# jopohl/urh

Measured on NVIDIA H100. Metric: MSamples/s IQ demod+digitize (complex64), higher is better.
Workload: dtype f32

## Files before the change

urh_b200/csrc/center.cu:

```cuda
#include "dense.cuh"
#include "scan.cuh"

#include <math.h>
#include <stdlib.h>

int urh_window_var_bitwise(urh_ctx* ctx, const float* d_x, int64_t n, const int64_t* d_prefix, int64_t t0, int64_t t1, int64_t r0,
                           int64_t r1, float* h_out2);

struct CenStats {
    double sum, sumsq;
    float mn, mx;
    long long cnt;
};

__global__ void __launch_bounds__(URH_WARPS_PER_BLOCK * 32)
k_tile_stats_f32(const float* __restrict__ x, int64_t n, int64_t ntiles, UrhTileStats* __restrict__ ts) {
    const int lane = threadIdx.x & 31;
    const int64_t tile = (int64_t)blockIdx.x * URH_WARPS_PER_BLOCK + (threadIdx.x >> 5);
    if (tile >= ntiles) return;
    const int64_t base = tile * URH_TILE;
    UrhStatAcc acc;
    acc.init();
    acc.all_noise = false;
    if (base + URH_TILE <= n && (((uintptr_t)x) & 15) == 0) {
// ... 344 lines not shown
    const int lane = threadIdx.x & 31;
    if (SMEM)
        for (int b = threadIdx.x; b < nbins; b += 256) s_hist[b] = 0u;
    if (edges_in_smem)
        for (int b = threadIdx.x; b < nbins + 3; b += 256) s_fe[b] = g_fe[b];
    __syncthreads();
    HistBins hb;
    if (FAST) hb.load(s_fe, scale, nbins);
    else hb.load(edges_in_smem ? s_fe : g_fe, scale, nbins);
    HistCache hc;
    hc.init();
    const int64_t gw = (int64_t)blk * 8 + (threadIdx.x >> 5), nw = (int64_t)nblk * 8;
    const bool vec = (((uintptr_t)x) & 15) == 0;
    const unsigned one = blockDim.x >> 8;
    {
        for (int64_t t = t_first + gw; t < t_end; t += nw) {
            if (prefix[t + 1] == prefix[t]) continue;
            const int64_t base = t * URH_TILE;
            if (vec) {
                const float4* p = (const float4*)(x + base) + lane;
                constexpr int ITERS = URH_TILE / 128, DEPTH = 4;
                float4 buf[DEPTH];
#pragma unroll
                for (int j = 0; j < DEPTH; j++) buf[j] = __ldg(p + j * 32);
#pragma unroll 1
                for (int it = 0; it < ITERS; it += DEPTH) {
                    const bool more = it + DEPTH < ITERS;
#pragma unroll
                    for (int j = 0; j < DEPTH; j++) {
                        const float4 v = buf[j];
                        if (more) buf[j] = __ldg(p + (it + DEPTH + j) * 32);
                        hist_put<SMEM, FAST>(hc, hb, s_hist, hist, v.x, one);
                        hist_put<SMEM, FAST>(hc, hb, s_hist, hist, v.y, one);
                        hist_put<SMEM, FAST>(hc, hb, s_hist, hist, v.z, one);
                        hist_put<SMEM, FAST>(hc, hb, s_hist, hist, v.w, one);
                    }
                }
            } else {
                for (int j = lane; j < URH_TILE; j += 32) hist_put<SMEM, FAST>(hc, hb, s_hist, hist, x[base + j], one);
            }
        }
    }
    hist_flush<SMEM>(hc, s_hist, hist);
    if (SMEM) {
        __syncthreads();
        for (int b = threadIdx.x; b < nbins; b += 256)
            if (s_hist[b]) atomicAdd(&hist[b], (unsigned long long)s_hist[b]);
    }
}

template <bool SMEM, bool FAST>
__global__ void __launch_bounds__(256, 4) k_hist_interior(const float* __restrict__ x, int64_t n, const int64_t* __restrict__ win,
                                                      const float* __restrict__ g_fe, float scale, int nbins,
                                                      unsigned long long* __restrict__ hist, int edges_in_smem,
                                                      const int64_t* __restrict__ prefix) {
    const int64_t w0 = win[0];
    hist_interior_body<SMEM, FAST>(x, n, w0 + 1, w0 >= 0 ? win[1] : 0, blockIdx.x, gridDim.x, g_fe, scale, nbins, hist, edges_in_smem, prefix);
}

__device__ __forceinline__ void hist_window_ends_body(const float* __restrict__ x, int64_t n, const int64_t* __restrict__ prefix,
                                                      const int64_t* __restrict__ win, int64_t r0, int64_t r1,
                                                      const float* __restrict__ g_fe, float scale, int nbins,
                                                      unsigned long long* __restrict__ hist, unsigned long long* __restrict__ hist2 = nullptr) {
    __shared__ int s_pre[256];
    const int64_t t = win[blockIdx.x];
    if (t < 0 || (blockIdx.x == 1 && t == win[0])) return;
    HistBins hb;
    hb.load(g_fe, scale, nbins);
    float v[CEN_PER];
    int64_t rank = cen_tile_ranks(x, n, t, prefix[t], v, s_pre);
#pragma unroll
    for (int j = 0; j < CEN_PER; j++) {
        const bool kept = v[j] > -4.0f;
        const int k = hb.bin_of<false>(v[j]);
        if (k >= 0 && rank >= r0 && rank < r1) {
            atomicAdd(&hist[k], 1ull);
            if (hist2) atomicAdd(&hist2[k], 1ull);
        }
        rank += kept ? 1 : 0;
    }
}

__global__ void __launch_bounds__(256) k_hist_window_ends(const float* __restrict__ x, int64_t n, const int64_t* __restrict__ prefix,
                                                         const int64_t* __restrict__ win, int64_t r0, int64_t r1,
                                                         const float* __restrict__ g_fe, float scale, int nbins,
                                                         unsigned long long* __restrict__ hist) {
    hist_window_ends_body(x, n, prefix, win, r0, r1, g_fe, scale, nbins, hist);
}

extern "C" int urh_center_histogram_tiles(urh_ctx* ctx, const float* d_qad, int64_t n, int64_t r0, int64_t r1, double hmin,
                                          double hstep, int64_t nbins, int64_t* h_hist) {
    if (nbins <= 0) return URH_OK;
    if (!tiles_match(ctx, d_qad, n)) URH_FAIL(ctx, URH_ERR_INVALID, "urh_afp_demod_tiles (same qad, same n) must precede urh_center_histogram_tiles");
    if (nbins > (int64_t)1 << 30) URH_FAIL(ctx, URH_ERR_INVALID, "too many histogram bins");
    const int64_t ntiles = urh_div_up(n, URH_TILE);
    const int64_t* prefix = (const int64_t*)ctx->center_prefix;
    unsigned long long* hist;
    float* fe;
    int64_t* d_win;
    URH_CHECK(urh_arena(ctx, (size_t)nbins, &hist));
    URH_CHECK(urh_arena(ctx, (size_t)nbins + 3, &fe));
    URH_CHECK(urh_arena(ctx, 4, &d_win));
    URH_CUDA(ctx, cudaMemsetAsync(hist, 0, (size_t)nbins * sizeof(unsigned long long), ctx->stream));
    URH_CUDA(ctx, cudaMemsetAsync(d_win, 0xff, 4 * sizeof(int64_t), ctx->stream));
    if (r1 > r0) {
        URH_LAUNCH(ctx, k_hist_edges, (unsigned)urh_div_up(nbins + 1, 256), 256, 0, hmin, hstep, nbins, fe);
        URH_LAUNCH(ctx, k_find_window_tiles, (unsigned)urh_div_up(ntiles, 256), 256, 0, prefix, ntiles, r0, r1, d_win);
        const bool in_smem = nbins <= 12000;
        const int edges_smem = (in_smem && nbins <= 6000) ? 1 : 0;
        const size_t dyn = (in_smem ? (size_t)nbins * 4 : 0) + (edges_smem ? (size_t)(nbins + 3) * 4 : 0);
        const float scale = (float)(1.0 / hstep);
        const double edge_abs = fmax(fabs(hmin), fabs(hmin + (double)nbins * hstep));
        const bool fast = edges_smem && hstep > 0.0 && edge_abs / hstep < 1048576.0;
        const unsigned gs = (unsigned)min(urh_div_up(ntiles, 8), (int64_t)ctx->sm_count * 8);
        const int64_t* cw = d_win;
        const float* cfe = fe;
        if (in_smem && fast) URH_LAUNCH(ctx, (k_hist_interior<true, true>), gs, 256, dyn, d_qad, n, cw, cfe, scale, (int)nbins, hist, edges_smem, prefix);
        else if (in_smem) URH_LAUNCH(ctx, (k_hist_interior<true, false>), gs, 256, dyn, d_qad, n, cw, cfe, scale, (int)nbins, hist, edges_smem, prefix);
        else URH_LAUNCH(ctx, (k_hist_interior<false, false>), gs, 256, dyn, d_qad, n, cw, cfe, scale, (int)nbins, hist, edges_smem, prefix);
        URH_LAUNCH(ctx, k_hist_window_ends, 2, 256, 0, d_qad, n, prefix, (const int64_t*)d_win, r0, r1, (const float*)fe, scale, (int)nbins, hist);
    }
    URH_CUDA(ctx, cudaMemcpyAsync(h_hist, hist, (size_t)nbins * sizeof(int64_t), cudaMemcpyDeviceToHost, ctx->stream));
    URH_CUDA(ctx, cudaStreamSynchronize(ctx->stream));
    return URH_OK;
}

extern "C" int urh_center_histogram(urh_ctx* ctx, const float* d_x, int64_t n, int64_t r0, int64_t r1, double hmin,
                                    double hstep, int64_t nbins, int64_t* h_hist) {
    if (nbins <= 0 || n <= 0) return URH_OK;
    if (!tiles_match(ctx, d_x, n)) {
        int64_t total = 0;
        URH_CHECK(tiles_from_array(ctx, d_x, n, &total));
    }
    return urh_center_histogram_tiles(ctx, d_x, n, r0, r1, hmin, hstep, nbins, h_hist);
}

#include "tilescan.cuh"

#define CEN_MAX_BINS 6000

struct __align__(16) CenterPlan {
    long long total, offset;
    long long r0, r1;
    long long lr0, lr1;
    long long win[4];
    CenStats local;
    double hmin, edge1, delta;
    long long nbins;
    double center;
    float centerf;
    float scale;
    int fast;
    int state;
    unsigned int ticket;
    int certified;
    long long straddle;
    long long pad;
};

struct ScanKept {
    const UrhTileStats* ts;
    int64_t* prefix;
    __device__ __forceinline__ int64_t load(int64_t t) const { return ts[t].cnt; }
    __device__ __forceinline__ void post(int64_t t, const int64_t& excl, const int64_t&) const { prefix[t] = excl; }
};
struct CenAddI64 {
    __device__ __forceinline__ int64_t operator()(int64_t a, int64_t b) const { return a + b; }
};

__global__ void k_center_ranks(const int64_t* __restrict__ counts, int rank, int world, int64_t max_size, CenterPlan* __restrict__ plan) {
    long long total = 0, offset = 0;
    for (int q = 0; q < world; q++) {
        if (q < rank) offset += counts[q];
        total += counts[q];
    }
    const long long kept = counts[rank];
    long long r0 = (long long)(0.05 * (double)total), r1 = (long long)(0.95 * (double)total);
    if (max_size >= 0 && r1 - r0 > max_size) r1 = r0 + max_size;
    plan->total = total; plan->offset = offset; plan->r0 = r0; plan->r1 = r1;
    long long a = r0 - offset, b = r1 - offset;
    a = a < 0 ? 0 : (a > kept ? kept : a);
    b = b < 0 ? 0 : (b > kept ? kept : b);
    plan->lr0 = a; plan->lr1 = b;
    plan->ticket = 0u;
    plan->state = 1;
    plan->certified = 0;
    plan->straddle = 0;
}

__device__ __forceinline__ int64_t cen_tile_of_rank(const int64_t* __restrict__ prefix, int64_t ntiles, int64_t r) {
    int64_t lo = 0, hi = ntiles;
    while (hi - lo > 1) {
        const int64_t mid = (lo + hi) >> 1;
        if (prefix[mid] <= r) lo = mid; else hi = mid;
    }
    return lo;
}

__global__ void __launch_bounds__(256) k_center_window(const float* __restrict__ x, int64_t n, const UrhTileStats* __restrict__ ts,
                                                      const int64_t* __restrict__ prefix, int64_t ntiles, CenterPlan* __restrict__ plan,
                                                      CenStats* __restrict__ partial) {
    __shared__ long long s_win[4];
    __shared__ int s_pre[256];
    __shared__ bool s_last;
    const long long r0 = plan->lr0, r1 = plan->lr1;
    if (threadIdx.x == 0) {
        long long w0 = -1, w1 = -1, w2 = -1, w3 = -1;
        if (r1 > r0) {
            w0 = cen_tile_of_rank(prefix, ntiles, r0);
            w1 = cen_tile_of_rank(prefix, ntiles, r1 - 1);
            const bool cov0 = prefix[w0] >= r0 && prefix[w0 + 1] <= r1;
            const bool cov1 = prefix[w1] >= r0 && prefix[w1 + 1] <= r1;
            w2 = cov0 ? -1 : w0;
            w3 = (cov1 || w1 == w0) ? -1 : w1;
        }
        s_win[0] = w0; s_win[1] = w1; s_win[2] = w2; s_win[3] = w3;
        if (blockIdx.x == 0) { plan->win[0] = w0; plan->win[1] = w1; plan->win[2] = w2; plan->win[3] = w3; }
    }
    __syncthreads();
    double sum = 0.0, sq = 0.0;
    float mn = INFINITY, mx = -INFINITY;
    long long cnt = 0;
    if (s_win[0] >= 0) {
        for (int64_t t = s_win[0] + (int64_t)blockIdx.x * 256 + threadIdx.x; t <= s_win[1]; t += (int64_t)gridDim.x * 256) {
            const int64_t a = prefix[t], b = prefix[t + 1];
            if (b > a && a >= r0 && b <= r1) {
                const UrhTileStats v = ts[t];
                sum += v.sum; sq += v.sumsq; mn = fminf(mn, v.mn); mx = fmaxf(mx, v.mx); cnt += v.cnt;
            }
        }
    }
    cen_block_fold(sum, sq, mn, mx, cnt, partial + blockIdx.x);
    if (blockIdx.x < 2) {
        const int64_t t = s_win[2 + blockIdx.x];
        sum = 0.0; sq = 0.0; mn = INFINITY; mx = -INFINITY; cnt = 0;
        if (t >= 0) {
            float v[CEN_PER];
            int64_t rank = cen_tile_ranks(x, n, t, prefix[t], v, s_pre);
#pragma unroll
            for (int j = 0; j < CEN_PER; j++) {
                if (v[j] > -4.0f) {
                    if (rank >= r0 && rank < r1) {
                        sum += (double)v[j];
                        sq += (double)v[j] * (double)v[j];
                        mn = fminf(mn, v[j]);
                        mx = fmaxf(mx, v[j]);
                        cnt++;
                    }
                    rank++;
                }
            }
        }
        cen_block_fold(sum, sq, mn, mx, cnt, partial + gridDim.x + blockIdx.x);
    }
    __threadfence();
    __syncthreads();
    if (threadIdx.x == 0) s_last = atomicAdd(&plan->ticket, 1u) == gridDim.x - 1;
    __syncthreads();
    if (!s_last) return;
    __threadfence();
    sum = 0.0; sq = 0.0; mn = INFINITY; mx = -INFINITY; cnt = 0;
    for (int64_t t = threadIdx.x; t < (int64_t)gridDim.x + 2; t += 256) {
        CenStats p;
        {
            const int4* src = (const int4*)(partial + t);
            int4 w0 = __ldcg(src), w1 = __ldcg(src + 1);
            memcpy(&p, &w0, 16);
            memcpy((char*)&p + 16, &w1, 16);
        }
        sum += p.sum; sq += p.sumsq; mn = fminf(mn, p.mn); mx = fmaxf(mx, p.mx); cnt += p.cnt;
    }
    cen_block_fold(sum, sq, mn, mx, cnt, &plan->local);
}

__global__ void __launch_bounds__(256) k_center_plan(const CenStats* __restrict__ parts, int world, CenterPlan* __restrict__ plan,
                                                    float* __restrict__ fe, unsigned long long* __restrict__ hist,
                                                    unsigned long long* __restrict__ xhist) {
    __shared__ int s_state;
    __shared__ long long s_nbins;
    __shared__ double s_hmin, s_edge1, s_delta;
    if (threadIdx.x == 0) {
        double cnt = 0.0, sum = 0.0, sq = 0.0;
        float mn = INFINITY, mx = -INFINITY;
        for (int q = 0; q < world; q++) {
            cnt += (double)parts[q].cnt;
            mn = fminf(mn, parts[q].mn);
            mx = fmaxf(mx, parts[q].mx);
            sum = __dadd_rn(sum, parts[q].sum);
            sq = __dadd_rn(sq, parts[q].sumsq);
        }
        int state = 0;
        long long nbins = 0;
        double hmin = 0.0, edge1 = 0.0, delta = 0.0;
        if (plan->r1 > plan->r0 && cnt > 0.0) {
            const double mean = __ddiv_rn(sum, cnt);
            double ss = __dsub_rn(sq, __dmul_rn(__dmul_rn(cnt, mean), mean));
            if (ss < 0.0) ss = 0.0;
            const double var = __ddiv_rn(ss, cnt);
            const double hstep = (double)__double2float_rn(var);
            hmin = (double)mn;
            const double stop = __dadd_rn((double)mx, hstep);
            if (hstep != 0.0) {
                const double val = __ddiv_rn(__dsub_rn(stop, hmin), hstep);
                if (val == val && fabs(val) < 9.0e18) {
                    const long long len = (long long)ceil(val);
                    if (len >= 2) {
                        nbins = len - 1;
                        edge1 = __dadd_rn(hmin, hstep);
                        delta = __dsub_rn(edge1, hmin);
                        state = (nbins <= CEN_MAX_BINS && delta > 0.0) ? 1 : 2;
                    }
                }
            }
        }
        plan->hmin = hmin; plan->edge1 = edge1; plan->delta = delta; plan->nbins = nbins;
        plan->state = state;
        plan->center = 0.0; plan->centerf = 0.0f;
        if (state == 1) {
            plan->scale = (float)(1.0 / delta);
            const double edge_abs = fmax(fabs(hmin), fabs(hmin + (double)nbins * delta));
            plan->fast = (edge_abs / delta < 1048576.0) ? 1 : 0;
        }
        s_state = state; s_nbins = nbins; s_hmin = hmin; s_edge1 = edge1; s_delta = delta;
    }
    __syncthreads();
    if (s_state != 1) return;
    const long long nbins = s_nbins;
    for (long long k = threadIdx.x; k <= nbins; k += 256) {
        const double e = (k == 0) ? s_hmin : (k == 1 ? s_edge1 : __dadd_rn(s_hmin, __dmul_rn((double)k, s_delta)));
        fe[k] = __double2float_ru(e);
        if (k == nbins) {
            fe[nbins + 1] = __double2float_rd(e);
            fe[nbins + 2] = fmaxf(__double2float_ru(s_hmin), nextafterf(-4.0f, 0.0f));
        }
        if (k < nbins) {
            hist[k] = 0ull;
            if (xhist) xhist[k] = 0ull;
        }
    }
}

template <bool FAST>
__global__ void __launch_bounds__(256, 3) k_hist_interior_dev(const float* __restrict__ x, int64_t n, const CenterPlan* __restrict__ plan,
                                                          const float* __restrict__ g_fe, unsigned long long* __restrict__ hist,
                                                          const int64_t* __restrict__ prefix) {
    if (plan->state != 1 || plan->certified || (plan->fast != 0) != FAST) return;
    hist_interior_body<true, FAST>(x, n, plan->win[0] + 1, plan->win[1], blockIdx.x, gridDim.x, g_fe, plan->scale, (int)plan->nbins, hist, 1,
                                   prefix);
}

__device__ __forceinline__ void cen_full_slabs(int64_t win0, int64_t win1, int64_t slab_tiles, int64_t* sf, int64_t* se) {
    *sf = (win0 + slab_tiles) / slab_tiles;
    *se = win1 / slab_tiles;
}

__global__ void __launch_bounds__(256) k_hist_window_ends_dev(const float* __restrict__ x, int64_t n, const int64_t* __restrict__ prefix,
                                                             const CenterPlan* __restrict__ plan, const float* __restrict__ g_fe,
                                                             unsigned long long* __restrict__ hist, unsigned long long* __restrict__ xhist,
                                                             int64_t slab_tiles) {
    if (plan->state != 1) return;
    if (blockIdx.x < 2) {
        hist_window_ends_body(x, n, prefix, (const int64_t*)plan->win, plan->lr0, plan->lr1, g_fe, plan->scale, (int)plan->nbins, hist, xhist);
        return;
    }
    const int64_t w0 = plan->win[0], w1 = plan->win[1];
    int64_t sf, se;
    cen_full_slabs(w0, w1, slab_tiles, &sf, &se);
    int64_t a_end = w1, b_begin = w1;
    if (sf < se) { a_end = sf * slab_tiles; b_begin = se * slab_tiles; }
    const int blk = blockIdx.x - 2, nblk = gridDim.x - 2, nbins = (int)plan->nbins;
    const float scale = plan->scale;
    if (plan->fast) {
        hist_interior_body<true, true>(x, n, w0 + 1, a_end, blk, nblk, g_fe, scale, nbins, xhist, 1, prefix);
        hist_interior_body<true, true>(x, n, b_begin, w1, blk, nblk, g_fe, scale, nbins, xhist, 1, prefix);
    } else {
        hist_interior_body<true, false>(x, n, w0 + 1, a_end, blk, nblk, g_fe, scale, nbins, xhist, 1, prefix);
        hist_interior_body<true, false>(x, n, b_begin, w1, blk, nblk, g_fe, scale, nbins, xhist, 1, prefix);
    }
}

__device__ __forceinline__ double cen_left_edge(const CenterPlan* plan, int k) {
    return (k == 0) ? plan->hmin : (k == 1 ? plan->edge1 : __dadd_rn(plan->hmin, __dmul_rn((double)k, plan->delta)));
}

#define CERT_THREADS 512
__global__ void __launch_bounds__(CERT_THREADS) k_center_certify(const UrhFine fine, CenterPlan* __restrict__ plan, const float* __restrict__ fe,
                                                                 const unsigned long long* __restrict__ xhist, unsigned long long* __restrict__ lo,
                                                                 unsigned long long* __restrict__ hi) {
    __shared__ unsigned long long s_ge[URH_FINE_NB + 1];
    __shared__ unsigned long long s_part[CERT_THREADS];
    __shared__ unsigned char s_flag[CEN_MAX_BINS];
    __shared__ unsigned long long s_key[3];
    __shared__ unsigned int s_certain;
    if (plan->state != 1) return;
    const int tid = threadIdx.x;
    constexpr int PER = URH_FINE_NB / CERT_THREADS;
    int64_t sf, se;
    cen_full_slabs(plan->win[0], plan->win[1], fine.slab_tiles, &sf, &se);
    unsigned long long b[PER], tot = 0;
#pragma unroll
    for (int j = 0; j < PER; j++) {
        unsigned long long v = 0;
        for (int64_t sl = sf; sl < se; sl++) v += fine.gh[sl * URH_FINE_NB + tid * PER + j];
        b[j] = v;
        tot += v;
    }
    s_part[tid] = tot;
    if (tid < 3) s_key[tid] = 0ull;
    if (tid == 0) s_certain = 0u;
    __syncthreads();
    for (int off = 1; off < CERT_THREADS; off <<= 1) {
        const unsigned long long add = (tid + off < CERT_THREADS) ? s_part[tid + off] : 0ull;
        __syncthreads();
        s_part[tid] += add;
        __syncthreads();
    }
    unsigned long long run = (tid + 1 < CERT_THREADS) ? s_part[tid + 1] : 0ull;
#pragma unroll
    for (int j = PER - 1; j >= 0; j--) {
        run += b[j];
        s_ge[tid * PER + j] = run;
    }
    if (tid == 0) s_ge[URH_FINE_NB] = 0ull;
    __syncthreads();
    const int nbins = (int)plan->nbins;
    const float f_hi = fe[nbins + 1], f_min = fe[nbins + 2], top = nextafterf(f_hi, INFINITY);
    auto ge = [&](float t, unsigned long long& glo, unsigned long long& ghi) {
        const int bt = urh_fine_bucket(t, fine.scale, fine.off);
        const bool straddles = urh_fine_bucket(nextafterf(t, -INFINITY), fine.scale, fine.off) == bt;
        ghi = s_ge[bt];
        glo = straddles ? s_ge[bt + 1] : s_ge[bt];
    };
    for (int k = tid; k < nbins; k += CERT_THREADS) {
        const float a = fmaxf(fe[k], f_min), e = (k == nbins - 1) ? top : fminf(fe[k + 1], top);
        unsigned long long l = 0, u = 0;
        if (a < e) {
            unsigned long long alo, ahi, elo, ehi;
            ge(a, alo, ahi);
            ge(e, elo, ehi);
            l = alo > ehi ? alo - ehi : 0ull;
            u = ahi - elo;
        }
        lo[k] = xhist[k] + l;
        hi[k] = xhist[k] + u;
    }
    __syncthreads();
    int window = (int)(0.05 * (double)nbins) + 1;
    if (window < 2) window = 2;
    for (int k = tid; k < nbins; k += CERT_THREADS) {
        const unsigned long long l = lo[k], u = hi[k];
        bool certain = l > 0ull, possible = u > 0ull;
        for (int d = -(window - 1); d < window && (certain || possible); d++) {
            const int j = k + d;
            if (d == 0 || j < 0 || j >= nbins) continue;
            certain = certain && l > hi[j];
            possible = possible && u > lo[j];
        }
        s_flag[k] = certain ? 1 : (possible ? 2 : 0);
        if (certain) atomicAdd(&s_certain, 1u);
    }
    __syncthreads();
    for (int pass = 0; pass < 3; pass++) {
        const long long p0 = pass > 0 ? (long long)(8191 - (s_key[0] & 8191)) : -1, p1 = pass > 1 ? (long long)(8191 - (s_key[1] & 8191)) : -1;
        for (int k = tid; k < nbins; k += CERT_THREADS) {
            if (k == p0 || k == p1) continue;
            if (pass < 2 && s_flag[k] == 1) atomicMax(&s_key[pass], (lo[k] << 13) | (unsigned long long)(8191 - k));
            if (pass == 2 && s_flag[k] != 0) atomicMax(&s_key[2], hi[k]);
        }
        __syncthreads();
    }
    if (tid != 0 || s_certain < 2u) return;
    const int k1 = 8191 - (int)(s_key[0] & 8191), k2 = 8191 - (int)(s_key[1] & 8191);
    plan->straddle = (long long)((hi[k1] - lo[k1]) + (hi[k2] - lo[k2]));
    if (!(lo[k2] > s_key[2])) return;
    const double c = __ddiv_rn(__dadd_rn(cen_left_edge(plan, k1), cen_left_edge(plan, k2)), 2.0);
    plan->center = c;
    plan->centerf = __double2float_rn(c);
    plan->certified = 1;
}

__global__ void __launch_bounds__(256) k_center_pick(const unsigned long long* __restrict__ y, CenterPlan* __restrict__ plan) {
    __shared__ unsigned long long s_best[256];
    __shared__ int s_idx[256];
    __shared__ int s_cnt[256];
    if (plan->state != 1 || plan->certified) return;
    const int nbins = (int)plan->nbins;
    int window = (int)(0.05 * (double)nbins) + 1;
    if (window < 2) window = 2;
    unsigned long long top_val[2] = {0ull, 0ull};
    int top_idx[2] = {-1, -1};
    int found = 0;
    bool undecided = false;
    for (int pass = 0; pass < 2 && !undecided; pass++) {
        unsigned long long best = 0ull;
        int bi = -1, ties = 0;
        for (int i = threadIdx.x; i < nbins; i += 256) {
            if (pass == 1 && i == top_idx[0]) continue;
            const unsigned long long v = y[i];
            if (v == 0ull || v < best) continue;
            bool peak = true;
            for (int d = 1; d < window && peak; d++) {
                const unsigned long long a = (i + d < nbins) ? y[i + d] : 0ull;
                const unsigned long long b = (i - d >= 0) ? y[i - d] : 0ull;
                peak = v > a && v > b;
            }
            if (!peak) continue;
            if (v > best) { best = v; bi = i; ties = 1; }
            else ties++;
        }
        s_best[threadIdx.x] = best; s_idx[threadIdx.x] = bi; s_cnt[threadIdx.x] = ties;
        __syncthreads();
        if (threadIdx.x == 0) {
            unsigned long long b = 0ull;
            int idx = -1, t = 0;
            for (int j = 0; j < 256; j++) {
                if (s_idx[j] < 0) continue;
                if (s_best[j] > b) { b = s_best[j]; idx = s_idx[j]; t = s_cnt[j]; }
                else if (s_best[j] == b) t += s_cnt[j];
            }
            s_best[0] = b; s_idx[0] = idx; s_cnt[0] = t;
        }
        __syncthreads();
        const unsigned long long b = s_best[0];
        const int idx = s_idx[0], t = s_cnt[0];
        __syncthreads();
        if (idx < 0) break;
        if (pass == 0) {
            top_val[0] = b; top_idx[0] = idx; found = 1;
            if (t == 2) {
                int other = -1;
                for (int i = threadIdx.x; i < nbins; i += 256) {
                    if (i == idx || y[i] != b) continue;
                    bool peak = true;
                    for (int d = 1; d < window && peak; d++) {
                        const unsigned long long a = (i + d < nbins) ? y[i + d] : 0ull;
                        const unsigned long long c = (i - d >= 0) ? y[i - d] : 0ull;
                        peak = b > a && b > c;
                    }
                    if (peak) other = i;
                }
                s_idx[threadIdx.x] = other;
                __syncthreads();
                if (threadIdx.x == 0) {
                    int o = -1;
                    for (int j = 0; j < 256; j++) if (s_idx[j] >= 0) o = s_idx[j];
                    s_idx[0] = o;
                }
                __syncthreads();
                top_idx[1] = s_idx[0]; top_val[1] = b; found = 2;
                __syncthreads();
                break;
            }
            if (t > 2) undecided = true;
        } else {
            if (t > 1) undecided = true;
            else { top_val[1] = b; top_idx[1] = idx; found = 2; }
        }
    }
    if (threadIdx.x != 0) return;
    if (undecided) { plan->state = 2; return; }
    if (found == 0) { plan->state = 0; return; }
    double c;
    if (found == 1) c = cen_left_edge(plan, top_idx[0]);
    else c = __ddiv_rn(__dadd_rn(cen_left_edge(plan, top_idx[0]), cen_left_edge(plan, top_idx[1])), 2.0);
    plan->center = c;
    plan->centerf = __double2float_rn(c);
    plan->state = 1;
    (void)top_val;
}

int urh_coll_allgather(urh_ctx* ctx, const void* d_send, void* d_recv, size_t bytes_per_rank);
bool urh_p2p_usable(urh_ctx* ctx, size_t bytes_per_rank);
extern "C" int urh_p2p_allreduce_u64_dev(urh_ctx* ctx, const void* d_in, void* d_out, const int64_t* d_count, int max_words);
extern "C" int urh_nccl_allreduce_i64(urh_ctx* ctx, int64_t* d_buf, int64_t count, int op);

int urh_center_chain(urh_ctx* ctx, const float* d_qad, int64_t n, const UrhTileStats* ts, int64_t max_size, int rank, int world,
                     const UrhFine* fine, CenterPlan** d_plan_out) {
    const int64_t ntiles = urh_div_up(n, URH_TILE);
    int64_t* prefix;
    CenterPlan* plan;
    CenStats* partial;
    float* fe;
    unsigned long long* hist;
    int64_t* d_counts;
    CenStats* d_parts;
    unsigned long long *xhist = nullptr, *cert_lo = nullptr, *cert_hi = nullptr;
    const int nb = ctx->sm_count * 2;
    URH_CHECK(urh_arena(ctx, (size_t)ntiles + 1, &prefix));
    URH_CHECK(urh_arena(ctx, 1, &plan));
    URH_CHECK(urh_arena(ctx, (size_t)nb + 2, &partial));
    URH_CHECK(urh_arena(ctx, (size_t)CEN_MAX_BINS + 3, &fe));
    URH_CHECK(urh_arena(ctx, (size_t)CEN_MAX_BINS, &hist));
    URH_CHECK(urh_arena(ctx, (size_t)world, &d_counts));
    URH_CHECK(urh_arena(ctx, (size_t)world, &d_parts));
    if (fine) {
        URH_CHECK(urh_arena(ctx, (size_t)CEN_MAX_BINS, &xhist));
        URH_CHECK(urh_arena(ctx, (size_t)CEN_MAX_BINS, &cert_lo));
        URH_CHECK(urh_arena(ctx, (size_t)CEN_MAX_BINS, &cert_hi));
    }
    ScanKept fk;
    fk.ts = ts; fk.prefix = prefix;
    URH_CHECK((urhts::scan<int64_t, CenAddI64, ScanKept>(ctx, ntiles, (int64_t)0, CenAddI64(), fk, prefix + ntiles)));
    const int64_t* counts = prefix + ntiles;
    if (world > 1) {
        URH_TL_MARK(ctx, "x1 kept counts: enter");
        URH_CHECK(urh_coll_allgather(ctx, prefix + ntiles, d_counts, sizeof(int64_t)));
        URH_TL_MARK(ctx, "x1 kept counts: done");
        counts = d_counts;
    }
    URH_LAUNCH(ctx, k_center_ranks, 1, 1, 0, counts, rank, world, max_size, plan);
    URH_LAUNCH(ctx, k_center_window, nb, 256, 0, d_qad, n, ts, (const int64_t*)prefix, ntiles, plan, partial);
    const CenStats* parts = &plan->local;
    if (world > 1) {
        URH_TL_MARK(ctx, "x2 window partials: enter");
        URH_CHECK(urh_coll_allgather(ctx, &plan->local, d_parts, sizeof(CenStats)));
        URH_TL_MARK(ctx, "x2 window partials: done");
        parts = d_parts;
    }
    URH_LAUNCH(ctx, k_center_plan, 1, 256, 0, parts, world, plan, fe, hist, xhist);
    const size_t dyn = (size_t)CEN_MAX_BINS * 4 + (size_t)(CEN_MAX_BINS + 3) * 4;
    const unsigned gs = (unsigned)min(urh_div_up(ntiles, 8), (int64_t)ctx->sm_count * 8);
    URH_LAUNCH(ctx, k_hist_window_ends_dev, fine ? 2 + ctx->sm_count * 4 : 2, 256, fine ? dyn : 0, d_qad, n, (const int64_t*)prefix,
               (const CenterPlan*)plan, (const float*)fe, hist, xhist, fine ? fine->slab_tiles : (int64_t)1);
    if (fine) URH_LAUNCH(ctx, k_center_certify, 1, CERT_THREADS, 0, *fine, plan, (const float*)fe, (const unsigned long long*)xhist, cert_lo, cert_hi);
    URH_LAUNCH(ctx, (k_hist_interior_dev<true>), gs, 256, dyn, d_qad, n, (const CenterPlan*)plan, (const float*)fe, hist, (const int64_t*)prefix);
    URH_LAUNCH(ctx, (k_hist_interior_dev<false>), gs, 256, dyn, d_qad, n, (const CenterPlan*)plan, (const float*)fe, hist, (const int64_t*)prefix);
    const unsigned long long* hist_all = hist;
    if (world > 1) URH_TL_MARK(ctx, "x3 histogram sum: enter");
    if (world > 1) {
        if (urh_p2p_usable(ctx, 8)) {
            unsigned long long* hist_sum;
            URH_CHECK(urh_arena(ctx, (size_t)CEN_MAX_BINS, &hist_sum));
            URH_CHECK(urh_p2p_allreduce_u64_dev(ctx, hist, hist_sum, (const int64_t*)&plan->nbins, CEN_MAX_BINS));
            hist_all = hist_sum;
        } else {
            URH_CHECK(urh_nccl_allreduce_i64(ctx, (int64_t*)hist, CEN_MAX_BINS, 0));
        }
    }
    if (world > 1) URH_TL_MARK(ctx, "x3 histogram sum: done");
    URH_LAUNCH(ctx, k_center_pick, 1, 256, 0, hist_all, plan);
    ctx->center_prefix = prefix;
    ctx->center_ts = ts;
    ctx->center_n = n;
    ctx->center_x = d_qad;
    *d_plan_out = plan;
    return URH_OK;
}

int urh_center_plan_certify_stats(urh_ctx* ctx, const CenterPlan* plan, int64_t* h_dst3) {
    h_dst3[0] = h_dst3[1] = h_dst3[2] = 0;
    URH_CUDA(ctx, cudaMemcpyAsync(h_dst3, &plan->certified, sizeof(int), cudaMemcpyDeviceToHost, ctx->stream));
    URH_CUDA(ctx, cudaMemcpyAsync(h_dst3 + 2, &plan->straddle, sizeof(long long), cudaMemcpyDeviceToHost, ctx->stream));
    return URH_OK;
}

extern "C" int urh_center_certify_stats(urh_ctx* ctx, int64_t* h_out3) {
    for (int i = 0; i < 3; i++) h_out3[i] = ctx->center_cert[i];
    return URH_OK;
}

int urh_center_plan_result(urh_ctx* ctx, const CenterPlan* plan, const float** d_centerf, const double** d_center, const int** d_state) {
    if (d_centerf) *d_centerf = &plan->centerf;
    if (d_center) *d_center = &plan->center;
    if (d_state) *d_state = &plan->state;
    return URH_OK;
}
```

urh_b200/csrc/common.cuh:

```cuda
#pragma once
#include <cuda_runtime.h>
#include <stdint.h>
#include <stdio.h>
#include <stdlib.h>
#include <string.h>
#include <vector>

#include "../../include/urh_b200.h"

#define URH_FULL_MASK 0xffffffffu

struct urh_block {
    void* ptr;
    size_t bytes;
};

struct urh_ctx {
    int device;
    int sm_count;
    cudaStream_t stream;
    cudaStream_t copy_stream[2];
    cudaEvent_t ev_start, ev_stop;
    cudaEvent_t ev_copy[2], ev_comp[2];
    cudaEvent_t ev_k0, ev_k1;
    int profiling;
    int dense_timed;
    cudaEvent_t tl_ev[32];
    const char* tl_name[32];
    int tl_count, tl_ready;
    char err[512];
    int64_t launches;
    std::vector<urh_block> arena;
    size_t arena_block;
    size_t arena_used;
    size_t arena_need;
    int64_t* pulses;
    size_t pulses_cap_rows;
    int64_t pulses_k;
    int64_t* h_mail;
    void* h_stage[2];
    size_t h_stage_bytes;
    int fft_plan;
    int fft_nfft;
    int64_t fft_batch;
    bool fft_valid;
    void* img_tw;
    int img_tw_n;
    void* shard_tiles;
    void* shard_staging;
    int shard_cap, shard_tol;
    int64_t shard_n;
    void* shard_state;
    int64_t costas_stats[3];
    int64_t costas_redone;
    int64_t costas_stitch[4];
    int mod_plan[2];
    int mod_plan_valid[2];
    int64_t mod_plan_n[2];
    int bits_valid;
    int64_t bits_nmsg, bits_total, bits_npos;
    void *bits_ptr, *bits_msg_off, *bits_pauses, *bits_pos;
    const void* center_ts;
    const void* center_x;
    int64_t center_n;
    void* center_prefix;
    int64_t center_cert[3];
    int64_t spec_stats[3];
    void* nccl_comm;
    void* nccl_stage;
    void* nccl_hstage;
    int nccl_rank, nccl_world;
    void* p2p_local;
    void* p2p_peer[8];
    void* p2p_hout;
    int p2p_rank, p2p_world;
    unsigned long long p2p_seq;
    void* ts_mem;
    int64_t ts_cap_blocks;
    unsigned long long ts_issued;
    uint32_t ts_epoch;
    void* step_dev;
    void* shard_fin;
    int64_t stream_free_low, stream_chunks;
    size_t arena_live;
    size_t arena_peak;
};

#define URH_CUDA(ctx, call)                                                                         \
    do {                                                                                            \
        cudaError_t e__ = (call);                                                                   \
        if (e__ != cudaSuccess) {                                                                   \
            snprintf((ctx)->err, sizeof((ctx)->err), "%s:%d: %s -> %s", __FILE__, __LINE__, #call,  \
                     cudaGetErrorString(e__));                                                      \
            return (e__ == cudaErrorMemoryAllocation) ? URH_ERR_NOMEM : URH_ERR_CUDA;               \
        }                                                                                           \
    } while (0)

#define URH_CHECK(call)                 \
    do {                                \
        int rc__ = (call);              \
        if (rc__ != URH_OK) return rc__; \
    } while (0)

#define URH_FAIL(ctx, code, ...)                                  \
    do {                                                          \
        snprintf((ctx)->err, sizeof((ctx)->err), __VA_ARGS__);    \
        return (code);                                            \
    } while (0)

#define URH_LAUNCH(ctx, kernel, grid, block, smem, ...)                                   \
    do {                                                                                  \
        kernel<<<(grid), (block), (smem), (ctx)->stream>>>(__VA_ARGS__);                  \
        (ctx)->launches++;                                                                \
        URH_CUDA(ctx, cudaGetLastError());                                                \
    } while (0)

#define URH_TL_MARK(ctx, label) do { if ((ctx)->profiling >= 2 && (ctx)->tl_ready && (ctx)->tl_count < 32) { \
        (ctx)->tl_name[(ctx)->tl_count] = (label); cudaEventRecord((ctx)->tl_ev[(ctx)->tl_count++], (ctx)->stream); } } while (0)
#define URH_TL_RESET(ctx) do { (ctx)->tl_count = 0; } while (0)
#define URH_PROF_BEGIN(ctx) do { if ((ctx)->profiling) cudaEventRecord((ctx)->ev_k0, (ctx)->stream); } while (0)
#define URH_PROF_END(ctx) do { if ((ctx)->profiling) { cudaEventRecord((ctx)->ev_k1, (ctx)->stream); (ctx)->dense_timed = 1; } } while (0)

void urh_arena_reset(urh_ctx* ctx);
int urh_arena_alloc(urh_ctx* ctx, size_t bytes, void** out);
template <typename T>
static inline int urh_arena(urh_ctx* ctx, size_t count, T** out) {
    void* p = nullptr;
    int rc = urh_arena_alloc(ctx, count * sizeof(T), &p);
    *out = (T*)p;
    return rc;
}
struct UrhArenaMark {
    size_t block, used, live;
};
static inline UrhArenaMark urh_arena_mark(const urh_ctx* ctx) { return UrhArenaMark{ctx->arena_block, ctx->arena_used, ctx->arena_live}; }
static inline void urh_arena_release(urh_ctx* ctx, const UrhArenaMark& m) {
    ctx->arena_block = m.block;
    ctx->arena_used = m.used;
    ctx->arena_live = m.live;
}
int urh_ensure_pulses(urh_ctx* ctx, size_t rows);
int urh_ensure_pulses_keep(urh_ctx* ctx, size_t rows, size_t keep);
void urh_stream_sample_free(urh_ctx* ctx);
void urh_release_mod_plans(urh_ctx* ctx);
int urh_ensure_stage(urh_ctx* ctx, size_t bytes);

struct UrhCostasStream {
    float* state;
    int64_t* acc;
    int segs;
};
int urh_costas_stream_begin(urh_ctx* ctx, UrhCostasStream* S);
int urh_costas_stream_chunk(urh_ctx* ctx, UrhCostasStream* S, int64_t c, const void* d_iq, int dtype, int64_t n, float noise_sqrd,
                            int loop_order, float bandwidth, float* d_out);
int urh_costas_stream_end(urh_ctx* ctx, const UrhCostasStream* S);
int64_t urh_costas_arena_bytes(int64_t n, int loop_order);

int urh_read_i64(urh_ctx* ctx, const int64_t* d_src, int count, int64_t* h_out);

__host__ __device__ static inline int64_t urh_div_up(int64_t a, int64_t b) { return (a + b - 1) / b; }

static inline int urh_iq_bytes(int dtype) {
    switch (dtype) {
        case URH_DT_I8:
        case URH_DT_U8: return 2;
        case URH_DT_I16:
        case URH_DT_U16: return 4;
        case URH_DT_F32: return 8;
        default: return 0;
    }
}

static inline float urh_noise_value(int mod_type) {
    switch (mod_type) {
        case URH_MOD_ASK: return 0.0f;
        case URH_MOD_FSK:
        case URH_MOD_PSK:
        case URH_MOD_OQPSK: return -4.0f;
        case URH_MOD_QAM: return 0.0f * -4.0f;
        default: return 0.0f;
    }
}
```

urh_b200/csrc/context.cu:

```cuda
#include "common.cuh"
#include "tilescan.cuh"

extern "C" int urh_device_count(void) {
    int n = 0;
    if (cudaGetDeviceCount(&n) != cudaSuccess) return 0;
    return n;
}

extern "C" int urh_ctx_create(int device, urh_ctx** out) {
    if (!out) return URH_ERR_INVALID;
    *out = nullptr;
    int n = 0;
    if (cudaGetDeviceCount(&n) != cudaSuccess || n <= 0) return URH_ERR_NO_DEVICE;
    if (device < 0 || device >= n) return URH_ERR_INVALID;
    urh_ctx* ctx = new urh_ctx();
    ctx->device = device;
    ctx->err[0] = 0;
    ctx->launches = 0;
    ctx->arena_block = 0;
    ctx->arena_used = 0;
    ctx->arena_need = 0;
    ctx->pulses = nullptr;
    ctx->pulses_cap_rows = 0;
    ctx->pulses_k = 0;
    ctx->h_mail = nullptr;
    ctx->h_stage[0] = ctx->h_stage[1] = nullptr;
    ctx->h_stage_bytes = 0;
    ctx->fft_valid = false;
    ctx->shard_tiles = nullptr;
    ctx->shard_staging = nullptr;
    ctx->shard_state = nullptr;
    ctx->bits_valid = 0;
    ctx->mod_plan_valid[0] = ctx->mod_plan_valid[1] = 0;
    ctx->center_prefix = nullptr;
    ctx->center_ts = nullptr;
    ctx->center_x = nullptr;
    ctx->center_n = 0;
    ctx->nccl_comm = nullptr;
    ctx->nccl_stage = nullptr;
    ctx->nccl_hstage = nullptr;
    ctx->p2p_local = nullptr;
    ctx->p2p_hout = nullptr;
    ctx->p2p_world = 0;
    ctx->p2p_rank = 0;
    ctx->p2p_seq = 0;
    for (int i = 0; i < 8; i++) ctx->p2p_peer[i] = nullptr;
    ctx->nccl_rank = 0;
    ctx->nccl_world = 1;
    ctx->stream_free_low = -1;
    ctx->stream_chunks = 0;
    if (cudaSetDevice(device) != cudaSuccess) {
        delete ctx;
        return URH_ERR_CUDA;
    }
    cudaDeviceProp prop;
    if (cudaGetDeviceProperties(&prop, device) != cudaSuccess) {
        delete ctx;
        return URH_ERR_CUDA;
    }
    ctx->sm_count = prop.multiProcessorCount;
    {
        cudaMemPool_t pool;
        if (cudaDeviceGetDefaultMemPool(&pool, device) == cudaSuccess) {
            unsigned long long keep = ~0ull;
            cudaMemPoolSetAttribute(pool, cudaMemPoolAttrReleaseThreshold, &keep);
        }
    }
    bool ok = cudaStreamCreateWithFlags(&ctx->stream, cudaStreamNonBlocking) == cudaSuccess;
    ok = ok && cudaStreamCreateWithFlags(&ctx->copy_stream[0], cudaStreamNonBlocking) == cudaSuccess;
    ok = ok && cudaStreamCreateWithFlags(&ctx->copy_stream[1], cudaStreamNonBlocking) == cudaSuccess;
    ok = ok && cudaEventCreate(&ctx->ev_start) == cudaSuccess && cudaEventCreate(&ctx->ev_stop) == cudaSuccess;
    for (int i = 0; i < 2 && ok; i++) {
        ok = ok && cudaEventCreateWithFlags(&ctx->ev_copy[i], cudaEventDisableTiming) == cudaSuccess;
        ok = ok && cudaEventCreateWithFlags(&ctx->ev_comp[i], cudaEventDisableTiming) == cudaSuccess;
    }
    ok = ok && cudaEventCreate(&ctx->ev_k0) == cudaSuccess && cudaEventCreate(&ctx->ev_k1) == cudaSuccess;
    ctx->profiling = 0;
    ctx->dense_timed = 0;
    ctx->tl_count = 0;
    ctx->tl_ready = 0;
    ok = ok && cudaHostAlloc((void**)&ctx->h_mail, 64 * sizeof(int64_t), cudaHostAllocDefault) == cudaSuccess;
    if (!ok) {
        delete ctx;
        return URH_ERR_CUDA;
    }
    *out = ctx;
    return URH_OK;
}

extern "C" void urh_ctx_destroy(urh_ctx* ctx) {
    if (!ctx) return;
    cudaSetDevice(ctx->device);
    cudaStreamSynchronize(ctx->stream);
    urh_release_mod_plans(ctx);
    for (auto& b : ctx->arena) cudaFree(b.ptr);
    if (ctx->pulses) cudaFree(ctx->pulses);
    if (ctx->shard_state) free(ctx->shard_state);
    if (ctx->h_mail) cudaFreeHost(ctx->h_mail);
    if (ctx->ts_mem) cudaFree(ctx->ts_mem);
    if (ctx->step_dev) cudaFree(ctx->step_dev);
    if (ctx->img_tw) cudaFree(ctx->img_tw);
    if (ctx->shard_fin) free(ctx->shard_fin);
    for (int i = 0; i < 2; i++)
        if (ctx->h_stage[i]) cudaFreeHost(ctx->h_stage[i]);
    cudaEventDestroy(ctx->ev_start);
    cudaEventDestroy(ctx->ev_stop);
    for (int i = 0; i < 2; i++) {
        cudaEventDestroy(ctx->ev_copy[i]);
        cudaEventDestroy(ctx->ev_comp[i]);
        cudaStreamDestroy(ctx->copy_stream[i]);
    }
    cudaStreamDestroy(ctx->stream);
    delete ctx;
}

extern "C" const char* urh_last_error(urh_ctx* ctx) { return ctx ? ctx->err : "null context"; }

extern "C" int urh_sync(urh_ctx* ctx) {
    URH_CUDA(ctx, cudaStreamSynchronize(ctx->stream));
    return URH_OK;
}

extern "C" int urh_device_info(urh_ctx* ctx, int* sm_count, int* cc_major, int* cc_minor, size_t* total_mem,
                               char* name, int name_cap) {
    cudaDeviceProp prop;
    URH_CUDA(ctx, cudaGetDeviceProperties(&prop, ctx->device));
    if (sm_count) *sm_count = prop.multiProcessorCount;
    if (cc_major) *cc_major = prop.major;
    if (cc_minor) *cc_minor = prop.minor;
    if (total_mem) *total_mem = prop.totalGlobalMem;
    if (name && name_cap > 0) {
        strncpy(name, prop.name, name_cap - 1);
        name[name_cap - 1] = 0;
    }
    return URH_OK;
}

extern "C" int urh_malloc(urh_ctx* ctx, size_t bytes, void** d_ptr) {
    URH_CUDA(ctx, cudaSetDevice(ctx->device));
    if (bytes == 0) bytes = 16;
    URH_CUDA(ctx, cudaMallocAsync(d_ptr, bytes, ctx->stream));
    return URH_OK;
}

extern "C" int urh_free(urh_ctx* ctx, void* d_ptr) {
    if (!d_ptr) return URH_OK;
    URH_CUDA(ctx, cudaFreeAsync(d_ptr, ctx->stream));
    return URH_OK;
}

extern "C" int urh_memset(urh_ctx* ctx, void* d_ptr, int value, size_t bytes) {
    URH_CUDA(ctx, cudaMemsetAsync(d_ptr, value, bytes, ctx->stream));
    return URH_OK;
}

extern "C" int urh_memcpy_h2d(urh_ctx* ctx, void* d_dst, const void* h_src, size_t bytes) {
    if (bytes == 0) return URH_OK;
    URH_CUDA(ctx, cudaMemcpyAsync(d_dst, h_src, bytes, cudaMemcpyHostToDevice, ctx->stream));
    return URH_OK;
}

extern "C" int urh_memcpy_d2h(urh_ctx* ctx, void* h_dst, const void* d_src, size_t bytes) {
    if (bytes) URH_CUDA(ctx, cudaMemcpyAsync(h_dst, d_src, bytes, cudaMemcpyDeviceToHost, ctx->stream));
    URH_CUDA(ctx, cudaStreamSynchronize(ctx->stream));
    return URH_OK;
}

extern "C" int urh_memcpy_d2d(urh_ctx* ctx, void* d_dst, const void* d_src, size_t bytes) {
    if (bytes == 0) return URH_OK;
    URH_CUDA(ctx, cudaMemcpyAsync(d_dst, d_src, bytes, cudaMemcpyDeviceToDevice, ctx->stream));
    return URH_OK;
}

extern "C" int urh_host_alloc(urh_ctx* ctx, size_t bytes, void** h_ptr) {
    if (bytes == 0) bytes = 16;
    URH_CUDA(ctx, cudaHostAlloc(h_ptr, bytes, cudaHostAllocDefault));
    return URH_OK;
}

extern "C" int urh_host_free(urh_ctx* ctx, void* h_ptr) {
    if (h_ptr) URH_CUDA(ctx, cudaFreeHost(h_ptr));
    return URH_OK;
}

extern "C" int urh_timer_start(urh_ctx* ctx) {
    URH_CUDA(ctx, cudaEventRecord(ctx->ev_start, ctx->stream));
    return URH_OK;
}

extern "C" int urh_timer_stop(urh_ctx* ctx, float* ms) {
    URH_CUDA(ctx, cudaEventRecord(ctx->ev_stop, ctx->stream));
    URH_CUDA(ctx, cudaEventSynchronize(ctx->ev_stop));
    float t = 0.f;
    URH_CUDA(ctx, cudaEventElapsedTime(&t, ctx->ev_start, ctx->ev_stop));
    if (ms) *ms = t;
    return URH_OK;
}

extern "C" int urh_set_profiling(urh_ctx* ctx, int enabled) {
    ctx->profiling = enabled < 0 ? 0 : (enabled > 2 ? 2 : enabled);
    ctx->dense_timed = 0;
    if (ctx->profiling >= 2 && !ctx->tl_ready) {
        for (int i = 0; i < 32; i++) URH_CUDA(ctx, cudaEventCreate(&ctx->tl_ev[i]));
        ctx->tl_ready = 1;
    }
    ctx->tl_count = 0;
    return URH_OK;
}

extern "C" int urh_timeline_fetch(urh_ctx* ctx, float* h_ms, char* h_names, int names_cap, int* count) {
    if (!count) return URH_ERR_INVALID;
    *count = 0;
    if (ctx->profiling < 2 || ctx->tl_count == 0) return URH_OK;
    URH_CUDA(ctx, cudaEventSynchronize(ctx->tl_ev[ctx->tl_count - 1]));
    int pos = 0;
    for (int i = 0; i < ctx->tl_count; i++) {
        float t = 0.f;
        URH_CUDA(ctx, cudaEventElapsedTime(&t, ctx->tl_ev[0], ctx->tl_ev[i]));
        if (h_ms) h_ms[i] = t;
        if (h_names) pos += snprintf(h_names + pos, pos < names_cap ? (size_t)(names_cap - pos) : 0, "%s\n", ctx->tl_name[i]);
    }
    *count = ctx->tl_count;
    return URH_OK;
}

extern "C" int urh_last_dense_ms(urh_ctx* ctx, float* ms) {
    if (!ctx->dense_timed) URH_FAIL(ctx, URH_ERR_INVALID, "no dense kernel timed (enable urh_set_profiling first)");
    URH_CUDA(ctx, cudaEventSynchronize(ctx->ev_k1));
    URH_CUDA(ctx, cudaEventElapsedTime(ms, ctx->ev_k0, ctx->ev_k1));
    return URH_OK;
}

extern "C" int64_t urh_launch_count(urh_ctx* ctx) { return ctx ? ctx->launches : 0; }

void urh_arena_reset(urh_ctx* ctx) {
    if (ctx->arena.size() > 1) {
        cudaStreamSynchronize(ctx->stream);
        size_t total = 0;
        for (auto& b : ctx->arena) {
            total += b.bytes;
            cudaFree(b.ptr);
        }
        ctx->arena.clear();
        void* p = nullptr;
        if (cudaMalloc(&p, total) == cudaSuccess) ctx->arena.push_back({p, total});
        else cudaGetLastError();
    }
    ctx->arena_block = 0;
    ctx->arena_used = 0;
    ctx->arena_need = 0;
    ctx->arena_live = 0;
    ctx->arena_peak = 0;
    ctx->center_prefix = nullptr;
    ctx->bits_valid = 0;
}

static void arena_note_peak(urh_ctx* ctx) {
    if (ctx->arena_live > ctx->arena_peak) ctx->arena_peak = ctx->arena_live;
}

int urh_arena_alloc(urh_ctx* ctx, size_t bytes, void** out) {
    bytes = (bytes + 255) & ~(size_t)255;
    if (bytes == 0) bytes = 256;
    ctx->arena_need += bytes;
// ... 126 lines not shown
```

urh_b200/csrc/digitize.cu:

```cuda
#include "dense.cuh"
#include "scan.cuh"
#include "sparse.cuh"
#ifndef URH_FAST_MIN_BLOCKS
#define URH_FAST_MIN_BLOCKS 4
#endif
#include "fsk_fast.cuh"
#include "dense_f32.cuh"
#include "stream_ring.cuh"

#include <math.h>
#include <stdlib.h>


template <int DT, int MOD, bool DIGITIZE>
__device__ __forceinline__ void dense_iq_tile(const void* __restrict__ iq, int64_t n, const UrhDemodParams& dp, float* __restrict__ qad_out,
                                              int vec_in, int vec_out, const UrhClassify& cls, int tol, UrhTileSummary* __restrict__ tiles,
                                              uint32_t* __restrict__ staging, int stage_cap, int16_t* __restrict__ init_cls, int cls_of_zero,
                                              int64_t tile, int has_halo, UrhTileStats* __restrict__ tile_stats, const UrhFine& fine,
                                              unsigned int* s_fine, unsigned int* g_fine) {
    const int lane = threadIdx.x & 31;
    const int64_t tile_start = tile * URH_TILE;
    const int tile_len = (int)((n - tile_start) < URH_TILE ? (n - tile_start) : URH_TILE);
    const int iters = (tile_len + 63) >> 6;

    UrhRunTracker rt;
    if (DIGITIZE) rt.init(tol, staging + tile * (int64_t)stage_cap);
    UrhStatAcc acc;
    acc.init();

    float cA = 0.0f, cB = 0.0f;
    if (MOD == URH_MOD_FSK && (tile_start > 0 || has_halo) && lane == 0) {
        typedef typename UrhElem<DT>::type E;
        const E* pp = (const E*)iq + 2 * (tile_start - 1);
        const UrhFskTerms t = urh_fsk_terms((float)pp[0], (float)pp[1]);
        cA = t.A; cB = t.B;
    }

    UrhPair cur = urh_load_pair<DT>(iq, tile_start + 2 * lane, n, vec_in != 0);
    for (int it = 0; it < iters; it++) {
        const int64_t pos0 = tile_start + (int64_t)it * 64 + 2 * lane;
        UrhPair nxt;
        if (it + 1 < iters) nxt = urh_load_pair<DT>(iq, pos0 + 64, n, vec_in != 0);

        const float m0 = __fadd_rn(__fmul_rn(cur.r0, cur.r0), __fmul_rn(cur.i0, cur.i0));
        const float m1 = __fadd_rn(__fmul_rn(cur.r1, cur.r1), __fmul_rn(cur.i1, cur.i1));
        float s0 = dp.noise_value, s1 = dp.noise_value;
        if (MOD == URH_MOD_FSK) {
            const UrhFskTerms t0 = urh_fsk_terms(cur.r0, cur.i0);
            const UrhFskTerms t1 = urh_fsk_terms(cur.r1, cur.i1);
            float pA = __shfl_up_sync(URH_FULL_MASK, t1.A, 1);
            float pB = __shfl_up_sync(URH_FULL_MASK, t1.B, 1);
            if (lane == 0) { pA = cA; pB = cB; }
            cA = __shfl_sync(URH_FULL_MASK, t1.A, 31);
            cB = __shfl_sync(URH_FULL_MASK, t1.B, 31);
            if (!(m0 <= dp.noise_sqrd)) s0 = urh_fsk_angle(pA, pB, t0.C, t0.D);
            if (!(m1 <= dp.noise_sqrd)) s1 = urh_fsk_angle(t0.A, t0.B, t1.C, t1.D);
        } else if (MOD == URH_MOD_ASK) {
            if (!(m0 <= dp.noise_sqrd)) s0 = __fdiv_rn(__fsqrt_rn(m0), dp.max_mag);
            if (!(m1 <= dp.noise_sqrd)) s1 = __fdiv_rn(__fsqrt_rn(m1), dp.max_mag);
        }
        if (pos0 == 0 && !has_halo) s0 = dp.noise_value;

        const bool v0 = pos0 < n, v1 = pos0 + 1 < n;
        if (tile_stats) {
            if (v0) { acc.add(s0); acc.all_noise = acc.all_noise && (s0 == dp.noise_value); }
            if (v1) { acc.add(s1); acc.all_noise = acc.all_noise && (s1 == dp.noise_value); }
            if (s_fine) {
                if (v0) urh_fine_add(s0, fine, s_fine, g_fine);
                if (v1) urh_fine_add(s1, fine, s_fine, g_fine);
            }
        }
        if (qad_out) {
            if (v1 && vec_out) urh_stg_f2(qad_out + pos0, s0, s1);
            else {
                if (v0) qad_out[pos0] = s0;
                if (v1) qad_out[pos0 + 1] = s1;
            }
        }
        if (DIGITIZE) {
            const int c0 = urh_classify(s0, cls), c1 = urh_classify(s1, cls);
            if (pos0 == 0) *init_cls = (int16_t)((s0 == cls.noise_value) ? -1 : cls_of_zero);
            rt.feed(it, c0, c1, v0, v1, lane);
        }
        cur = nxt;
    }
    if (tile_stats) acc.store(tile_stats + tile, lane);
    if (DIGITIZE) rt.finish(tile_len, tiles + tile, lane);
}

template <int DT, int MOD, bool DIGITIZE>
__global__ void __launch_bounds__(URH_WARPS_PER_BLOCK * 32)
k_dense_iq(const void* __restrict__ iq, int64_t n, UrhDemodParams dp, float* __restrict__ qad_out, int vec_in,
           int vec_out, const __grid_constant__ UrhClassify cls, int tol, UrhTileSummary* __restrict__ tiles,
           uint32_t* __restrict__ staging, int stage_cap, int16_t* __restrict__ init_cls, int cls_of_zero,
           int64_t tile_begin, int64_t tile_count, int has_halo, UrhTileStats* __restrict__ tile_stats, const UrhFine fine) {
    extern __shared__ unsigned int s_fine[];
    const int64_t tile_rel = (int64_t)blockIdx.x * URH_WARPS_PER_BLOCK + (threadIdx.x >> 5);
    const int64_t block_tile0 = tile_begin + (int64_t)blockIdx.x * URH_WARPS_PER_BLOCK;
    if (fine.gh) urh_fine_zero(s_fine);
    if (tile_rel < tile_count && (tile_begin + tile_rel) * URH_TILE < n)
        dense_iq_tile<DT, MOD, DIGITIZE>(iq, n, dp, qad_out, vec_in, vec_out, cls, tol, tiles, staging, stage_cap, init_cls, cls_of_zero,
                                    tile_begin + tile_rel, has_halo, tile_stats, fine,
                                    fine.gh ? s_fine : nullptr, fine.gh ? urh_fine_row(fine, tile_begin + tile_rel, block_tile0) : nullptr);
    if (fine.gh) urh_fine_flush(fine, s_fine, block_tile0);
}

template <int DT, bool DIGITIZE, bool WRITE, bool STATS>
__global__ void __launch_bounds__(URH_WARPS_PER_BLOCK * 32, URH_FAST_MIN_BLOCKS)
k_fsk_fast(const void* __restrict__ iq, int64_t n, UrhDemodParams dp, float* __restrict__ qad_out, float thr0,
           float cls_noise, int tol, UrhTileSummary* __restrict__ tiles, uint32_t* __restrict__ staging, int stage_cap,
           int64_t tile_begin, int64_t tile_count, UrhTileStats* __restrict__ tile_stats, const UrhFine fine) {
    extern __shared__ unsigned int s_fine[];
    const bool fine_on = STATS && fine.gh;
    const int lane = threadIdx.x & 31;
    const int64_t tile_rel = (int64_t)blockIdx.x * URH_WARPS_PER_BLOCK + (threadIdx.x >> 5);
    const int64_t block_tile0 = tile_begin + (int64_t)blockIdx.x * URH_WARPS_PER_BLOCK;
    if (fine_on) urh_fine_zero(s_fine);
    if (tile_rel < tile_count) {
        const int64_t tile = tile_begin + tile_rel;
        UrhRunTracker rt;
        if (DIGITIZE) rt.init(tol, staging + tile * (int64_t)stage_cap);
        UrhOne one;
        one.p = dp.one;
        one.m = dp.mone;
        urh_fsk_full_tile<DT, DIGITIZE, WRITE, STATS>(iq, n, tile * URH_TILE, dp, qad_out, thr0, cls_noise, rt, lane, one,
                                                      STATS ? tile_stats + tile : nullptr, 0u, DIGITIZE ? tiles + tile : nullptr, fine,
                                                      fine_on ? s_fine : nullptr, fine_on ? urh_fine_row(fine, tile, block_tile0) : nullptr);
    }
    if (fine_on) urh_fine_flush(fine, s_fine, block_tile0);
}

#define URH_FSK_FIFO 3
template <int DT, bool DIGITIZE, bool WRITE, bool STATS>
__global__ void __launch_bounds__(URH_WARPS_PER_BLOCK * 32, (DT == URH_DT_F32) ? 5 : 4)
k_fsk_fifo(const void* __restrict__ iq, int64_t n, UrhDemodParams dp, float* __restrict__ qad_out, float thr0,
           float cls_noise, int tol, UrhTileSummary* __restrict__ tiles, uint32_t* __restrict__ staging, int stage_cap,
           int64_t tile_begin, int64_t tile_count, UrhTileStats* __restrict__ tile_stats, const UrhFine fine,
           const float* __restrict__ d_thr0 = nullptr, float* __restrict__ margin = nullptr) {
    __shared__ __align__(16) unsigned char s_fifo[URH_WARPS_PER_BLOCK][URH_FSK_FIFO + 1][64 * 2 * sizeof(typename UrhElem<DT>::type)];
    extern __shared__ unsigned int s_fine[];
    const bool fine_on = STATS && fine.gh;
    if (DIGITIZE && STATS) thr0 = *d_thr0;
    const int lane = threadIdx.x & 31;
    const int64_t tile_rel = (int64_t)blockIdx.x * URH_WARPS_PER_BLOCK + (threadIdx.x >> 5);
    const int64_t block_tile0 = tile_begin + (int64_t)blockIdx.x * URH_WARPS_PER_BLOCK;
    if (fine_on) urh_fine_zero(s_fine);
    if (tile_rel < tile_count) {
        const int64_t tile = tile_begin + tile_rel;
        UrhRunTracker rt;
        if (DIGITIZE) rt.init(tol, staging + tile * (int64_t)stage_cap);
        UrhOne one;
        one.p = dp.one;
        one.m = dp.mone;
        const uint32_t fifo = (uint32_t)__cvta_generic_to_shared(&s_fifo[threadIdx.x >> 5][0][0]);
        urh_fsk_full_tile<DT, DIGITIZE, WRITE, STATS, URH_FSK_FIFO>(iq, n, tile * URH_TILE, dp, qad_out, thr0, cls_noise, rt, lane, one,
                                                                    STATS ? tile_stats + tile : nullptr, fifo,
                                                                    DIGITIZE ? tiles + tile : nullptr, fine, fine_on ? s_fine : nullptr,
                                                                    fine_on ? urh_fine_row(fine, tile, block_tile0) : nullptr,
                                                                    (DIGITIZE && STATS) ? margin + tile : nullptr);
    }
    if (fine_on) urh_fine_flush(fine, s_fine, block_tile0);
}

#define URH_GUESS_SAMPLES 16384
#define URH_GUESS_BINS 128
#define URH_GUESS_THREADS 1024
__global__ void __launch_bounds__(URH_GUESS_THREADS) k_speculate_guess(const float2* __restrict__ iq, int64_t n, float noise_sqrd, int forced,
                                                                      float forced_tg, float* __restrict__ d_tg, unsigned int* __restrict__ redone) {
    constexpr int PER = URH_GUESS_SAMPLES / URH_GUESS_THREADS;
    __shared__ unsigned int s_hist[URH_GUESS_BINS];
    __shared__ float s_mn[32], s_mx[32];
    if (forced) {
        if (threadIdx.x == 0) { *d_tg = forced_tg; *redone = 0u; }
        return;
    }
    for (int b = threadIdx.x; b < URH_GUESS_BINS; b += blockDim.x) s_hist[b] = 0u;
    float v[PER];
    float mn = INFINITY, mx = -INFINITY;
#pragma unroll
    for (int k = 0; k < PER; k++) {
        const int64_t i = 1 + (int64_t)(k * URH_GUESS_THREADS + threadIdx.x) * (n - 1) / URH_GUESS_SAMPLES;
        const float2 p = iq[i - 1], c = iq[i];
        v[k] = NAN;
        if (!(c.x * c.x + c.y * c.y <= noise_sqrd)) {
            v[k] = atan2f(p.x * c.y - p.y * c.x, p.x * c.x + p.y * c.y);
            mn = fminf(mn, v[k]);
            mx = fmaxf(mx, v[k]);
        }
    }
    for (int off = 16; off > 0; off >>= 1) {
        mn = fminf(mn, __shfl_xor_sync(URH_FULL_MASK, mn, off));
        mx = fmaxf(mx, __shfl_xor_sync(URH_FULL_MASK, mx, off));
    }
    if ((threadIdx.x & 31) == 0) { s_mn[threadIdx.x >> 5] = mn; s_mx[threadIdx.x >> 5] = mx; }
    __syncthreads();
    mn = INFINITY; mx = -INFINITY;
    for (int w = 0; w < URH_GUESS_THREADS / 32; w++) { mn = fminf(mn, s_mn[w]); mx = fmaxf(mx, s_mx[w]); }
    const float width = (mx - mn) / URH_GUESS_BINS;
    if (width > 0.0f) {
#pragma unroll
        for (int k = 0; k < PER; k++)
            if (!isnan(v[k])) atomicAdd(&s_hist[min((int)((v[k] - mn) / width), URH_GUESS_BINS - 1)], 1u);
    }
    __syncthreads();
    if (threadIdx.x != 0) return;
    *redone = 0u;
    if (!(mn <= mx)) { *d_tg = 0.0f; return; }
    if (!(width > 0.0f)) { *d_tg = mn; return; }
    constexpr int WINDOW = (int)(0.05 * URH_GUESS_BINS) + 1;
    int top[2] = {-1, -1};
    for (int b = 0; b < URH_GUESS_BINS; b++) {
        const unsigned int y = s_hist[b];
        bool peak = y > 0u;
        for (int d = 1; d < WINDOW && peak; d++)
            peak = y > (b + d < URH_GUESS_BINS ? s_hist[b + d] : 0u) && y > (b - d >= 0 ? s_hist[b - d] : 0u);
        if (!peak) continue;
        if (top[0] < 0 || y > s_hist[top[0]]) { top[1] = top[0]; top[0] = b; }
        else if (top[1] < 0 || y > s_hist[top[1]]) top[1] = b;
    }
    if (top[0] < 0) *d_tg = 0.5f * (mn + mx);
    else if (top[1] < 0) *d_tg = mn + ((float)top[0] + 0.5f) * width;
    else *d_tg = mn + (0.5f * (float)(top[0] + top[1]) + 0.5f) * width;
}


extern "C" int urh_get_center_thresholds(float center, float spacing, int modulation_order, float* h_out) {
    const int n = modulation_order / 2;
    for (int i = 0; i < n; i++) {
        volatile float t = (float)(n - (i + 1)) * spacing;
        h_out[i] = center - t;
    }
    for (int i = n; i < modulation_order - 1; i++) {
        volatile float t = (float)(i + 1 - n) * spacing;
        h_out[i] = center + t;
    }
    return URH_OK;
}

static int fill_classify(urh_ctx* ctx, UrhClassify* C, int mod_type, float center, uint8_t bits_per_symbol,
                         float spacing) {
    if (bits_per_symbol > 8) URH_FAIL(ctx, URH_ERR_INVALID, "bits_per_symbol %d > 8 not supported", (int)bits_per_symbol);
    memset(C, 0, sizeof(*C));
    C->noise_value = urh_noise_value(mod_type);
    C->order = 1 << bits_per_symbol;
    if (C->order > 1) urh_get_center_thresholds(center, spacing, C->order, C->thr);
    return URH_OK;
}

static int host_classify(float s, const UrhClassify& C) {
    int c = C.order - 1;
    for (int k = 0; k < C.order - 1; k++)
        if (s <= C.thr[k]) { c = k; break; }
    return c;
}

static float max_magnitude_for(int dtype) {
    switch (dtype) {
        case URH_DT_I8: return (float)sqrt(127.0 * 127.0 + 128.0 * 128.0);
        case URH_DT_U8: return (float)sqrt(255.0 * 255.0);
        case URH_DT_I16: return (float)sqrt(32768.0 * 32768.0 + 32767.0 * 32767.0);
        case URH_DT_U16: return (float)sqrt(65535.0 * 65535.0);
        default: return (float)sqrt(2.0);
    }
}

static bool iq_vec_aligned(const void* p, int dtype) { return ((uintptr_t)p % (2 * (size_t)urh_iq_bytes(dtype))) == 0; }

template <int DT, int MOD, bool DIG>
static int launch_dense_iq_t(urh_ctx* ctx, const void* d_iq, int64_t n, const UrhDemodParams& dp, float* d_qad,
                             const UrhClassify& cls, int tol, UrhTileSummary* tiles, uint32_t* staging,
                             int stage_cap, int16_t* init_cls, int cls_of_zero, int has_halo = 0,
                             UrhTileStats* tile_stats = nullptr, int64_t tile_lo = 0, int64_t tile_hi = -1,
                             const UrhFine& fine = UrhFine{}, UrhSpec* spec = nullptr) {
    const int64_t ntiles = urh_div_up(n, URH_TILE);
    const size_t fine_smem = fine.gh ? (size_t)URH_FINE_NB * sizeof(unsigned int) : 0;
    if (tile_hi < 0 || tile_hi > ntiles) tile_hi = ntiles;
    const int vec_in = iq_vec_aligned(d_iq, DT) ? 1 : 0;
    const int vec_out = (d_qad && ((uintptr_t)d_qad % 8) == 0) ? 1 : 0;
    const int threads = URH_WARPS_PER_BLOCK * 32;
    auto generic = [&](int64_t begin, int64_t end) -> int {
        begin = begin < tile_lo ? tile_lo : begin;
        end = end > tile_hi ? tile_hi : end;
        const int64_t count = end - begin;
        if (count <= 0) return URH_OK;
        URH_LAUNCH(ctx, (k_dense_iq<DT, MOD, DIG>), (unsigned)urh_div_up(count, URH_WARPS_PER_BLOCK), threads, fine_smem, d_iq, n, dp,
                   d_qad, vec_in, vec_out, cls, tol, tiles, staging, stage_cap, init_cls, cls_of_zero, begin, count, has_halo,
                   tile_stats, fine);
        return URH_OK;
    };
    const int64_t nfull = n / URH_TILE;
    const bool fast = MOD == URH_MOD_FSK && vec_in && (!d_qad || vec_out) && (!DIG || cls.order == 2) && nfull > 1;
    URH_PROF_BEGIN(ctx);
    if (fast) {
        const int64_t fb = tile_lo > 1 ? tile_lo : 1, fe = tile_hi < nfull ? tile_hi : nfull;
        if (fe > fb) {
            const unsigned grid = (unsigned)urh_div_up(fe - fb, URH_WARPS_PER_BLOCK);
            static const bool fifo = getenv("URH_B200_FSK_NO_FIFO") == nullptr;
            const bool ff = fifo;
            bool speculated = false;
            if constexpr (DT == URH_DT_F32 && MOD == URH_MOD_FSK && !DIG) {
                if (spec && ff && tile_stats && d_qad) {
                    URH_LAUNCH(ctx, (k_fsk_fifo<DT, true, true, true>), grid, threads, fine_smem, d_iq, n, dp, d_qad, 0.0f, dp.noise_value,
                               tol, tiles, staging, stage_cap, fb, fe - fb, tile_stats, fine, (const float*)spec->tg, spec->margin);
                    spec->lo = fb;
                    spec->hi = fe;
                    speculated = true;
                }
            }
            if (speculated) {
            } else if (tile_stats && d_qad && !DIG) {
                if (ff) URH_LAUNCH(ctx, (k_fsk_fifo<DT, false, true, true>), grid, threads, fine_smem, d_iq, n, dp, d_qad, cls.thr[0], cls.noise_value,
                                   tol, tiles, staging, stage_cap, fb, fe - fb, tile_stats, fine);
                else URH_LAUNCH(ctx, (k_fsk_fast<DT, false, true, true>), grid, threads, fine_smem, d_iq, n, dp, d_qad, cls.thr[0], cls.noise_value,
                                tol, tiles, staging, stage_cap, fb, fe - fb, tile_stats, fine);
            } else if (d_qad) {
                if (ff) URH_LAUNCH(ctx, (k_fsk_fifo<DT, DIG, true, false>), grid, threads, 0, d_iq, n, dp, d_qad, cls.thr[0], cls.noise_value, tol,
                                   tiles, staging, stage_cap, fb, fe - fb, nullptr, UrhFine{});
                else URH_LAUNCH(ctx, (k_fsk_fast<DT, DIG, true, false>), grid, threads, 0, d_iq, n, dp, d_qad, cls.thr[0], cls.noise_value, tol,
                                tiles, staging, stage_cap, fb, fe - fb, nullptr, UrhFine{});
            } else {
                if (ff) URH_LAUNCH(ctx, (k_fsk_fifo<DT, DIG, false, false>), grid, threads, 0, d_iq, n, dp, d_qad, cls.thr[0], cls.noise_value, tol,
                                   tiles, staging, stage_cap, fb, fe - fb, nullptr, UrhFine{});
                else URH_LAUNCH(ctx, (k_fsk_fast<DT, DIG, false, false>), grid, threads, 0, d_iq, n, dp, d_qad, cls.thr[0], cls.noise_value, tol,
                                tiles, staging, stage_cap, fb, fe - fb, nullptr, UrhFine{});
            }
        }
        URH_CHECK(generic(0, 1));
        URH_CHECK(generic(nfull, ntiles));
    } else {
        URH_CHECK(generic(0, ntiles));
    }
    URH_PROF_END(ctx);
    return URH_OK;
}

template <int MOD, bool DIG>
static int launch_dense_iq_m(urh_ctx* ctx, int dtype, const void* d_iq, int64_t n, const UrhDemodParams& dp,
                             float* d_qad, const UrhClassify& cls, int tol, UrhTileSummary* tiles,
                             uint32_t* staging, int stage_cap, int16_t* init_cls, int cls_of_zero, int has_halo = 0,
                             UrhTileStats* tile_stats = nullptr, int64_t tile_lo = 0, int64_t tile_hi = -1,
                             const UrhFine& fine = UrhFine{}, UrhSpec* spec = nullptr) {
    switch (dtype) {
        case URH_DT_I8: return launch_dense_iq_t<URH_DT_I8, MOD, DIG>(ctx, d_iq, n, dp, d_qad, cls, tol, tiles, staging, stage_cap, init_cls, cls_of_zero, has_halo, tile_stats, tile_lo, tile_hi, fine);
        case URH_DT_U8: return launch_dense_iq_t<URH_DT_U8, MOD, DIG>(ctx, d_iq, n, dp, d_qad, cls, tol, tiles, staging, stage_cap, init_cls, cls_of_zero, has_halo, tile_stats, tile_lo, tile_hi, fine);
        case URH_DT_I16: return launch_dense_iq_t<URH_DT_I16, MOD, DIG>(ctx, d_iq, n, dp, d_qad, cls, tol, tiles, staging, stage_cap, init_cls, cls_of_zero, has_halo, tile_stats, tile_lo, tile_hi, fine);
        case URH_DT_U16: return launch_dense_iq_t<URH_DT_U16, MOD, DIG>(ctx, d_iq, n, dp, d_qad, cls, tol, tiles, staging, stage_cap, init_cls, cls_of_zero, has_halo, tile_stats, tile_lo, tile_hi, fine);
        case URH_DT_F32: return launch_dense_iq_t<URH_DT_F32, MOD, DIG>(ctx, d_iq, n, dp, d_qad, cls, tol, tiles, staging, stage_cap, init_cls, cls_of_zero, has_halo, tile_stats, tile_lo, tile_hi, fine, spec);
        default: URH_FAIL(ctx, URH_ERR_DTYPE, "Unsupported dtype");
    }
}

int urh_costas_demod(urh_ctx* ctx, const void* d_iq, int dtype, int64_t n, float noise_sqrd, int loop_order,
                     float bandwidth, float* d_out);

static UrhDemodParams make_demod_params(float noise_mag, int mod_type, int dtype) {
    UrhDemodParams dp;
    volatile float nm = noise_mag;
    volatile float sq = nm * nm;
    dp.noise_sqrd = sq;
    dp.noise_value = urh_noise_value(mod_type);
    dp.max_mag = max_magnitude_for(dtype);
    dp.one = 1.0f;
    dp.mone = -1.0f;
    return dp;
}

extern "C" int urh_afp_demod(urh_ctx* ctx, const void* d_iq, int dtype, int64_t n, float noise_mag, int mod_type,
                             int mod_order, float costas_loop_bandwidth, float* d_out) {
    if (n < 0) URH_FAIL(ctx, URH_ERR_INVALID, "negative length");
    if (urh_iq_bytes(dtype) == 0) URH_FAIL(ctx, URH_ERR_DTYPE, "Unsupported dtype");
    if (n == 0) return URH_OK;
    if (n <= 2 || (mod_type != URH_MOD_ASK && mod_type != URH_MOD_FSK && mod_type != URH_MOD_PSK)) {
        URH_CUDA(ctx, cudaMemsetAsync(d_out, 0, (size_t)n * sizeof(float), ctx->stream));
        if (n > 2) {
            const float nv = urh_noise_value(mod_type);
            URH_CUDA(ctx, cudaMemcpyAsync(d_out, &nv, sizeof(float), cudaMemcpyHostToDevice, ctx->stream));
            URH_CUDA(ctx, cudaStreamSynchronize(ctx->stream));
        }
        return URH_OK;
    }
    const UrhDemodParams dp = make_demod_params(noise_mag, mod_type, dtype);
    if (mod_type == URH_MOD_PSK) return urh_costas_demod(ctx, d_iq, dtype, n, dp.noise_sqrd, mod_order, costas_loop_bandwidth, d_out);
    UrhClassify cls;
    memset(&cls, 0, sizeof(cls));
    if (mod_type == URH_MOD_ASK)
        return launch_dense_iq_m<URH_MOD_ASK, false>(ctx, dtype, d_iq, n, dp, d_out, cls, 0, nullptr, nullptr, 0, nullptr, 0);
    return launch_dense_iq_m<URH_MOD_FSK, false>(ctx, dtype, d_iq, n, dp, d_out, cls, 0, nullptr, nullptr, 0, nullptr, 0);
}

int urh_center_tiles_begin(urh_ctx* ctx, const float* d_x, const UrhTileStats* ts, int64_t n, int64_t* h_total);

extern "C" int urh_afp_demod_tiles(urh_ctx* ctx, const void* d_iq, int dtype, int64_t n, float noise_mag, int mod_type,
                                   float* d_qad_out, int halo, int64_t* h_kept) {
    if (n <= 2 || (mod_type != URH_MOD_ASK && mod_type != URH_MOD_FSK) || !d_qad_out)
        URH_FAIL(ctx, URH_ERR_INVALID, "urh_afp_demod_tiles: ASK/FSK, n > 2 and a qad buffer are required");
    if (urh_iq_bytes(dtype) == 0) URH_FAIL(ctx, URH_ERR_DTYPE, "Unsupported dtype");
    urh_arena_reset(ctx);
    const UrhDemodParams dp = make_demod_params(noise_mag, mod_type, dtype);
    UrhClassify cls;
    memset(&cls, 0, sizeof(cls));
    const int64_t ntiles = urh_div_up(n, URH_TILE);
    UrhTileStats* ts;
    URH_CHECK(urh_arena(ctx, (size_t)ntiles, &ts));
    if (mod_type == URH_MOD_ASK)
        URH_CHECK((launch_dense_iq_m<URH_MOD_ASK, false>(ctx, dtype, d_iq, n, dp, d_qad_out, cls, 0, nullptr, nullptr, 0, nullptr, 0, halo, ts)));
    else
        URH_CHECK((launch_dense_iq_m<URH_MOD_FSK, false>(ctx, dtype, d_iq, n, dp, d_qad_out, cls, 0, nullptr, nullptr, 0, nullptr, 0, halo, ts)));
    return urh_center_tiles_begin(ctx, d_qad_out, ts, n, h_kept);
}

int urh_finish_local(urh_ctx* ctx, int64_t n, int tol, bool is_ask, uint32_t sps, const UrhTileSummary* tiles, const uint32_t* staging,
                     int stage_cap, const int16_t* d_init, int64_t* k);
int urh_finish_shard(urh_ctx* ctx, int64_t n, int tol, bool is_ask, uint32_t sps, const UrhTileSummary* tiles, const uint32_t* staging,
                     int stage_cap, const int16_t* d_init, int64_t global_offset, int64_t n_total, int64_t* k);

static int digitize_finish(urh_ctx* ctx, int64_t n, int tol, bool is_ask, uint32_t sps, UrhTileSummary* tiles,
                           uint32_t* staging, int stage_cap, int16_t* d_init, int64_t* k) {
    if (getenv("URH_B200_OLD_FINISH")) {
        UrhCandidates cand;
        URH_CHECK(urh_collect_candidates(ctx, n, tol, tiles, staging, stage_cap, &cand));
        return urh_pulses_from_candidates(ctx, n, tol, is_ask, sps, cand, d_init, k);
    }
    return urh_finish_local(ctx, n, tol, is_ask, sps, tiles, staging, stage_cap, d_init, k);
}

static int stage_cap_for(int tol) { return URH_TILE / (tol + 1) + 2; }

extern "C" int urh_grab_pulse_lens(urh_ctx* ctx, const float* d_qad, int64_t n, float center, uint16_t tolerance,
                                   int mod_type, uint32_t samples_per_symbol, uint8_t bits_per_symbol,
                                   float center_spacing, int64_t* k) {
    if (!k) return URH_ERR_INVALID;
    *k = 0;
    ctx->pulses_k = 0;
    if (n < 0) URH_FAIL(ctx, URH_ERR_INVALID, "negative length");
    if (n == 0) return URH_OK;
    urh_arena_reset(ctx);
    UrhClassify cls;
    URH_CHECK(fill_classify(ctx, &cls, mod_type, center, bits_per_symbol, center_spacing));
    const int tol = tolerance;
    const int64_t ntiles = urh_div_up(n, URH_TILE);
    const int cap = stage_cap_for(tol);
    UrhTileSummary* tiles;
    uint32_t* staging;
    int16_t* d_init;
    URH_CHECK(urh_arena(ctx, (size_t)ntiles, &tiles));
    URH_CHECK(urh_arena(ctx, (size_t)ntiles * cap, &staging));
    URH_CHECK(urh_arena(ctx, 8, &d_init));
    const unsigned grid = (unsigned)urh_div_up(ntiles, URH_WARPS_PER_BLOCK);
    const int vec_in = (((uintptr_t)d_qad % 8) == 0) ? 1 : 0;
    URH_PROF_BEGIN(ctx);
    if (cls.order == 2)
        URH_LAUNCH(ctx, (k_dense_f32<SrcQad2, float>), grid, URH_WARPS_PER_BLOCK * 32, 0, d_qad, n, vec_in, cls, tol, tiles,
                   staging, cap, d_init, host_classify(0.0f, cls));
    else
        URH_LAUNCH(ctx, (k_dense_f32<SrcQad, float>), grid, URH_WARPS_PER_BLOCK * 32, 0, d_qad, n, vec_in, cls, tol, tiles,
                   staging, cap, d_init, host_classify(0.0f, cls));
    URH_PROF_END(ctx);
    return digitize_finish(ctx, n, tol, mod_type == URH_MOD_ASK, samples_per_symbol, tiles, staging, cap, d_init, k);
}

extern "C" int urh_demod_digitize(urh_ctx* ctx, const void* d_iq, int dtype, int64_t n, float noise_mag,
                                  int mod_type, float center, uint16_t tolerance, uint32_t samples_per_symbol,
                                  uint8_t bits_per_symbol, float center_spacing, float* d_qad_out, int64_t* k) {
    if (!k) return URH_ERR_INVALID;
    *k = 0;
    ctx->pulses_k = 0;
    if (n < 0) URH_FAIL(ctx, URH_ERR_INVALID, "negative length");
    if (urh_iq_bytes(dtype) == 0) URH_FAIL(ctx, URH_ERR_DTYPE, "Unsupported dtype");
    if (n == 0) return URH_OK;
    if (n <= 2 || (mod_type != URH_MOD_ASK && mod_type != URH_MOD_FSK)) {
        float* q = d_qad_out;
        if (!q) URH_CUDA(ctx, cudaMalloc((void**)&q, (size_t)n * sizeof(float)));
        int rc = urh_afp_demod(ctx, d_iq, dtype, n, noise_mag, mod_type, 1 << bits_per_symbol, 0.1f, q);
        if (rc == URH_OK)
            rc = urh_grab_pulse_lens(ctx, q, n, center, tolerance, mod_type, samples_per_symbol, bits_per_symbol,
                                     center_spacing, k);
        if (!d_qad_out) {
            cudaStreamSynchronize(ctx->stream);
            cudaFree(q);
        }
        return rc;
    }
    urh_arena_reset(ctx);
    UrhClassify cls;
    URH_CHECK(fill_classify(ctx, &cls, mod_type, center, bits_per_symbol, center_spacing));
    const UrhDemodParams dp = make_demod_params(noise_mag, mod_type, dtype);
    const int tol = tolerance;
    const int64_t ntiles = urh_div_up(n, URH_TILE);
    const int cap = stage_cap_for(tol);
    UrhTileSummary* tiles;
    uint32_t* staging;
    int16_t* d_init;
    URH_CHECK(urh_arena(ctx, (size_t)ntiles, &tiles));
    URH_CHECK(urh_arena(ctx, (size_t)ntiles * cap, &staging));
    URH_CHECK(urh_arena(ctx, 8, &d_init));
    const int c0 = host_classify(0.0f, cls);
    if (mod_type == URH_MOD_ASK)
        URH_CHECK((launch_dense_iq_m<URH_MOD_ASK, true>(ctx, dtype, d_iq, n, dp, d_qad_out, cls, tol, tiles, staging, cap, d_init, c0)));
    else
        URH_CHECK((launch_dense_iq_m<URH_MOD_FSK, true>(ctx, dtype, d_iq, n, dp, d_qad_out, cls, tol, tiles, staging, cap, d_init, c0)));
    return digitize_finish(ctx, n, tol, mod_type == URH_MOD_ASK, samples_per_symbol, tiles, staging, cap, d_init, k);
}

extern "C" int urh_shard_dense(urh_ctx* ctx, const void* d_iq, int dtype, int64_t n, int has_halo, float noise_mag, int mod_type,
                               float center, uint16_t tolerance, uint8_t bits_per_symbol, float center_spacing,
                               float* d_qad_out, int64_t* h_summary) {
    if (n <= 0) URH_FAIL(ctx, URH_ERR_INVALID, "empty shard");
    if (mod_type != URH_MOD_ASK && mod_type != URH_MOD_FSK) URH_FAIL(ctx, URH_ERR_INVALID, "sharded path: ASK / FSK only (PSK is a serial recurrence)");
    if (urh_iq_bytes(dtype) == 0) URH_FAIL(ctx, URH_ERR_DTYPE, "Unsupported dtype");
    urh_arena_reset(ctx);
    UrhClassify cls;
    URH_CHECK(fill_classify(ctx, &cls, mod_type, center, bits_per_symbol, center_spacing));
    const UrhDemodParams dp = make_demod_params(noise_mag, mod_type, dtype);
    const int tol = tolerance;
    const int64_t ntiles = urh_div_up(n, URH_TILE);
    const int cap = stage_cap_for(tol);
    UrhTileSummary* tiles;
    uint32_t* staging;
    int16_t* d_init;
    URH_CHECK(urh_arena(ctx, (size_t)ntiles, &tiles));
    URH_CHECK(urh_arena(ctx, (size_t)ntiles * cap, &staging));
    URH_CHECK(urh_arena(ctx, 8, &d_init));
    URH_CUDA(ctx, cudaMemsetAsync(d_init, 0, 16, ctx->stream));
    const int c0 = host_classify(0.0f, cls);
    if (mod_type == URH_MOD_ASK)
        URH_CHECK((launch_dense_iq_m<URH_MOD_ASK, true>(ctx, dtype, d_iq, n, dp, d_qad_out, cls, tol, tiles, staging, cap, d_init, c0, has_halo)));
    else
        URH_CHECK((launch_dense_iq_m<URH_MOD_FSK, true>(ctx, dtype, d_iq, n, dp, d_qad_out, cls, tol, tiles, staging, cap, d_init, c0, has_halo)));
    ctx->shard_tiles = tiles;
    ctx->shard_staging = staging;
    ctx->shard_cap = cap;
    ctx->shard_n = n;
    ctx->shard_tol = tol;
    URH_CHECK(urh_shard_run_total(ctx, n, tiles, h_summary));
    int16_t init16 = 0;
    URH_CUDA(ctx, cudaMemcpyAsync(&init16, d_init, sizeof(int16_t), cudaMemcpyDeviceToHost, ctx->stream));
    URH_CUDA(ctx, cudaStreamSynchronize(ctx->stream));
    h_summary[3] = init16;
    return URH_OK;
}

extern "C" int urh_shard_dense_qad(urh_ctx* ctx, const float* d_qad, int64_t n, int mod_type, float center, uint16_t tolerance,
                                   uint8_t bits_per_symbol, float center_spacing, int64_t* h_summary) {
    if (n <= 0) URH_FAIL(ctx, URH_ERR_INVALID, "empty shard");
    urh_arena_reset(ctx);
    UrhClassify cls;
    URH_CHECK(fill_classify(ctx, &cls, mod_type, center, bits_per_symbol, center_spacing));
    const int tol = tolerance;
    const int64_t ntiles = urh_div_up(n, URH_TILE);
    const int cap = stage_cap_for(tol);
    UrhTileSummary* tiles;
    uint32_t* staging;
    int16_t* d_init;
    URH_CHECK(urh_arena(ctx, (size_t)ntiles, &tiles));
    URH_CHECK(urh_arena(ctx, (size_t)ntiles * cap, &staging));
    URH_CHECK(urh_arena(ctx, 8, &d_init));
    URH_CUDA(ctx, cudaMemsetAsync(d_init, 0, 16, ctx->stream));
    const int vec_in = (((uintptr_t)d_qad % 8) == 0) ? 1 : 0;
    URH_PROF_BEGIN(ctx);
    const unsigned grid = (unsigned)urh_div_up(ntiles, URH_WARPS_PER_BLOCK);
    if (cls.order == 2)
        URH_LAUNCH(ctx, (k_dense_f32<SrcQad2, float>), grid, URH_WARPS_PER_BLOCK * 32, 0, d_qad, n, vec_in, cls, tol, tiles, staging, cap,
                   d_init, host_classify(0.0f, cls));
    else
        URH_LAUNCH(ctx, (k_dense_f32<SrcQad, float>), grid, URH_WARPS_PER_BLOCK * 32, 0, d_qad, n, vec_in, cls, tol, tiles, staging, cap,
                   d_init, host_classify(0.0f, cls));
    URH_PROF_END(ctx);
// ... 83 lines not shown
    } else {
        z.src_slot = (kind == URH_STREAM_ENTRY_GRAB_PULSE_LENS && (entry & URH_STREAM_QAD_ON_DEVICE)) ? 0
                     : URH_STREAM_PAD + z.cs * (iq ? urh_iq_bytes(dtype) : 4);
        const bool qad_ring = kind == URH_STREAM_ENTRY_AFP_DEMOD ||
                              (kind == URH_STREAM_ENTRY_DEMOD_DIGITIZE && ((entry & URH_STREAM_QAD_OUT) || psk));
        z.qad_slot = qad_ring ? z.cs * 4 : 0;
        z.ring_bytes = ring * (r256(z.src_slot) + r256(z.qad_slot));
        if (kind == URH_STREAM_ENTRY_DEMOD_CENTER_DIGITIZE) z.ring_bytes += r256(n * 4);
    }
    z.arena = 0;
    z.scan_items = ct > z.rows_chunk ? ct : z.rows_chunk;
    if (digitize) z.arena += r256(ct * (int64_t)sizeof(UrhTileSummary)) + r256(ct * cap * 4) + r256(16) + r256(sizeof(UrhChain)) +
                             finish_arena_bytes(ct, z.rows_chunk, true);
    if (psk && !resident) z.arena += urh_costas_arena_bytes(z.cs, psk) + r256(16) + r256(6 * 8);
    if (kind == URH_STREAM_ENTRY_DEMOD_CENTER_DIGITIZE) {
        z.arena += r256(ntiles * (int64_t)sizeof(UrhTileStats)) + r256((int64_t)URH_FINE_SLABS * URH_FINE_NB * 4) + r256((ntiles + 1) * 8) +
                   ((int64_t)2 << 20);
        if (ntiles > z.scan_items) z.scan_items = ntiles;
    }
    return z;
}

extern "C" int urh_stream_footprint(int64_t n, int dtype, int tolerance, int64_t chunk_samples, int ring, int entry, int64_t rows,
                                    int64_t* bytes) {
    if (!bytes || n < 0 || tolerance < 0 || tolerance > 0xffff || (entry & 0xf) > URH_STREAM_ENTRY_DEMOD_CENTER_DIGITIZE) return URH_ERR_INVALID;
    if (!(entry & URH_STREAM_RESIDENT) && (ring < 2 || ring > URH_STREAM_MAX_RING)) return URH_ERR_INVALID;
    if ((entry & 0xf) != URH_STREAM_ENTRY_GRAB_PULSE_LENS && urh_iq_bytes(dtype) == 0) return URH_ERR_DTYPE;
    if ((entry & URH_STREAM_PSK) && (entry & 0xf) != URH_STREAM_ENTRY_AFP_DEMOD && (entry & 0xf) != URH_STREAM_ENTRY_DEMOD_DIGITIZE)
        return URH_ERR_INVALID;
    const StreamSizes z = stream_sizes(n, dtype, tolerance, chunk_samples, ring, entry);
    const bool digitize = (entry & 0xf) != URH_STREAM_ENTRY_AFP_DEMOD;
    const int64_t r = rows == -2 ? n / 64 + 1024 : (rows < 0 ? rows_bound(n, tolerance) : rows);
    if (entry & URH_STREAM_RESIDENT) {
        const int64_t ntiles = urh_div_up(n, URH_TILE);
        int64_t b = z.ring_bytes + ((int64_t)64 << 20);
        if (digitize)
            b += r256(ntiles * (int64_t)sizeof(UrhTileSummary)) + r256(ntiles * (int64_t)stage_cap_for(tolerance) * 4) +
                 finish_arena_bytes(ntiles, r + r / 4, true) + 16 * (r + r / 4);
        if ((entry & 0xf) == URH_STREAM_ENTRY_DEMOD_CENTER_DIGITIZE)
            b += r256(ntiles * (int64_t)sizeof(UrhTileStats)) + r256((int64_t)URH_FINE_SLABS * URH_FINE_NB * 4) + r256((ntiles + 1) * 8);
        if (psk_order_of(entry)) b += urh_costas_arena_bytes(n, psk_order_of(entry));
        *bytes = b;
        return URH_OK;
    }
    int64_t b = z.ring_bytes;
    b += 2 * z.arena + ((int64_t)64 << 20);
    const int64_t nb = 2 * (z.scan_items / 256 + 1);
    b += 256 + (nb > 8192 ? nb : 8192) * (4 + 2 * 32);
    if (digitize) b += 3 * 16 * (r + z.rows_chunk);
    *bytes = b;
    return URH_OK;
}

extern "C" int urh_stream_stats(urh_ctx* ctx, int64_t* h_out3) {
    h_out3[0] = ctx->stream_free_low;
    h_out3[1] = ctx->stream_chunks;
    h_out3[2] = (int64_t)ctx->arena_peak;
    return URH_OK;
}

struct StreamDigitizer {
    UrhTileSummary* tiles;
    uint32_t* staging;
    int16_t* d_init;
    UrhChain* chain;
    int cap, tol;
    bool is_ask;
    uint32_t sps;
    int64_t n, rows, rows_all;
    UrhArenaMark mark;
    int init(urh_ctx* ctx, int64_t n_total, int64_t cs, int tolerance, bool ask, uint32_t samples_per_symbol) {
        n = n_total; tol = tolerance; is_ask = ask; sps = samples_per_symbol; rows = 0;
        cap = stage_cap_for(tol);
        rows_all = rows_bound(n, tol);
        const int64_t ct = cs / URH_TILE;
        URH_CHECK(urh_arena(ctx, (size_t)ct, &tiles));
        URH_CHECK(urh_arena(ctx, (size_t)ct * cap, &staging));
        URH_CHECK(urh_arena(ctx, 8, &d_init));
        URH_CHECK(urh_arena(ctx, 1, &chain));
        URH_CUDA(ctx, cudaMemsetAsync(d_init, 0, 16, ctx->stream));
        mark = urh_arena_mark(ctx);
        return URH_OK;
    }
    int finish(urh_ctx* ctx, int64_t s0, int64_t s1) {
        const int64_t rc = rows_bound(s1 - s0, tol);
        const int64_t need = rows + rc;
        if (need > (int64_t)ctx->pulses_cap_rows) {
            int64_t grow = 2 * (int64_t)ctx->pulses_cap_rows;
            if (grow > rows_all + rc) grow = rows_all + rc;
            URH_CHECK(urh_ensure_pulses_keep(ctx, (size_t)(grow > need ? grow : need), (size_t)rows));
        }
        urh_arena_release(ctx, mark);
        int64_t kc = 0;
        URH_CHECK(urh_finish_chunk(ctx, s1 - s0, tol, is_ask, sps, tiles, staging, cap, d_init, chain, s0, n, rows, rc, &kc));
        urh_stream_sample_free(ctx);
        rows += kc;
        return URH_OK;
    }
};

static int stream_check(urh_ctx* ctx, int64_t n, int ring, int mod_type, int dtype, bool iq);
static int psk_stream_check(urh_ctx* ctx, int64_t n, int ring, int dtype) {
    URH_CHECK(stream_check(ctx, n, ring, URH_MOD_PSK, dtype, false));
    if (n <= 2) URH_FAIL(ctx, URH_ERR_INVALID, "streamed PSK demodulation: n > 2");
    if (urh_iq_bytes(dtype) == 0) URH_FAIL(ctx, URH_ERR_DTYPE, "Unsupported dtype");
    return URH_OK;
}

static int stream_check(urh_ctx* ctx, int64_t n, int ring, int mod_type, int dtype, bool iq) {
    if (n <= 0) URH_FAIL(ctx, URH_ERR_INVALID, "streamed call: empty capture");
    if (ring < 2 || ring > URH_STREAM_MAX_RING) URH_FAIL(ctx, URH_ERR_INVALID, "streamed call: ring of %d slots (2..%d)", ring, URH_STREAM_MAX_RING);
    if (iq && (n <= 2 || (mod_type != URH_MOD_ASK && mod_type != URH_MOD_FSK)))
        URH_FAIL(ctx, URH_ERR_INVALID, "streamed demodulation: ASK/FSK and n > 2 (PSK is a serial recurrence)");
    if (iq && urh_iq_bytes(dtype) == 0) URH_FAIL(ctx, URH_ERR_DTYPE, "Unsupported dtype");
    return URH_OK;
}

template <bool DIG>
static int stream_dense_iq(urh_ctx* ctx, int dtype, int mod_type, const char* d_src, int64_t src_slot, int64_t n, const UrhDemodParams& dp,
                           float* qad_global, const UrhClassify& cls, int tol, StreamDigitizer* dz, int64_t s0, int64_t s1, int s,
                           UrhTileStats* ts = nullptr, const UrhFine& fine = UrhFine{}) {
    const int b = urh_iq_bytes(dtype);
    const void* iq = d_src + s * src_slot + URH_STREAM_PAD - s0 * b;
    const int64_t t0 = s0 / URH_TILE, t1 = urh_div_up(s1, URH_TILE);
    UrhTileSummary* tiles = dz ? dz->tiles - t0 : nullptr;
    uint32_t* staging = dz ? dz->staging - t0 * dz->cap : nullptr;
    const int cap = dz ? dz->cap : 0;
    int16_t* init = dz ? dz->d_init : nullptr;
    const int c0 = DIG ? host_classify(0.0f, cls) : 0;
    if (mod_type == URH_MOD_ASK)
        return launch_dense_iq_m<URH_MOD_ASK, DIG>(ctx, dtype, iq, n, dp, qad_global, cls, tol, tiles, staging, cap, init, c0, 0, ts, t0, t1, fine);
    return launch_dense_iq_m<URH_MOD_FSK, DIG>(ctx, dtype, iq, n, dp, qad_global, cls, tol, tiles, staging, cap, init, c0, 0, ts, t0, t1, fine);
}

static int stream_dense_qad(urh_ctx* ctx, const float* x, int64_t s0, int64_t s1, const UrhClassify& cls, StreamDigitizer& dz,
                            const float* d_thr0 = nullptr, const UrhTileStats* ts = nullptr) {
    const int64_t nc = s1 - s0;
    const unsigned grid = (unsigned)urh_div_up(urh_div_up(nc, URH_TILE), URH_WARPS_PER_BLOCK);
    const int vec_in = (((uintptr_t)x % 8) == 0) ? 1 : 0;
    int16_t* init = s0 == 0 ? dz.d_init : nullptr;
    const int c0 = d_thr0 ? 0 : host_classify(0.0f, cls);
    const UrhTileStats* tsc = ts ? ts + s0 / URH_TILE : nullptr;
    if (cls.order == 2)
        URH_LAUNCH(ctx, (k_dense_f32<SrcQad2, float>), grid, URH_WARPS_PER_BLOCK * 32, 0, x, nc, vec_in, cls, dz.tol, dz.tiles, dz.staging,
                   dz.cap, init, c0, d_thr0, tsc);
    else
        URH_LAUNCH(ctx, (k_dense_f32<SrcQad, float>), grid, URH_WARPS_PER_BLOCK * 32, 0, x, nc, vec_in, cls, dz.tol, dz.tiles, dz.staging,
                   dz.cap, init, c0, d_thr0, tsc);
    return URH_OK;
}

struct CenterPlan;
int urh_center_chain(urh_ctx* ctx, const float* d_qad, int64_t n, const UrhTileStats* ts, int64_t max_size, int rank, int world,
                     const UrhFine* fine, CenterPlan** d_plan_out);
int urh_center_plan_result(urh_ctx* ctx, const CenterPlan* plan, const float** d_centerf, const double** d_center, const int** d_state);
int urh_center_plan_certify_stats(urh_ctx* ctx, const CenterPlan* plan, int64_t* h_dst3);

extern "C" int urh_shard_digitize(urh_ctx* ctx, const void* d_iq, int dtype, const float* d_qad_in, int64_t n, int has_halo,
                                  float noise_mag, int mod_type, float center, uint16_t tolerance, uint32_t samples_per_symbol,
                                  uint8_t bits_per_symbol, float center_spacing, float* d_qad_out, int64_t global_offset,
                                  int64_t n_total, int64_t* k) {
    if (!k) return URH_ERR_INVALID;
    *k = 0;
    ctx->pulses_k = 0;
    if (n <= 0) URH_FAIL(ctx, URH_ERR_INVALID, "empty shard");
    if (mod_type != URH_MOD_ASK && mod_type != URH_MOD_FSK) URH_FAIL(ctx, URH_ERR_INVALID, "sharded path: ASK / FSK only");
    if (!d_qad_in && urh_iq_bytes(dtype) == 0) URH_FAIL(ctx, URH_ERR_DTYPE, "Unsupported dtype");
    if (!ctx->nccl_comm) URH_FAIL(ctx, URH_ERR_INVALID, "NCCL communicator not initialised (urh_nccl_init)");
    urh_arena_reset(ctx);
    UrhClassify cls;
    URH_CHECK(fill_classify(ctx, &cls, mod_type, center, bits_per_symbol, center_spacing));
    const int tol = tolerance;
    const int64_t ntiles = urh_div_up(n, URH_TILE);
    const int cap = stage_cap_for(tol);
    UrhTileSummary* tiles;
    uint32_t* staging;
    int16_t* d_init;
    URH_CHECK(urh_arena(ctx, (size_t)ntiles, &tiles));
    URH_CHECK(urh_arena(ctx, (size_t)ntiles * cap, &staging));
    URH_CHECK(urh_arena(ctx, 8, &d_init));
    URH_CUDA(ctx, cudaMemsetAsync(d_init, 0, 16, ctx->stream));
    const int c0 = host_classify(0.0f, cls);
    if (d_qad_in) {
        const int vec_in = (((uintptr_t)d_qad_in % 8) == 0) ? 1 : 0;
        const unsigned grid = (unsigned)urh_div_up(ntiles, URH_WARPS_PER_BLOCK);
        URH_PROF_BEGIN(ctx);
        if (cls.order == 2)
            URH_LAUNCH(ctx, (k_dense_f32<SrcQad2, float>), grid, URH_WARPS_PER_BLOCK * 32, 0, d_qad_in, n, vec_in, cls, tol, tiles, staging, cap,
                       d_init, c0, (const float*)nullptr);
        else
            URH_LAUNCH(ctx, (k_dense_f32<SrcQad, float>), grid, URH_WARPS_PER_BLOCK * 32, 0, d_qad_in, n, vec_in, cls, tol, tiles, staging, cap,
                       d_init, c0, (const float*)nullptr);
        URH_PROF_END(ctx);
    } else {
        const UrhDemodParams dp = make_demod_params(noise_mag, mod_type, dtype);
        if (mod_type == URH_MOD_ASK)
            URH_CHECK((launch_dense_iq_m<URH_MOD_ASK, true>(ctx, dtype, d_iq, n, dp, d_qad_out, cls, tol, tiles, staging, cap, d_init, c0, has_halo)));
        else
            URH_CHECK((launch_dense_iq_m<URH_MOD_FSK, true>(ctx, dtype, d_iq, n, dp, d_qad_out, cls, tol, tiles, staging, cap, d_init, c0, has_halo)));
    }
    return urh_finish_shard(ctx, n, tol, mod_type == URH_MOD_ASK, samples_per_symbol, tiles, staging, cap, d_init, global_offset, n_total, k);
}

struct StreamCenter {
    int ring;
    int64_t chunk_samples;
    const void* h_iq;
    float* h_qad;
    int64_t* kept;
};
static int demod_center_digitize_impl(urh_ctx* ctx, const void* d_iq, int dtype, int64_t n, int has_halo, float noise_mag, int mod_type,
                                      uint16_t tolerance, uint32_t samples_per_symbol, int64_t max_size, float* d_qad_out, bool sharded,
                                      int64_t global_offset, int64_t n_total, double* center, int* center_state, int64_t* k,
                                      const void* h_iq = nullptr, int64_t chunk_samples = 0, const StreamCenter* sc = nullptr) {
    if (!k || !center || !center_state) return URH_ERR_INVALID;
    *k = 0;
    *center = 0.0;
    *center_state = 0;
    ctx->pulses_k = 0;
    if (n <= 2 || (mod_type != URH_MOD_ASK && mod_type != URH_MOD_FSK) || !d_qad_out)
        URH_FAIL(ctx, URH_ERR_INVALID, "demod_center_digitize: ASK/FSK, n > 2 and a qad buffer are required");
    if (urh_iq_bytes(dtype) == 0) URH_FAIL(ctx, URH_ERR_DTYPE, "Unsupported dtype");
    if (sharded && !ctx->nccl_comm) URH_FAIL(ctx, URH_ERR_INVALID, "NCCL communicator not initialised (urh_nccl_init)");
    urh_arena_reset(ctx);
    URH_TL_RESET(ctx);
    URH_TL_MARK(ctx, "step start");
    const UrhDemodParams dp = make_demod_params(noise_mag, mod_type, dtype);
    UrhClassify cls;
    memset(&cls, 0, sizeof(cls));
    const int64_t ntiles = urh_div_up(n, URH_TILE);
    UrhTileStats* ts;
    URH_CHECK(urh_arena(ctx, (size_t)ntiles, &ts));
    const bool no_certify = getenv("URH_B200_CENTER_NO_CERTIFY") != nullptr;
    UrhFine fine = {};
    if (!sharded && !no_certify) {
        fine.slab_tiles = urh_div_up(ntiles, URH_FINE_SLABS);
        if (fine.slab_tiles < URH_WARPS_PER_BLOCK) fine.slab_tiles = URH_WARPS_PER_BLOCK;
        const int64_t nslabs = urh_div_up(ntiles, fine.slab_tiles);
        URH_CHECK(urh_arena(ctx, (size_t)(nslabs * URH_FINE_NB), &fine.gh));
        URH_CUDA(ctx, cudaMemsetAsync(fine.gh, 0, (size_t)(nslabs * URH_FINE_NB) * sizeof(unsigned int), ctx->stream));
        fine.scale = (mod_type == URH_MOD_FSK) ? 512.0f : 4096.0f;
        fine.off = (mod_type == URH_MOD_FSK) ? 2048.0f : 0.0f;
    }
    const int64_t chunk_tiles = (h_iq && chunk_samples > 0) ? (chunk_samples >= URH_TILE ? chunk_samples / URH_TILE : 1) : ntiles;
    const size_t sample_bytes = (size_t)urh_iq_bytes(dtype);
    StreamRing ring;
    int64_t scs = 0;
    if (sc) {
        const StreamSizes z = stream_sizes(n, dtype, tolerance, sc->chunk_samples, sc->ring, URH_STREAM_ENTRY_DEMOD_CENTER_DIGITIZE);
        scs = z.cs;
        URH_CHECK(ring.init(ctx, sc->ring, sc->ring * r256(z.src_slot)));
        const int64_t slot = r256(z.src_slot);
        URH_CHECK(stream_run(ctx, n, scs, ring, (const char*)sc->h_iq, urh_iq_bytes(dtype), true, ring.mem, slot, sc->h_qad, d_qad_out,
                             [&](int64_t, int64_t s0, int64_t s1, int s) {
                                 return stream_dense_iq<false>(ctx, dtype, mod_type, ring.mem, slot, n, dp, d_qad_out, cls, 0, nullptr, s0, s1, s,
                                                               ts, fine);
                             }, true));
    }
    cls.noise_value = urh_noise_value(mod_type);
    cls.order = 2;
    const int tol = tolerance;
    const int cap = stage_cap_for(tol);
    UrhTileSummary* tiles = nullptr;
    uint32_t* staging = nullptr;
    int16_t* d_init = nullptr;
    if (!sc) {
        URH_CHECK(urh_arena(ctx, (size_t)ntiles, &tiles));
        URH_CHECK(urh_arena(ctx, (size_t)ntiles * cap, &staging));
        URH_CHECK(urh_arena(ctx, 8, &d_init));
    }
    const bool speculate = !sharded && !h_iq && !sc && mod_type == URH_MOD_FSK && dtype == URH_DT_F32 &&
                           getenv("URH_B200_NO_SPECULATE") == nullptr;
    UrhSpec spec = {};
    if (speculate) {
        float* tg;
        URH_CHECK(urh_arena(ctx, 1, &tg));
        URH_CHECK(urh_arena(ctx, 1, &spec.redone));
        URH_CHECK(urh_arena(ctx, (size_t)ntiles, &spec.margin));
        spec.tg = tg;
        const char* forced = getenv("URH_B200_SPECULATE_GUESS");
        URH_LAUNCH(ctx, k_speculate_guess, 1, URH_GUESS_THREADS, 0, (const float2*)d_iq, n, dp.noise_sqrd, forced ? 1 : 0,
                   forced ? strtof(forced, nullptr) : 0.0f, tg, spec.redone);
    }
    int chunk_no = 0;
    for (int64_t t0 = 0; t0 < (sc ? 0 : ntiles); t0 += chunk_tiles, chunk_no++) {
        const int64_t t1 = (t0 + chunk_tiles < ntiles) ? t0 + chunk_tiles : ntiles;
        if (h_iq) {
            const int64_t s0 = t0 * URH_TILE, s1 = (t1 * URH_TILE < n) ? t1 * URH_TILE : n;
            cudaEvent_t ev = ctx->ev_copy[chunk_no & 1];
            URH_CUDA(ctx, cudaMemcpyAsync((char*)d_iq + (size_t)s0 * sample_bytes, (const char*)h_iq + (size_t)s0 * sample_bytes,
                                          (size_t)(s1 - s0) * sample_bytes, cudaMemcpyHostToDevice, ctx->copy_stream[0]));
            URH_CUDA(ctx, cudaEventRecord(ev, ctx->copy_stream[0]));
            URH_CUDA(ctx, cudaStreamWaitEvent(ctx->stream, ev, 0));
        }
        if (mod_type == URH_MOD_ASK)
            URH_CHECK((launch_dense_iq_m<URH_MOD_ASK, false>(ctx, dtype, d_iq, n, dp, d_qad_out, cls, 0, nullptr, nullptr, 0, nullptr, 0, has_halo, ts, t0, t1, fine)));
        else
            URH_CHECK((launch_dense_iq_m<URH_MOD_FSK, false>(ctx, dtype, d_iq, n, dp, d_qad_out, cls, tol, tiles, staging, cap, nullptr, 0, has_halo,
                                                             ts, t0, t1, fine, speculate ? &spec : nullptr)));
    }
    CenterPlan* plan = nullptr;
    URH_CHECK(urh_center_chain(ctx, d_qad_out, n, ts, max_size, sharded ? ctx->nccl_rank : 0, sharded ? ctx->nccl_world : 1,
                               fine.gh ? &fine : nullptr, &plan));
    const float* d_centerf;
    const double* d_center;
    const int* d_state;
    urh_center_plan_result(ctx, plan, &d_centerf, &d_center, &d_state);
    int64_t rows = 0;
    if (sc) {
        URH_CUDA(ctx, cudaMemcpyAsync(ctx->h_mail + 40, d_center, sizeof(double), cudaMemcpyDeviceToHost, ctx->stream));
        URH_CUDA(ctx, cudaMemcpyAsync(ctx->h_mail + 41, d_state, sizeof(int), cudaMemcpyDeviceToHost, ctx->stream));
        URH_CHECK(urh_center_plan_certify_stats(ctx, plan, ctx->h_mail + 42));
        URH_CUDA(ctx, cudaMemcpyAsync(ctx->h_mail + 45, (const int64_t*)ctx->center_prefix + ntiles, sizeof(int64_t), cudaMemcpyDeviceToHost,
                                      ctx->stream));
        URH_CUDA(ctx, cudaStreamSynchronize(ctx->stream));
        int st0 = 0;
        memcpy(&st0, ctx->h_mail + 41, sizeof(int));
        if (st0 == 1) {
            StreamDigitizer dz;
            URH_CHECK(dz.init(ctx, n, scs, tol, mod_type == URH_MOD_ASK, samples_per_symbol));
            for (int64_t s0 = 0; s0 < n; s0 += scs) {
                const int64_t s1 = s0 + scs < n ? s0 + scs : n;
                URH_CHECK(stream_dense_qad(ctx, d_qad_out + s0, s0, s1, cls, dz, d_centerf, ts));
                URH_CHECK(dz.finish(ctx, s0, s1));
            }
            rows = dz.rows;
        }
        *sc->kept = ctx->h_mail[45];
    } else {
        URH_CUDA(ctx, cudaMemsetAsync(d_init, 0, 16, ctx->stream));
        const int vec_in = (((uintptr_t)d_qad_out % 8) == 0) ? 1 : 0;
        int64_t grid = urh_div_up(ntiles, URH_WARPS_PER_BLOCK);
        if (speculate) {
            int per_sm = 0;
            URH_CUDA(ctx, cudaOccupancyMaxActiveBlocksPerMultiprocessor(&per_sm, k_dense_f32<SrcQad2, float>, URH_WARPS_PER_BLOCK * 32, 0));
            const int64_t resident = (int64_t)ctx->sm_count * (per_sm > 0 ? per_sm : 1);
            if (grid > resident) grid = resident;
        }
        URH_LAUNCH(ctx, (k_dense_f32<SrcQad2, float>), (unsigned)grid, URH_WARPS_PER_BLOCK * 32, 0,
                   (const float*)d_qad_out, n, vec_in, cls, tol, tiles, staging, cap, d_init, 0, d_centerf, (const UrhTileStats*)ts, spec);
        URH_CUDA(ctx, cudaMemcpyAsync(ctx->h_mail + 40, d_center, sizeof(double), cudaMemcpyDeviceToHost, ctx->stream));
        URH_CUDA(ctx, cudaMemcpyAsync(ctx->h_mail + 41, d_state, sizeof(int), cudaMemcpyDeviceToHost, ctx->stream));
        URH_CHECK(urh_center_plan_certify_stats(ctx, plan, ctx->h_mail + 42));
        ctx->h_mail[46] = 0;
        if (speculate) URH_CUDA(ctx, cudaMemcpyAsync(ctx->h_mail + 46, spec.redone, sizeof(unsigned int), cudaMemcpyDeviceToHost, ctx->stream));
        if (sharded)
            URH_CHECK(urh_finish_shard(ctx, n, tol, mod_type == URH_MOD_ASK, samples_per_symbol, tiles, staging, cap, d_init, global_offset, n_total, &rows));
        else
            URH_CHECK(urh_finish_local(ctx, n, tol, mod_type == URH_MOD_ASK, samples_per_symbol, tiles, staging, cap, d_init, &rows));
    }
    memcpy(center, ctx->h_mail + 40, sizeof(double));
    int st = 0;
    memcpy(&st, ctx->h_mail + 41, sizeof(int));
    *center_state = st;
    ctx->center_cert[0] = ctx->h_mail[42];
    ctx->center_cert[1] = fine.gh ? URH_FINE_NB : 0;
    ctx->center_cert[2] = ctx->h_mail[44];
    const int64_t redone = (spec.hi > spec.lo) ? ctx->h_mail[46] : 0;
    ctx->spec_stats[0] = spec.hi - spec.lo;
    ctx->spec_stats[1] = spec.hi - spec.lo - redone;
    ctx->spec_stats[2] = redone;
    if (st != 1) {
        ctx->pulses_k = 0;
        rows = 0;
    }
    *k = rows;
    return URH_OK;
}

extern "C" int urh_speculate_stats(urh_ctx* ctx, int64_t* h_out3) {
    for (int i = 0; i < 3; i++) h_out3[i] = ctx->spec_stats[i];
    return URH_OK;
}

extern "C" int urh_demod_center_digitize(urh_ctx* ctx, const void* d_iq, int dtype, int64_t n, float noise_mag, int mod_type,
                                         uint16_t tolerance, uint32_t samples_per_symbol, int64_t max_size, float* d_qad_out,
                                         double* center, int* center_state, int64_t* k) {
    return demod_center_digitize_impl(ctx, d_iq, dtype, n, 0, noise_mag, mod_type, tolerance, samples_per_symbol, max_size, d_qad_out, false,
                                      0, n, center, center_state, k);
}

extern "C" int urh_demod_center_digitize_host(urh_ctx* ctx, const void* h_iq, int dtype, int64_t n, float noise_mag, int mod_type,
                                              uint16_t tolerance, uint32_t samples_per_symbol, int64_t max_size, int64_t chunk_samples,
                                              void* d_iq_scratch, float* d_qad_out, double* center, int* center_state, int64_t* k) {
    if (!h_iq || !d_iq_scratch) return URH_ERR_INVALID;
    URH_CUDA(ctx, cudaEventRecord(ctx->ev_comp[0], ctx->stream));
    URH_CUDA(ctx, cudaStreamWaitEvent(ctx->copy_stream[0], ctx->ev_comp[0], 0));
    return demod_center_digitize_impl(ctx, d_iq_scratch, dtype, n, 0, noise_mag, mod_type, tolerance, samples_per_symbol, max_size, d_qad_out,
                                      false, 0, n, center, center_state, k, h_iq, chunk_samples > 0 ? chunk_samples : ((int64_t)1 << 24));
}

extern "C" int urh_shard_demod_center_digitize_host(urh_ctx* ctx, const void* h_iq, int dtype, int64_t n, int has_halo, float noise_mag,
                                                    int mod_type, uint16_t tolerance, uint32_t samples_per_symbol, int64_t max_size,
                                                    int64_t chunk_samples, void* d_iq_scratch, float* d_qad_out, int64_t global_offset,
                                                    int64_t n_total, double* center, int* center_state, int64_t* k) {
    if (!h_iq || !d_iq_scratch) return URH_ERR_INVALID;
    URH_CUDA(ctx, cudaEventRecord(ctx->ev_comp[0], ctx->stream));
    URH_CUDA(ctx, cudaStreamWaitEvent(ctx->copy_stream[0], ctx->ev_comp[0], 0));
    return demod_center_digitize_impl(ctx, d_iq_scratch, dtype, n, has_halo, noise_mag, mod_type, tolerance, samples_per_symbol, max_size,
                                      d_qad_out, true, global_offset, n_total, center, center_state, k, h_iq,
                                      chunk_samples > 0 ? chunk_samples : ((int64_t)1 << 24));
}

extern "C" int urh_shard_demod_center_digitize(urh_ctx* ctx, const void* d_iq, int dtype, int64_t n, int has_halo, float noise_mag,
                                               int mod_type, uint16_t tolerance, uint32_t samples_per_symbol, int64_t max_size,
                                               float* d_qad_out, int64_t global_offset, int64_t n_total, double* center,
                                               int* center_state, int64_t* k) {
    return demod_center_digitize_impl(ctx, d_iq, dtype, n, has_halo, noise_mag, mod_type, tolerance, samples_per_symbol, max_size, d_qad_out,
                                      true, global_offset, n_total, center, center_state, k);
}

extern "C" int urh_afp_demod_stream(urh_ctx* ctx, const void* h_iq, int dtype, int64_t n, float noise_mag, int mod_type, int64_t chunk_samples,
                                    int ring, float* h_qad) {
    if (!h_iq || !h_qad) return URH_ERR_INVALID;
    URH_CHECK(stream_check(ctx, n, ring, mod_type, dtype, true));
    urh_arena_reset(ctx);
    const StreamSizes z = stream_sizes(n, dtype, 0, chunk_samples, ring, URH_STREAM_ENTRY_AFP_DEMOD);
    StreamRing R;
    URH_CHECK(R.init(ctx, ring, z.ring_bytes));
    char* d_src = R.mem;
    float* d_qad = (float*)(R.mem + ring * r256(z.src_slot));
    const UrhDemodParams dp = make_demod_params(noise_mag, mod_type, dtype);
    UrhClassify cls;
    memset(&cls, 0, sizeof(cls));
    return stream_run(ctx, n, z.cs, R, (const char*)h_iq, urh_iq_bytes(dtype), true, d_src, r256(z.src_slot), h_qad, d_qad,
                      [&](int64_t, int64_t s0, int64_t s1, int s) {
                          return stream_dense_iq<false>(ctx, dtype, mod_type, d_src, r256(z.src_slot), n, dp, d_qad + s * z.cs - s0, cls, 0,
                                                        nullptr, s0, s1, s);
                      });
}

extern "C" int urh_grab_pulse_lens_stream(urh_ctx* ctx, const float* qad, int qad_on_device, int64_t n, float center, uint16_t tolerance,
                                          int mod_type, uint32_t samples_per_symbol, uint8_t bits_per_symbol, float center_spacing,
                                          int64_t chunk_samples, int ring, int64_t* k) {
    if (!k || !qad) return URH_ERR_INVALID;
    *k = 0;
    ctx->pulses_k = 0;
    URH_CHECK(stream_check(ctx, n, ring, mod_type, 0, false));
    urh_arena_reset(ctx);
    UrhClassify cls;
    URH_CHECK(fill_classify(ctx, &cls, mod_type, center, bits_per_symbol, center_spacing));
    const StreamSizes z = stream_sizes(n, 0, tolerance, chunk_samples, ring,
                                       URH_STREAM_ENTRY_GRAB_PULSE_LENS | (qad_on_device ? URH_STREAM_QAD_ON_DEVICE : 0));
    StreamRing R;
    URH_CHECK(R.init(ctx, ring, z.ring_bytes));
    StreamDigitizer dz;
    URH_CHECK(dz.init(ctx, n, z.cs, tolerance, mod_type == URH_MOD_ASK, samples_per_symbol));
    char* d_src = R.mem;
    URH_CHECK(stream_run(ctx, n, z.cs, R, qad_on_device ? nullptr : (const char*)qad, 4, false, d_src, r256(z.src_slot), nullptr, nullptr,
                         [&](int64_t, int64_t s0, int64_t s1, int s) {
                             const float* x = qad_on_device ? qad + s0 : (const float*)(d_src + s * r256(z.src_slot) + URH_STREAM_PAD);
                             URH_CHECK(stream_dense_qad(ctx, x, s0, s1, cls, dz));
                             return dz.finish(ctx, s0, s1);
                         }));
    *k = dz.rows;
    return URH_OK;
}

extern "C" int urh_demod_digitize_stream(urh_ctx* ctx, const void* h_iq, int dtype, int64_t n, float noise_mag, int mod_type, float center,
                                         uint16_t tolerance, uint32_t samples_per_symbol, uint8_t bits_per_symbol, float center_spacing,
                                         int64_t chunk_samples, int ring, float* h_qad_out, int64_t* k) {
    if (!k || !h_iq) return URH_ERR_INVALID;
    *k = 0;
    ctx->pulses_k = 0;
    URH_CHECK(stream_check(ctx, n, ring, mod_type, dtype, true));
    urh_arena_reset(ctx);
    UrhClassify cls;
    URH_CHECK(fill_classify(ctx, &cls, mod_type, center, bits_per_symbol, center_spacing));
    const UrhDemodParams dp = make_demod_params(noise_mag, mod_type, dtype);
    const StreamSizes z = stream_sizes(n, dtype, tolerance, chunk_samples, ring,
                                       URH_STREAM_ENTRY_DEMOD_DIGITIZE | (h_qad_out ? URH_STREAM_QAD_OUT : 0));
    StreamRing R;
    URH_CHECK(R.init(ctx, ring, z.ring_bytes));
    StreamDigitizer dz;
    URH_CHECK(dz.init(ctx, n, z.cs, tolerance, mod_type == URH_MOD_ASK, samples_per_symbol));
    char* d_src = R.mem;
    float* d_qad = h_qad_out ? (float*)(R.mem + ring * r256(z.src_slot)) : nullptr;
    URH_CHECK(stream_run(ctx, n, z.cs, R, (const char*)h_iq, urh_iq_bytes(dtype), true, d_src, r256(z.src_slot), h_qad_out, d_qad,
                         [&](int64_t, int64_t s0, int64_t s1, int s) {
                             URH_CHECK(stream_dense_iq<true>(ctx, dtype, mod_type, d_src, r256(z.src_slot), n, dp,
                                                             d_qad ? d_qad + s * z.cs - s0 : nullptr, cls, tolerance, &dz, s0, s1, s));
                             return dz.finish(ctx, s0, s1);
                         }));
    *k = dz.rows;
    return URH_OK;
}

extern "C" int urh_demod_center_digitize_stream(urh_ctx* ctx, const void* h_iq, int dtype, int64_t n, float noise_mag, int mod_type,
                                                uint16_t tolerance, uint32_t samples_per_symbol, int64_t max_size, int64_t chunk_samples,
                                                int ring, float* d_qad_out, float* h_qad_out, double* center, int* center_state,
                                                int64_t* kept, int64_t* k) {
    if (!h_iq || !d_qad_out || !kept) return URH_ERR_INVALID;
    URH_CHECK(stream_check(ctx, n, ring, mod_type, dtype, true));
    StreamCenter sc;
    sc.ring = ring; sc.chunk_samples = chunk_samples; sc.h_iq = h_iq; sc.h_qad = h_qad_out; sc.kept = kept;
    return demod_center_digitize_impl(ctx, nullptr, dtype, n, 0, noise_mag, mod_type, tolerance, samples_per_symbol, max_size, d_qad_out,
                                      false, 0, n, center, center_state, k, nullptr, 0, &sc);
}

extern "C" int urh_afp_demod_psk_stream(urh_ctx* ctx, const void* h_iq, int dtype, int64_t n, float noise_mag, int mod_order,
                                        float costas_loop_bandwidth, int64_t chunk_samples, int ring, float* h_qad) {
    if (!h_iq || !h_qad) return URH_ERR_INVALID;
    URH_CHECK(psk_stream_check(ctx, n, ring, dtype));
    urh_arena_reset(ctx);
    const StreamSizes z = stream_sizes(n, dtype, 0, chunk_samples, ring, URH_STREAM_ENTRY_AFP_DEMOD | psk_entry_flags(mod_order));
    StreamRing R;
    URH_CHECK(R.init(ctx, ring, z.ring_bytes));
    const int64_t slot = r256(z.src_slot);
    char* d_src = R.mem;
    float* d_qad = (float*)(R.mem + ring * slot);
    const UrhDemodParams dp = make_demod_params(noise_mag, URH_MOD_PSK, dtype);
// ... 187 lines not shown
```

urh_b200/csrc/finish.cu:

```cuda
#include "sparse.cuh"
#include "tilescan.cuh"

#include <limits.h>

#define CLS_NONE INT_MIN

struct __align__(16) CandAgg {
    int64_t cnt;
    int32_t last_cls;
    int32_t pad;
};
struct CandOp {
    __device__ __forceinline__ CandAgg operator()(const CandAgg& a, const CandAgg& b) const {
        CandAgg r;
        r.cnt = a.cnt + b.cnt;
        r.last_cls = (b.last_cls != CLS_NONE) ? b.last_cls : a.last_cls;
        r.pad = 0;
        return r;
    }
};
struct __align__(16) FireAgg {
    int64_t fired;
    int64_t last_pos;
};
struct FireOp {
    __device__ __forceinline__ FireAgg operator()(const FireAgg& a, const FireAgg& b) const {
        FireAgg r;
        r.fired = a.fired + b.fired;
        r.last_pos = (b.last_pos >= 0) ? b.last_pos : a.last_pos;
        return r;
    }
};

struct ScanRunCarry {
    const UrhTileSummary* tiles;
    int64_t n;
    RunCarry* carry;
    __device__ __forceinline__ RunCarry load(int64_t t) const {
        const int64_t rem = n - t * URH_TILE;
        const int tile_len = rem < URH_TILE ? (int)rem : URH_TILE;
        const UrhTileSummary s = tiles[t];
        RunCarry r;
        r.len = s.tail_len;
        r.cls = s.last_cls;
        r.flags = (s.head_len == tile_len) ? 1 : 0;
        return r;
    }
    __device__ __forceinline__ void post(int64_t t, const RunCarry& excl, const RunCarry&) const { carry[t] = excl; }
};

struct __align__(16) TileFire {
    int32_t first_cls;
    int32_t first_rel;
    int32_t fired;
    int32_t last_rel;
};
struct ScanCandidates {
    const UrhTileSummary* tiles;
    const uint32_t* staging;
    int stage_cap;
    const RunCarry* carry;
    const RunCarry* xcarry;
    int tol;
    int32_t* head_rel;
    int32_t* prev_cls;
    TileFire* fire;
    __device__ __forceinline__ CandAgg load(int64_t t) const {
        const UrhTileSummary s = tiles[t];
        RunCarry c = carry[t];
        if (xcarry) c = RunCarryOp()(*xcarry, c);
        int64_t start_len = 0;
        if (!(c.flags & 2) && c.cls == s.first_cls) start_len = c.len;
        int32_t rel = -1;
        if (start_len <= tol && (int64_t)tol < start_len + s.head_len) rel = (int32_t)(tol - start_len);
        head_rel[t] = rel;
        TileFire f;
        f.first_cls = CLS_NONE; f.first_rel = -1; f.fired = 0; f.last_rel = -1;
        int prev = CLS_NONE;
        if (rel >= 0) {
            prev = s.first_cls;
            f.first_cls = prev;
            f.first_rel = rel;
        }
        const uint32_t* st = staging + t * (int64_t)stage_cap;
        for (int j = 0; j < s.ncand; j += 4) {
            uint32_t w[4];
#pragma unroll
            for (int u = 0; u < 4; u++) w[u] = (j + u < s.ncand) ? st[j + u] : 0u;
#pragma unroll
            for (int u = 0; u < 4; u++) {
                if (j + u < s.ncand) {
                    const int cl = (int)(w[u] & 0xffffu) - 1;
                    const int p = (int)(w[u] >> 16);
                    if (prev == CLS_NONE) {
                        f.first_cls = cl;
                        f.first_rel = p;
                    } else if (cl != prev) {
                        f.fired++;
                        f.last_rel = p;
                    }
                    prev = cl;
                }
            }
        }
        fire[t] = f;
        CandAgg r;
        r.cnt = (int64_t)s.ncand + (rel >= 0 ? 1 : 0);
        r.last_cls = prev;
        r.pad = 0;
        return r;
    }
    __device__ __forceinline__ void post(int64_t t, const CandAgg& excl, const CandAgg&) const { prev_cls[t] = excl.last_cls; }
};

struct ScanFirings {
    const TileFire* fire;
    const int32_t* prev_cls;
    const int16_t* d_prev0;
    int64_t global_offset;
    int64_t* row_off;
    int64_t* prev_fired;
    __device__ __forceinline__ FireAgg load(int64_t t) const {
        const TileFire f = fire[t];
        int prev = prev_cls[t];
        if (prev == CLS_NONE) prev = *d_prev0;
        FireAgg r;
        r.fired = f.fired;
        int32_t last = f.last_rel;
        if (f.first_cls != CLS_NONE && f.first_cls != prev) {
            r.fired++;
            if (last < 0) last = f.first_rel;
        }
        r.last_pos = (last >= 0) ? t * URH_TILE + global_offset + last : -1;
        return r;
    }
    __device__ __forceinline__ void post(int64_t t, const FireAgg& excl, const FireAgg&) const {
        row_off[t] = excl.fired;
        prev_fired[t] = excl.last_pos;
    }
};

constexpr int FIN_TILES = 32;
constexpr int FIN_BATCH = 8;

struct FinRows {
    int64_t* out;
    int64_t cap_rows;
    int tol;
    int is_ask;
    int64_t sps;
};

struct FinWalk {
    int prev;
    int64_t pp;
    int64_t idx;
};

__device__ __forceinline__ void fin_row(const FinRows& R, int64_t idx, int64_t p, int64_t pp, int prev) {
    const int64_t rec = (pp >= 0) ? (p - pp) : (p + 1 - R.tol);
    int64_t st = prev;
    if (R.is_ask && st == -1 && rec < R.sps) st = 0;
    if (idx < R.cap_rows) *((longlong2*)R.out + idx) = make_longlong2(st, rec);
}

__device__ __forceinline__ void fin_chunk(FinWalk& W, uint32_t w, int cnt, int lane, int64_t base, const FinRows& R) {
    const int c = (int)(w & 0xffffu) - 1;
    const int rel = (int)(w >> 16);
    int pc = __shfl_up_sync(URH_FULL_MASK, c, 1);
    if (lane == 0) pc = W.prev;
    const bool fire = lane < cnt && c != pc;
    const unsigned fm = __ballot_sync(URH_FULL_MASK, fire);
    const unsigned lower = fm & ((1u << lane) - 1u);
    const int before = __shfl_sync(URH_FULL_MASK, rel, lower ? 31 - __clz(lower) : 0);
    if (fire) fin_row(R, W.idx + __popc(lower), base + rel, lower ? base + before : W.pp, pc);
    if (fm) W.pp = base + __shfl_sync(URH_FULL_MASK, rel, 31 - __clz(fm));
    W.idx += __popc(fm);
    if (cnt > 0) W.prev = __shfl_sync(URH_FULL_MASK, c, cnt - 1);
}

__global__ void __launch_bounds__(256) k_finish_rows(const UrhTileSummary* __restrict__ tiles, const uint32_t* __restrict__ staging,
                                                    int stage_cap, const int32_t* __restrict__ head_rel, const int32_t* __restrict__ prev_cls,
                                                    const int16_t* __restrict__ d_prev0, const int64_t* __restrict__ row_off,
                                                    const int64_t* __restrict__ prev_fired, const int64_t* __restrict__ d_xprev_fired,
                                                    int64_t ntiles, int64_t global_offset, int64_t n_total, int tol, int is_ask, int64_t sps,
                                                    int emit_tail, int64_t row_base, int64_t* __restrict__ out, int64_t cap_rows,
                                                    int64_t* __restrict__ d_out) {
    const int64_t t0 = ((int64_t)blockIdx.x * blockDim.x + threadIdx.x) / 32 * FIN_TILES;
    if (t0 >= ntiles) return;
    const int lane = threadIdx.x & 31;
    FinRows R;
    R.out = out; R.cap_rows = cap_rows; R.tol = tol; R.is_ask = is_ask; R.sps = sps;
    const int64_t tl = t0 + lane;
    int l_first = 0, l_ncand = 0, l_rel = -1, l_prev = 0;
    int64_t l_idx = 0, l_pp = -1;
    if (tl < ntiles) {
        const UrhTileSummary s = tiles[tl];
        l_first = s.first_cls;
        l_ncand = s.ncand;
        l_rel = head_rel[tl];
        l_prev = prev_cls[tl];
        if (l_prev == CLS_NONE) l_prev = *d_prev0;
        l_idx = row_off[tl];
        l_pp = prev_fired[tl];
        if (l_pp < 0) l_pp = *d_xprev_fired;
    }
    for (int j0 = 0; j0 < FIN_TILES && t0 + j0 < ntiles; j0 += FIN_BATCH) {
        uint32_t w0[FIN_BATCH];
#pragma unroll
        for (int u = 0; u < FIN_BATCH; u++) {
            const int nc = __shfl_sync(URH_FULL_MASK, l_ncand, j0 + u);
            w0[u] = (lane < nc) ? __ldg(staging + (t0 + j0 + u) * (int64_t)stage_cap + lane) : 0u;
        }
#pragma unroll
        for (int u = 0; u < FIN_BATCH; u++) {
            const int j = j0 + u;
            const int64_t t = t0 + j;
            if (t >= ntiles) break;
            const int64_t base = t * URH_TILE + global_offset;
            const int ncand = __shfl_sync(URH_FULL_MASK, l_ncand, j);
            const int rel = __shfl_sync(URH_FULL_MASK, l_rel, j);
            FinWalk W;
            W.prev = __shfl_sync(URH_FULL_MASK, l_prev, j);
            W.pp = __shfl_sync(URH_FULL_MASK, l_pp, j);
            W.idx = __shfl_sync(URH_FULL_MASK, l_idx, j);
            if (rel >= 0) {
                const int c = __shfl_sync(URH_FULL_MASK, l_first, j);
                if (c != W.prev) {
                    if (lane == 0) fin_row(R, W.idx, base + rel, W.pp, W.prev);
                    W.idx++;
                    W.pp = base + rel;
                }
                W.prev = c;
            }
            const uint32_t* st = staging + t * (int64_t)stage_cap;
            for (int k = 0; k < ncand; k += 32) {
                const uint32_t w = (k == 0) ? w0[u] : ((k + lane < ncand) ? __ldg(st + k + lane) : 0u);
                fin_chunk(W, w, min(32, ncand - k), lane, base, R);
            }
            if (t == ntiles - 1 && lane == 0) {
                int64_t idx = W.idx;
                const int64_t fired = idx;
                if (emit_tail && (is_ask || row_base + fired < n_total)) {
                    if (idx < cap_rows) *((longlong2*)out + idx) = make_longlong2(W.prev, (W.pp >= 0) ? (n_total - 1 - W.pp) : (n_total - tol));
                    idx++;
                }
                d_out[0] = idx;
                d_out[1] = fired;
            }
        }
    }
}

struct ScanMergeRows {
    const int64_t* raw;
    int64_t rows;
    int64_t n_total;
    int has_tail;
    int64_t* out;
    int64_t* d_k;
    const int64_t* prev_last;
    int64_t row_base;
    __device__ __forceinline__ int64_t load(int64_t r) const {
        if (r == 0) return (prev_last && raw[0] == *prev_last) ? 0 : 1;
        return raw[2 * r] != raw[2 * r - 2] ? 1 : 0;
    }
    __device__ __forceinline__ void post(int64_t r, const int64_t& excl, const int64_t& head) const {
        const bool is_tail = has_tail && r == rows - 1;
        if (is_tail && row_base + excl >= n_total) {
            *d_k = excl;
            return;
        }
        const int64_t o = excl + head - 1;
        if (head) out[2 * o] = raw[2 * r];
        atomicAdd((unsigned long long*)&out[2 * o + 1], (unsigned long long)raw[2 * r + 1]);
        if (r == rows - 1) *d_k = o + 1;
    }
};
struct AddI64 {
    __device__ __forceinline__ int64_t operator()(int64_t a, int64_t b) const { return a + b; }
};

__global__ void k_pack_stage1(const int16_t* __restrict__ d_init, const RunCarry* __restrict__ total, int64_t* __restrict__ msg) {
    memcpy(msg, total, sizeof(RunCarry));
    msg[2] = *d_init;
    msg[3] = 0;
}
__global__ void k_fold_carry(const int64_t* __restrict__ all, int rank, RunCarry* __restrict__ xcarry) {
    RunCarry acc;
    acc.len = 0; acc.cls = 0; acc.flags = 2 | 1;
    for (int q = 0; q < rank; q++) {
        RunCarry c;
        memcpy(&c, all + 4 * q, sizeof(c));
        acc = RunCarryOp()(acc, c);
    }
    if (rank == 0) acc.flags = 2;
    else acc.flags &= ~1;
    *xcarry = acc;
}
__global__ void k_fold_prev_cls(const int64_t* __restrict__ all, int rank, const int64_t* __restrict__ stage1, int16_t* __restrict__ prev0) {
    int v = (int)stage1[2];
    for (int q = 0; q < rank; q++) {
        CandAgg c;
        memcpy(&c, all + 2 * q, sizeof(c));
        if (c.last_cls != CLS_NONE) v = c.last_cls;
    }
    *prev0 = (int16_t)v;
}
__global__ void k_fold_prev_fired(const int64_t* __restrict__ all, int rank, int64_t* __restrict__ xprev) {
    int64_t v = -1;
    for (int q = 0; q < rank; q++) {
        FireAgg c;
        memcpy(&c, all + 2 * q, sizeof(c));
        if (c.last_pos >= 0) v = c.last_pos;
    }
    *xprev = v;
}

__global__ void k_chain_start(const int16_t* __restrict__ d_init, UrhChain* __restrict__ chain) {
    chain->run.len = 0; chain->run.cls = 0; chain->run.flags = 2 | 1;
    chain->prev_fired = -1;
    chain->last_state = INT64_MIN;
    chain->prev_cls = *d_init;
}
__global__ void k_chain_advance(UrhChain* __restrict__ chain, const RunCarry* __restrict__ tot_run, const CandAgg* __restrict__ tot_cand,
                                const FireAgg* __restrict__ tot_fire) {
    chain->run = RunCarryOp()(chain->run, *tot_run);
    if (tot_cand->last_cls != CLS_NONE) chain->prev_cls = (int16_t)tot_cand->last_cls;
    if (tot_fire->last_pos >= 0) chain->prev_fired = tot_fire->last_pos;
}
__global__ void k_chain_last_row(UrhChain* __restrict__ chain, const int64_t* __restrict__ table, int64_t rows) {
    if (rows > 0) chain->last_state = table[2 * (rows - 1)];
}

int urh_coll_allgather(urh_ctx* ctx, const void* d_send, void* d_recv, size_t bytes_per_rank);
extern "C" int urh_p2p_check(urh_ctx* ctx);

struct FinishShard {
    int rank, world;
    int64_t global_offset;
    int64_t n_total;
    int emit_tail;
    UrhChain* chain;
    int64_t row_base, rows_cap;
};

static int finish_tiles(urh_ctx* ctx, int64_t n, int tol, bool is_ask, uint32_t sps, const UrhTileSummary* tiles, const uint32_t* staging,
                        int stage_cap, const int16_t* d_init, const FinishShard& sh, int64_t* k) {
    const int64_t ntiles = urh_div_up(n, URH_TILE);
    const bool sharded = sh.world > 1;
    UrhChain* chain = sh.chain;
    RunCarry* carry;
    int32_t *head_rel, *prev_cls;
    int64_t *row_off, *prev_fired, *d_small;
    URH_CHECK(urh_arena(ctx, (size_t)ntiles, &carry));
    URH_CHECK(urh_arena(ctx, (size_t)ntiles, &head_rel));
    URH_CHECK(urh_arena(ctx, (size_t)ntiles, &prev_cls));
    URH_CHECK(urh_arena(ctx, (size_t)ntiles, &row_off));
    URH_CHECK(urh_arena(ctx, (size_t)ntiles, &prev_fired));
    TileFire* fire;
    URH_CHECK(urh_arena(ctx, (size_t)ntiles, &fire));
    URH_CHECK(urh_arena(ctx, (size_t)(32 + 8 * (sharded ? sh.world : 0)), &d_small));
    URH_CUDA(ctx, cudaMemsetAsync(d_small, 0xff, 4 * sizeof(int64_t), ctx->stream));
    RunCarry* d_tot_run = (RunCarry*)(d_small + 4);
    CandAgg* d_tot_cand = (CandAgg*)(d_small + 6);
    FireAgg* d_tot_fire = (FireAgg*)(d_small + 8);
    RunCarry* d_xcarry = (RunCarry*)(d_small + 10);
    int16_t* d_prev0 = (int16_t*)(d_small + 12);
    int64_t* d_xprev = d_small + 13;
    int64_t* d_msg1 = d_small + 16;
    int64_t* d_all1 = d_small + 32;
    int64_t* d_all2 = d_all1 + 4 * (sharded ? sh.world : 0);
    int64_t* d_all3 = d_all2 + 2 * (sharded ? sh.world : 0);

    if (chain && sh.global_offset == 0) URH_LAUNCH(ctx, k_chain_start, 1, 1, 0, d_init, chain);
    RunCarry rc_ident;
    rc_ident.len = 0; rc_ident.cls = 0; rc_ident.flags = 2 | 1;
    ScanRunCarry fa;
    fa.tiles = tiles; fa.n = n; fa.carry = carry;
    URH_CHECK((urhts::scan<RunCarry, RunCarryOp, ScanRunCarry>(ctx, ntiles, rc_ident, RunCarryOp(), fa, d_tot_run)));
    if (sharded) {
        URH_LAUNCH(ctx, k_pack_stage1, 1, 1, 0, d_init, (const RunCarry*)d_tot_run, d_msg1);
        URH_TL_MARK(ctx, "x4 run carry: enter");
        URH_CHECK(urh_coll_allgather(ctx, d_msg1, d_all1, 4 * sizeof(int64_t)));
        URH_TL_MARK(ctx, "x4 run carry: done");
        URH_LAUNCH(ctx, k_fold_carry, 1, 1, 0, (const int64_t*)d_all1, sh.rank, d_xcarry);
    }
    ScanCandidates fb;
    fb.tiles = tiles; fb.staging = staging; fb.stage_cap = stage_cap; fb.carry = carry;
    fb.xcarry = sharded ? d_xcarry : (chain ? &chain->run : nullptr);
    fb.tol = tol; fb.head_rel = head_rel; fb.prev_cls = prev_cls; fb.fire = fire;
    CandAgg ca_ident;
    ca_ident.cnt = 0; ca_ident.last_cls = CLS_NONE; ca_ident.pad = 0;
    URH_CHECK((urhts::scan<CandAgg, CandOp, ScanCandidates, 4>(ctx, ntiles, ca_ident, CandOp(), fb, d_tot_cand)));
    const int16_t* prev0 = chain ? &chain->prev_cls : d_init;
    if (sharded) {
        URH_TL_MARK(ctx, "x5 candidates: enter");
        URH_CHECK(urh_coll_allgather(ctx, d_tot_cand, d_all2, sizeof(CandAgg)));
        URH_TL_MARK(ctx, "x5 candidates: done");
        URH_LAUNCH(ctx, k_fold_prev_cls, 1, 1, 0, (const int64_t*)d_all2, sh.rank, (const int64_t*)d_all1, d_prev0);
        prev0 = d_prev0;
    }
    ScanFirings fc;
    fc.fire = fire; fc.prev_cls = prev_cls; fc.d_prev0 = prev0; fc.global_offset = sh.global_offset; fc.row_off = row_off;
    fc.prev_fired = prev_fired;
    FireAgg fi_ident;
    fi_ident.fired = 0; fi_ident.last_pos = -1;
    URH_CHECK((urhts::scan<FireAgg, FireOp, ScanFirings>(ctx, ntiles, fi_ident, FireOp(), fc, d_tot_fire)));
    const int64_t* xprev = chain ? &chain->prev_fired : d_small + 2;
    if (sharded) {
        URH_TL_MARK(ctx, "x6 firings: enter");
        URH_CHECK(urh_coll_allgather(ctx, d_tot_fire, d_all3, sizeof(FireAgg)));
        URH_TL_MARK(ctx, "x6 firings: done");
        URH_LAUNCH(ctx, k_fold_prev_fired, 1, 1, 0, (const int64_t*)d_all3, sh.rank, d_xprev);
        xprev = d_xprev;
    }

    int64_t cap_rows = (int64_t)ctx->pulses_cap_rows;
    const int64_t guess = n / 64 + 1024;
    if (!chain && cap_rows < guess) {
        URH_CHECK(urh_ensure_pulses(ctx, (size_t)guess));
        cap_rows = (int64_t)ctx->pulses_cap_rows;
    }
    const int64_t row_base = chain ? sh.row_base : 0;
    int64_t* raw = ctx->pulses + 2 * row_base;
    int64_t raw_cap = chain ? sh.rows_cap : cap_rows;
    if (is_ask) URH_CHECK(urh_arena(ctx, (size_t)raw_cap * 2, &raw));
    int64_t got[2] = {0, 0};
    for (int attempt = 0; attempt < 2; attempt++) {
        URH_LAUNCH(ctx, k_finish_rows, (unsigned)urh_div_up(ntiles, 8 * FIN_TILES), 256, 0, tiles, staging, stage_cap, (const int32_t*)head_rel,
                   (const int32_t*)prev_cls, prev0, (const int64_t*)row_off, (const int64_t*)prev_fired, xprev, ntiles, sh.global_offset,
                   sh.n_total, tol, is_ask ? 1 : 0, (int64_t)sps, sh.emit_tail, row_base, raw, raw_cap, d_small);
        if (sharded && attempt == 0) URH_TL_MARK(ctx, "rows written");
        URH_CHECK(urh_read_i64(ctx, d_small, 2, got));
        if (sharded) URH_CHECK(urh_p2p_check(ctx));
        if (got[0] <= raw_cap) break;
        if (attempt == 1 || chain) URH_FAIL(ctx, URH_ERR_CUDA, "finish_tiles: row buffer overflow after regrowth");
        if (is_ask) {
            URH_CHECK(urh_arena(ctx, (size_t)got[0] * 2, &raw));
            raw_cap = got[0];
        } else {
            URH_CHECK(urh_ensure_pulses(ctx, (size_t)got[0]));
            raw = ctx->pulses;
            raw_cap = (int64_t)ctx->pulses_cap_rows;
        }
    }
    if (chain) URH_LAUNCH(ctx, k_chain_advance, 1, 1, 0, chain, (const RunCarry*)d_tot_run, (const CandAgg*)d_tot_cand, (const FireAgg*)d_tot_fire);
    int64_t K = got[0];
    if (is_ask && K > 0) {
        if (!chain) URH_CHECK(urh_ensure_pulses(ctx, (size_t)K));
        int64_t* out = ctx->pulses + 2 * row_base;
        URH_CUDA(ctx, cudaMemsetAsync(out, 0, (size_t)K * 2 * sizeof(int64_t), ctx->stream));
        ScanMergeRows fm;
        fm.raw = raw; fm.rows = K; fm.n_total = sh.n_total; fm.has_tail = (sh.emit_tail && K > got[1]) ? 1 : 0; fm.out = out;
        fm.d_k = d_small;
        fm.prev_last = (chain && row_base > 0) ? &chain->last_state : nullptr;
        fm.row_base = row_base;
        URH_CHECK((urhts::scan<int64_t, AddI64, ScanMergeRows>(ctx, K, (int64_t)0, AddI64(), fm, (int64_t*)nullptr)));
        URH_CHECK(urh_read_i64(ctx, d_small, 1, &K));
        if (chain) URH_LAUNCH(ctx, k_chain_last_row, 1, 1, 0, chain, (const int64_t*)ctx->pulses, row_base + K);
    }
    ctx->pulses_k = row_base + K;
    *k = K;
    return URH_OK;
}

int urh_finish_chunk(urh_ctx* ctx, int64_t n, int tol, bool is_ask, uint32_t sps, const UrhTileSummary* tiles, const uint32_t* staging,
                     int stage_cap, const int16_t* d_init, UrhChain* chain, int64_t global_offset, int64_t n_total, int64_t row_base,
                     int64_t rows_cap, int64_t* k) {
    FinishShard sh;
    sh.rank = 0; sh.world = 1; sh.global_offset = global_offset; sh.n_total = n_total;
    sh.emit_tail = (global_offset + n == n_total) ? 1 : 0;
    sh.chain = chain; sh.row_base = row_base; sh.rows_cap = rows_cap;
    return finish_tiles(ctx, n, tol, is_ask, sps, tiles, staging, stage_cap, d_init, sh, k);
}

int urh_finish_local(urh_ctx* ctx, int64_t n, int tol, bool is_ask, uint32_t sps, const UrhTileSummary* tiles, const uint32_t* staging,
                     int stage_cap, const int16_t* d_init, int64_t* k) {
    FinishShard sh;
    sh.rank = 0; sh.world = 1; sh.global_offset = 0; sh.n_total = n; sh.emit_tail = 1;
    sh.chain = nullptr; sh.row_base = 0; sh.rows_cap = 0;
    return finish_tiles(ctx, n, tol, is_ask, sps, tiles, staging, stage_cap, d_init, sh, k);
}

int urh_finish_shard(urh_ctx* ctx, int64_t n, int tol, bool is_ask, uint32_t sps, const UrhTileSummary* tiles, const uint32_t* staging,
                     int stage_cap, const int16_t* d_init, int64_t global_offset, int64_t n_total, int64_t* k) {
    FinishShard sh;
    sh.rank = ctx->nccl_rank; sh.world = ctx->nccl_world; sh.global_offset = global_offset; sh.n_total = n_total;
    sh.emit_tail = (ctx->nccl_rank == ctx->nccl_world - 1) ? 1 : 0;
    sh.chain = nullptr; sh.row_base = 0; sh.rows_cap = 0;
    return finish_tiles(ctx, n, tol, is_ask, sps, tiles, staging, stage_cap, d_init, sh, k);
}
```

urh_b200/csrc/tilescan.cuh:

```cuda
#pragma once
#include "common.cuh"

namespace urhts {

constexpr int BLOCK = 256;
constexpr int SLOT = 32;

struct Ws {
    unsigned long long* counter;
    uint32_t* status;
    char* agg;
    char* pre;
    unsigned long long base;
    uint32_t epoch;
};

template <typename T>
union Words {
    T v;
    uint32_t w[sizeof(T) / 4];
    __device__ __forceinline__ Words() {}
};

template <typename T>
__device__ __forceinline__ T shfl_up_t(const T& x, int d) {
    static_assert(sizeof(T) % 4 == 0 && sizeof(T) <= SLOT, "scan element: multiple of 4 bytes, at most SLOT");
    Words<T> a, r;
    a.v = x;
#pragma unroll
    for (int k = 0; k < (int)(sizeof(T) / 4); k++) r.w[k] = __shfl_up_sync(URH_FULL_MASK, a.w[k], d);
    return r.v;
}
template <typename T>
__device__ __forceinline__ T shfl_t(const T& x, int src) {
    Words<T> a, r;
    a.v = x;
#pragma unroll
    for (int k = 0; k < (int)(sizeof(T) / 4); k++) r.w[k] = __shfl_sync(URH_FULL_MASK, a.w[k], src);
    return r.v;
}
template <typename T>
__device__ __forceinline__ void publish(char* slots, int64_t b, const T& x) {
    Words<T> a;
    a.v = x;
    uint32_t* p = (uint32_t*)(slots + b * SLOT);
#pragma unroll
    for (int k = 0; k < (int)(sizeof(T) / 4); k++) __stcg(p + k, a.w[k]);
}
template <typename T>
__device__ __forceinline__ T fetch(const char* slots, int64_t b) {
    Words<T> a;
    const uint32_t* p = (const uint32_t*)(slots + b * SLOT);
#pragma unroll
    for (int k = 0; k < (int)(sizeof(T) / 4); k++) a.w[k] = __ldcg(p + k);
    return a.v;
}
__device__ __forceinline__ uint32_t ld_status(const uint32_t* p) {
    uint32_t v;
    asm volatile("ld.volatile.global.u32 %0, [%1];" : "=r"(v) : "l"(p));
    return v;
}
__device__ __forceinline__ void st_status(uint32_t* p, uint32_t v) {
    asm volatile("st.volatile.global.u32 [%0], %1;" ::"l"(p), "r"(v) : "memory");
}

template <typename T, typename Op, typename F, int ITEMS>
__global__ void __launch_bounds__(BLOCK) k_scan(int64_t n, T identity, Op op, F f, Ws ws, T* __restrict__ total_out) {
    constexpr int CHUNK = BLOCK * ITEMS;
    __shared__ unsigned long long s_bid;
    __shared__ T s_warp[BLOCK / 32];
    __shared__ T s_block_excl;
    if (threadIdx.x == 0) s_bid = atomicAdd(ws.counter, 1ull) - ws.base;
    __syncthreads();
    const int64_t bid = (int64_t)s_bid;
    const int lane = threadIdx.x & 31, warp = threadIdx.x >> 5;
    const int64_t first = bid * CHUNK + (int64_t)threadIdx.x * ITEMS;
    T v[ITEMS];
    T acc = identity;
#pragma unroll
    for (int i = 0; i < ITEMS; i++) {
        v[i] = (first + i < n) ? f.load(first + i) : identity;
        acc = op(acc, v[i]);
    }
    T incl = acc;
#pragma unroll
    for (int off = 1; off < 32; off <<= 1) {
        const T o = shfl_up_t(incl, off);
        if (lane >= off) incl = op(o, incl);
    }
    T lane_excl = shfl_up_t(incl, 1);
    if (lane == 0) lane_excl = identity;
    if (lane == 31) s_warp[warp] = incl;
    __syncthreads();
    if (warp == 0) {
        constexpr int NW = BLOCK / 32;
        T wi = (lane < NW) ? s_warp[lane] : identity;
#pragma unroll
        for (int off = 1; off < NW; off <<= 1) {
            const T o = shfl_up_t(wi, off);
            if (lane >= off) wi = op(o, wi);
        }
        T wex = shfl_up_t(wi, 1);
        if (lane == 0) wex = identity;
        const T block_agg = shfl_t(wi, NW - 1);
        T excl = identity;
        if (bid > 0) {
            if (lane == 0) {
                publish(ws.agg, bid, block_agg);
                __threadfence();
                st_status(ws.status + bid, (ws.epoch << 2) | 1u);
            }
            int64_t look = bid - 1;
            bool done = false;
            while (!done) {
                const int64_t p = look - lane;
                uint32_t st;
                bool ready;
                do {
                    st = (p >= 0) ? ld_status(ws.status + p) : ((ws.epoch << 2) | 2u);
                    ready = (st >> 2) == ws.epoch && (st & 3u) != 0u;
                } while (!__all_sync(URH_FULL_MASK, ready));
                __threadfence();
                const bool is_pre = (st & 3u) == 2u;
                T val = identity;
                if (p >= 0) val = is_pre ? fetch<T>(ws.pre, p) : fetch<T>(ws.agg, p);
                const uint32_t pm = __ballot_sync(URH_FULL_MASK, is_pre);
                const int far = pm ? (__ffs(pm) - 1) : 31;
                T window = shfl_t(val, far);
                for (int j = far - 1; j >= 0; j--) window = op(window, shfl_t(val, j));
                excl = op(window, excl);
                done = pm != 0u;
                look -= 32;
            }
        }
        if (lane == 0) {
            const T inclusive = op(excl, block_agg);
            publish(ws.pre, bid, inclusive);
            __threadfence();
            st_status(ws.status + bid, (ws.epoch << 2) | 2u);
            s_block_excl = excl;
            if (total_out && (bid + 1) * (int64_t)CHUNK >= n) *total_out = inclusive;
        }
        if (lane < NW) s_warp[lane] = wex;
    }
    __syncthreads();
    T run = op(s_block_excl, op(s_warp[warp], lane_excl));
#pragma unroll
    for (int i = 0; i < ITEMS; i++) {
        if (first + i < n) {
            f.post(first + i, run, v[i]);
            run = op(run, v[i]);
        }
    }
}

int prepare(urh_ctx* ctx, int64_t nblocks, Ws* out);

template <typename T, typename Op, typename F, int ITEMS = 16>
static inline int scan(urh_ctx* ctx, int64_t n, T identity, Op op, F f, T* d_total) {
    if (n <= 0) return URH_OK;
    const int64_t nb = urh_div_up(n, (int64_t)BLOCK * ITEMS);
    Ws ws;
    URH_CHECK(prepare(ctx, nb, &ws));
    URH_LAUNCH(ctx, (k_scan<T, Op, F, ITEMS>), (unsigned)nb, BLOCK, 0, n, identity, op, f, ws, d_total);
    return URH_OK;
}

}
```

Before: 213,900.

## Fold small setup kernels, memsets and D2H copies into fewer launches

Merges the ranks kernel into the window kernel and the pick kernel with a step-record writer. Memsets are folded into existing kernels (guess kernel zeroing, scan post writing -1s), and the slab-sum reduction moves from the single-block certify kernel into the multi-block window-ends kernel. Scattered small device-to-host copies are replaced by one record read at the existing sync point. The goal is fewer launches, less serialized single-block work and fewer tiny transfers, at the cost of more complex kernels and a new side stream that may be unused.

Result: faster. 219,300, median of 6 (+2.5%).

```diff
diff --git a/urh_b200/csrc/center.cu b/urh_b200/csrc/center.cu
--- a/urh_b200/csrc/center.cu
+++ b/urh_b200/csrc/center.cu
@@ -520,7 +520,6 @@
     float scale;
     int fast;
     int state;
-    unsigned int ticket;
     int certified;
     long long straddle;
     long long pad;
@@ -536,7 +535,8 @@
     __device__ __forceinline__ int64_t operator()(int64_t a, int64_t b) const { return a + b; }
 };
 
-__global__ void k_center_ranks(const int64_t* __restrict__ counts, int rank, int world, int64_t max_size, CenterPlan* __restrict__ plan) {
+__device__ __forceinline__ void cen_ranks(const int64_t* __restrict__ counts, int rank, int world, int64_t max_size, long long* lr,
+                                          CenterPlan* __restrict__ plan) {
     long long total = 0, offset = 0;
     for (int q = 0; q < world; q++) {
         if (q < rank) offset += counts[q];
@@ -545,12 +545,13 @@
     const long long kept = counts[rank];
     long long r0 = (long long)(0.05 * (double)total), r1 = (long long)(0.95 * (double)total);
     if (max_size >= 0 && r1 - r0 > max_size) r1 = r0 + max_size;
-    plan->total = total; plan->offset = offset; plan->r0 = r0; plan->r1 = r1;
     long long a = r0 - offset, b = r1 - offset;
     a = a < 0 ? 0 : (a > kept ? kept : a);
     b = b < 0 ? 0 : (b > kept ? kept : b);
+    lr[0] = a; lr[1] = b;
+    if (!plan) return;
+    plan->total = total; plan->offset = offset; plan->r0 = r0; plan->r1 = r1;
     plan->lr0 = a; plan->lr1 = b;
-    plan->ticket = 0u;
     plan->state = 1;
     plan->certified = 0;
     plan->straddle = 0;
@@ -566,12 +567,15 @@
 }
 
 __global__ void __launch_bounds__(256) k_center_window(const float* __restrict__ x, int64_t n, const UrhTileStats* __restrict__ ts,
-                                                      const int64_t* __restrict__ prefix, int64_t ntiles, CenterPlan* __restrict__ plan,
+                                                      const int64_t* __restrict__ prefix, int64_t ntiles, const int64_t* __restrict__ counts,
+                                                      int rank, int world, int64_t max_size, urhts::Ws ws, CenterPlan* __restrict__ plan,
                                                       CenStats* __restrict__ partial) {
-    __shared__ long long s_win[4];
+    __shared__ long long s_win[4], s_lr[2];
     __shared__ int s_pre[256];
     __shared__ bool s_last;
-    const long long r0 = plan->lr0, r1 = plan->lr1;
+    if (threadIdx.x == 0) cen_ranks(counts, rank, world, max_size, s_lr, blockIdx.x == 0 ? plan : nullptr);
+    __syncthreads();
+    const long long r0 = s_lr[0], r1 = s_lr[1];
     if (threadIdx.x == 0) {
         long long w0 = -1, w1 = -1, w2 = -1, w3 = -1;
         if (r1 > r0) {
@@ -623,7 +627,7 @@
     }
     __threadfence();
     __syncthreads();
-    if (threadIdx.x == 0) s_last = atomicAdd(&plan->ticket, 1u) == gridDim.x - 1;
+    if (threadIdx.x == 0) s_last = urhts::arrives_last(ws);
     __syncthreads();
     if (!s_last) return;
     __threadfence();
@@ -725,7 +729,8 @@
 __global__ void __launch_bounds__(256) k_hist_window_ends_dev(const float* __restrict__ x, int64_t n, const int64_t* __restrict__ prefix,
                                                              const CenterPlan* __restrict__ plan, const float* __restrict__ g_fe,
                                                              unsigned long long* __restrict__ hist, unsigned long long* __restrict__ xhist,
-                                                             int64_t slab_tiles) {
+                                                             int64_t slab_tiles, const unsigned int* __restrict__ gh,
+                                                             unsigned long long* __restrict__ slab_sum) {
     if (plan->state != 1) return;
     if (blockIdx.x < 2) {
         hist_window_ends_body(x, n, prefix, (const int64_t*)plan->win, plan->lr0, plan->lr1, g_fe, plan->scale, (int)plan->nbins, hist, xhist);
@@ -734,6 +739,13 @@
     const int64_t w0 = plan->win[0], w1 = plan->win[1];
     int64_t sf, se;
     cen_full_slabs(w0, w1, slab_tiles, &sf, &se);
+    const int64_t bucket = (int64_t)(blockIdx.x - 2) * blockDim.x + threadIdx.x;
+    if (bucket < URH_FINE_NB) {
+        unsigned long long v = 0;
+#pragma unroll 8
+        for (int64_t sl = sf; sl < se; sl++) v += gh[sl * URH_FINE_NB + bucket];
+        slab_sum[bucket] = v;
+    }
     int64_t a_end = w1, b_begin = w1;
     if (sf < se) { a_end = sf * slab_tiles; b_begin = se * slab_tiles; }
     const int blk = blockIdx.x - 2, nblk = gridDim.x - 2, nbins = (int)plan->nbins;
@@ -753,7 +765,8 @@
 
 #define CERT_THREADS 512
 __global__ void __launch_bounds__(CERT_THREADS) k_center_certify(const UrhFine fine, CenterPlan* __restrict__ plan, const float* __restrict__ fe,
-                                                                 const unsigned long long* __restrict__ xhist, unsigned long long* __restrict__ lo,
+                                                                 const unsigned long long* __restrict__ xhist,
+                                                                 const unsigned long long* __restrict__ slab_sum, unsigned long long* __restrict__ lo,
                                                                  unsigned long long* __restrict__ hi) {
     __shared__ unsigned long long s_ge[URH_FINE_NB + 1];
     __shared__ unsigned long long s_part[CERT_THREADS];
@@ -763,15 +776,11 @@
     if (plan->state != 1) return;
     const int tid = threadIdx.x;
     constexpr int PER = URH_FINE_NB / CERT_THREADS;
-    int64_t sf, se;
-    cen_full_slabs(plan->win[0], plan->win[1], fine.slab_tiles, &sf, &se);
     unsigned long long b[PER], tot = 0;
 #pragma unroll
     for (int j = 0; j < PER; j++) {
-        unsigned long long v = 0;
-        for (int64_t sl = sf; sl < se; sl++) v += fine.gh[sl * URH_FINE_NB + tid * PER + j];
-        b[j] = v;
-        tot += v;
+        b[j] = slab_sum[tid * PER + j];
+        tot += b[j];
     }
     s_part[tid] = tot;
     if (tid < 3) s_key[tid] = 0ull;
@@ -847,11 +856,10 @@
     plan->certified = 1;
 }
 
-__global__ void __launch_bounds__(256) k_center_pick(const unsigned long long* __restrict__ y, CenterPlan* __restrict__ plan) {
+__device__ __forceinline__ void cen_pick(const unsigned long long* __restrict__ y, CenterPlan* __restrict__ plan) {
     __shared__ unsigned long long s_best[256];
     __shared__ int s_idx[256];
     __shared__ int s_cnt[256];
-    if (plan->state != 1 || plan->certified) return;
     const int nbins = (int)plan->nbins;
     int window = (int)(0.05 * (double)nbins) + 1;
     if (window < 2) window = 2;
@@ -937,13 +945,24 @@
     (void)top_val;
 }
 
+__global__ void __launch_bounds__(256) k_center_pick(const unsigned long long* __restrict__ y, CenterPlan* __restrict__ plan,
+                                                    UrhStepRecord* __restrict__ rec) {
+    if (plan->state == 1 && !plan->certified) cen_pick(y, plan);
+    if (threadIdx.x != 0) return;
+    rec->center = plan->center;
+    rec->state = plan->state;
+    rec->certified = plan->certified;
+    rec->straddle = plan->straddle;
+    rec->redone = 0u;
+}
+
 int urh_coll_allgather(urh_ctx* ctx, const void* d_send, void* d_recv, size_t bytes_per_rank);
 bool urh_p2p_usable(urh_ctx* ctx, size_t bytes_per_rank);
 extern "C" int urh_p2p_allreduce_u64_dev(urh_ctx* ctx, const void* d_in, void* d_out, const int64_t* d_count, int max_words);
 extern "C" int urh_nccl_allreduce_i64(urh_ctx* ctx, int64_t* d_buf, int64_t count, int op);
 
 int urh_center_chain(urh_ctx* ctx, const float* d_qad, int64_t n, const UrhTileStats* ts, int64_t max_size, int rank, int world,
-                     const UrhFine* fine, CenterPlan** d_plan_out) {
+                     const UrhFine* fine, UrhStepRecord* rec, CenterPlan** d_plan_out) {
     const int64_t ntiles = urh_div_up(n, URH_TILE);
     int64_t* prefix;
     CenterPlan* plan;
@@ -952,7 +971,7 @@
     unsigned long long* hist;
     int64_t* d_counts;
     CenStats* d_parts;
-    unsigned long long *xhist = nullptr, *cert_lo = nullptr, *cert_hi = nullptr;
+    unsigned long long *xhist = nullptr, *slab_sum = nullptr, *cert_lo = nullptr, *cert_hi = nullptr;
     const int nb = ctx->sm_count * 2;
     URH_CHECK(urh_arena(ctx, (size_t)ntiles + 1, &prefix));
     URH_CHECK(urh_arena(ctx, 1, &plan));
@@ -963,6 +982,7 @@
     URH_CHECK(urh_arena(ctx, (size_t)world, &d_parts));
     if (fine) {
         URH_CHECK(urh_arena(ctx, (size_t)CEN_MAX_BINS, &xhist));
+        URH_CHECK(urh_arena(ctx, (size_t)URH_FINE_NB, &slab_sum));
         URH_CHECK(urh_arena(ctx, (size_t)CEN_MAX_BINS, &cert_lo));
         URH_CHECK(urh_arena(ctx, (size_t)CEN_MAX_BINS, &cert_hi));
     }
@@ -976,8 +996,9 @@
         URH_TL_MARK(ctx, "x1 kept counts: done");
         counts = d_counts;
     }
-    URH_LAUNCH(ctx, k_center_ranks, 1, 1, 0, counts, rank, world, max_size, plan);
-    URH_LAUNCH(ctx, k_center_window, nb, 256, 0, d_qad, n, ts, (const int64_t*)prefix, ntiles, plan, partial);
+    urhts::Ws ws;
+    URH_CHECK(urhts::prepare(ctx, nb, &ws));
+    URH_LAUNCH(ctx, k_center_window, nb, 256, 0, d_qad, n, ts, (const int64_t*)prefix, ntiles, counts, rank, world, max_size, ws, plan, partial);
     const CenStats* parts = &plan->local;
     if (world > 1) {
         URH_TL_MARK(ctx, "x2 window partials: enter");
@@ -989,8 +1010,11 @@
     const size_t dyn = (size_t)CEN_MAX_BINS * 4 + (size_t)(CEN_MAX_BINS + 3) * 4;
     const unsigned gs = (unsigned)min(urh_div_up(ntiles, 8), (int64_t)ctx->sm_count * 8);
     URH_LAUNCH(ctx, k_hist_window_ends_dev, fine ? 2 + ctx->sm_count * 4 : 2, 256, fine ? dyn : 0, d_qad, n, (const int64_t*)prefix,
-               (const CenterPlan*)plan, (const float*)fe, hist, xhist, fine ? fine->slab_tiles : (int64_t)1);
-    if (fine) URH_LAUNCH(ctx, k_center_certify, 1, CERT_THREADS, 0, *fine, plan, (const float*)fe, (const unsigned long long*)xhist, cert_lo, cert_hi);
+               (const CenterPlan*)plan, (const float*)fe, hist, xhist, fine ? fine->slab_tiles : (int64_t)1,
+               fine ? (const unsigned int*)fine->gh : nullptr, slab_sum);
+    if (fine)
+        URH_LAUNCH(ctx, k_center_certify, 1, CERT_THREADS, 0, *fine, plan, (const float*)fe, (const unsigned long long*)xhist,
+                   (const unsigned long long*)slab_sum, cert_lo, cert_hi);
     URH_LAUNCH(ctx, (k_hist_interior_dev<true>), gs, 256, dyn, d_qad, n, (const CenterPlan*)plan, (const float*)fe, hist, (const int64_t*)prefix);
     URH_LAUNCH(ctx, (k_hist_interior_dev<false>), gs, 256, dyn, d_qad, n, (const CenterPlan*)plan, (const float*)fe, hist, (const int64_t*)prefix);
     const unsigned long long* hist_all = hist;
@@ -1006,7 +1030,7 @@
         }
     }
     if (world > 1) URH_TL_MARK(ctx, "x3 histogram sum: done");
-    URH_LAUNCH(ctx, k_center_pick, 1, 256, 0, hist_all, plan);
+    URH_LAUNCH(ctx, k_center_pick, 1, 256, 0, hist_all, plan, rec);
     ctx->center_prefix = prefix;
     ctx->center_ts = ts;
     ctx->center_n = n;
@@ -1015,13 +1039,6 @@
     return URH_OK;
 }
 
-int urh_center_plan_certify_stats(urh_ctx* ctx, const CenterPlan* plan, int64_t* h_dst3) {
-    h_dst3[0] = h_dst3[1] = h_dst3[2] = 0;
-    URH_CUDA(ctx, cudaMemcpyAsync(h_dst3, &plan->certified, sizeof(int), cudaMemcpyDeviceToHost, ctx->stream));
-    URH_CUDA(ctx, cudaMemcpyAsync(h_dst3 + 2, &plan->straddle, sizeof(long long), cudaMemcpyDeviceToHost, ctx->stream));
-    return URH_OK;
-}
-
 extern "C" int urh_center_certify_stats(urh_ctx* ctx, int64_t* h_out3) {
     for (int i = 0; i < 3; i++) h_out3[i] = ctx->center_cert[i];
     return URH_OK;
diff --git a/urh_b200/csrc/common.cuh b/urh_b200/csrc/common.cuh
--- a/urh_b200/csrc/common.cuh
+++ b/urh_b200/csrc/common.cuh
@@ -20,6 +20,8 @@
     int sm_count;
     cudaStream_t stream;
     cudaStream_t copy_stream[2];
+    cudaStream_t side_stream;
+    cudaEvent_t ev_fork, ev_join;
     cudaEvent_t ev_start, ev_stop;
     cudaEvent_t ev_copy[2], ev_comp[2];
     cudaEvent_t ev_k0, ev_k1;
@@ -108,12 +110,13 @@
         return (code);                                            \
     } while (0)
 
-#define URH_LAUNCH(ctx, kernel, grid, block, smem, ...)                                   \
+#define URH_LAUNCH_ON(ctx, strm, kernel, grid, block, smem, ...)                          \
     do {                                                                                  \
-        kernel<<<(grid), (block), (smem), (ctx)->stream>>>(__VA_ARGS__);                  \
+        kernel<<<(grid), (block), (smem), (strm)>>>(__VA_ARGS__);                         \
         (ctx)->launches++;                                                                \
         URH_CUDA(ctx, cudaGetLastError());                                                \
     } while (0)
+#define URH_LAUNCH(ctx, kernel, grid, block, smem, ...) URH_LAUNCH_ON(ctx, (ctx)->stream, kernel, grid, block, smem, __VA_ARGS__)
 
 #define URH_TL_MARK(ctx, label) do { if ((ctx)->profiling >= 2 && (ctx)->tl_ready && (ctx)->tl_count < 32) { \
         (ctx)->tl_name[(ctx)->tl_count] = (label); cudaEventRecord((ctx)->tl_ev[(ctx)->tl_count++], (ctx)->stream); } } while (0)
@@ -158,6 +161,15 @@
 
 int urh_read_i64(urh_ctx* ctx, const int64_t* d_src, int count, int64_t* h_out);
 
+struct UrhStepRecord {
+    long long rows, fired;
+    double center;
+    int state, certified;
+    long long straddle;
+    unsigned int redone;
+    unsigned int pad;
+};
+
 __host__ __device__ static inline int64_t urh_div_up(int64_t a, int64_t b) { return (a + b - 1) / b; }
 
 static inline int urh_iq_bytes(int dtype) {
diff --git a/urh_b200/csrc/context.cu b/urh_b200/csrc/context.cu
--- a/urh_b200/csrc/context.cu
+++ b/urh_b200/csrc/context.cu
@@ -69,6 +69,11 @@
     bool ok = cudaStreamCreateWithFlags(&ctx->stream, cudaStreamNonBlocking) == cudaSuccess;
     ok = ok && cudaStreamCreateWithFlags(&ctx->copy_stream[0], cudaStreamNonBlocking) == cudaSuccess;
     ok = ok && cudaStreamCreateWithFlags(&ctx->copy_stream[1], cudaStreamNonBlocking) == cudaSuccess;
+    int pri_low = 0, pri_high = 0;
+    ok = ok && cudaDeviceGetStreamPriorityRange(&pri_low, &pri_high) == cudaSuccess;
+    ok = ok && cudaStreamCreateWithPriority(&ctx->side_stream, cudaStreamNonBlocking, pri_high) == cudaSuccess;
+    ok = ok && cudaEventCreateWithFlags(&ctx->ev_fork, cudaEventDisableTiming) == cudaSuccess;
+    ok = ok && cudaEventCreateWithFlags(&ctx->ev_join, cudaEventDisableTiming) == cudaSuccess;
     ok = ok && cudaEventCreate(&ctx->ev_start) == cudaSuccess && cudaEventCreate(&ctx->ev_stop) == cudaSuccess;
     for (int i = 0; i < 2 && ok; i++) {
         ok = ok && cudaEventCreateWithFlags(&ctx->ev_copy[i], cudaEventDisableTiming) == cudaSuccess;
@@ -110,6 +115,9 @@
         cudaEventDestroy(ctx->ev_comp[i]);
         cudaStreamDestroy(ctx->copy_stream[i]);
     }
+    cudaEventDestroy(ctx->ev_fork);
+    cudaEventDestroy(ctx->ev_join);
+    cudaStreamDestroy(ctx->side_stream);
     cudaStreamDestroy(ctx->stream);
     delete ctx;
 }
diff --git a/urh_b200/csrc/digitize.cu b/urh_b200/csrc/digitize.cu
--- a/urh_b200/csrc/digitize.cu
+++ b/urh_b200/csrc/digitize.cu
@@ -7,6 +7,7 @@
 #include "fsk_fast.cuh"
 #include "dense_f32.cuh"
 #include "stream_ring.cuh"
+#include "tilescan.cuh"
 
 #include <math.h>
 #include <stdlib.h>
@@ -164,47 +165,71 @@
 
 #define URH_GUESS_SAMPLES 16384
 #define URH_GUESS_BINS 128
-#define URH_GUESS_THREADS 1024
+#define URH_GUESS_THREADS 256
+#define URH_GUESS_BLOCKS (URH_GUESS_SAMPLES / URH_GUESS_THREADS)
 __global__ void __launch_bounds__(URH_GUESS_THREADS) k_speculate_guess(const float2* __restrict__ iq, int64_t n, float noise_sqrd, int forced,
-                                                                      float forced_tg, float* __restrict__ d_tg, unsigned int* __restrict__ redone) {
-    constexpr int PER = URH_GUESS_SAMPLES / URH_GUESS_THREADS;
+                                                                      float forced_tg, float* __restrict__ d_tg, float* __restrict__ gv,
+                                                                      float2* __restrict__ gmm, urhts::Ws ws, uint4* __restrict__ zero,
+                                                                      int64_t zero_n) {
     __shared__ unsigned int s_hist[URH_GUESS_BINS];
-    __shared__ float s_mn[32], s_mx[32];
+    __shared__ float s_mn[URH_GUESS_THREADS / 32], s_mx[URH_GUESS_THREADS / 32];
+    __shared__ bool s_last;
+    for (int64_t w = (int64_t)blockIdx.x * URH_GUESS_THREADS + threadIdx.x; w < zero_n; w += (int64_t)gridDim.x * URH_GUESS_THREADS)
+        zero[w] = make_uint4(0u, 0u, 0u, 0u);
     if (forced) {
-        if (threadIdx.x == 0) { *d_tg = forced_tg; *redone = 0u; }
+        if (threadIdx.x == 0 && urhts::arrives_last(ws)) *d_tg = forced_tg;
         return;
     }
-    for (int b = threadIdx.x; b < URH_GUESS_BINS; b += blockDim.x) s_hist[b] = 0u;
-    float v[PER];
+    auto fold = [&](float& mn, float& mx) {
+        for (int off = 16; off > 0; off >>= 1) {
+            mn = fminf(mn, __shfl_xor_sync(URH_FULL_MASK, mn, off));
+            mx = fmaxf(mx, __shfl_xor_sync(URH_FULL_MASK, mx, off));
+        }
+        if ((threadIdx.x & 31) == 0) { s_mn[threadIdx.x >> 5] = mn; s_mx[threadIdx.x >> 5] = mx; }
+        __syncthreads();
+        mn = INFINITY; mx = -INFINITY;
+        for (int w = 0; w < URH_GUESS_THREADS / 32; w++) { mn = fminf(mn, s_mn[w]); mx = fmaxf(mx, s_mx[w]); }
+    };
     float mn = INFINITY, mx = -INFINITY;
-#pragma unroll
-    for (int k = 0; k < PER; k++) {
-        const int64_t i = 1 + (int64_t)(k * URH_GUESS_THREADS + threadIdx.x) * (n - 1) / URH_GUESS_SAMPLES;
+    {
+        const int j = blockIdx.x * URH_GUESS_THREADS + threadIdx.x;
+        const int64_t i = 1 + (int64_t)j * (n - 1) / URH_GUESS_SAMPLES;
         const float2 p = iq[i - 1], c = iq[i];
-        v[k] = NAN;
+        float v = NAN;
         if (!(c.x * c.x + c.y * c.y <= noise_sqrd)) {
-            v[k] = atan2f(p.x * c.y - p.y * c.x, p.x * c.x + p.y * c.y);
-            mn = fminf(mn, v[k]);
-            mx = fmaxf(mx, v[k]);
-        }
-    }
-    for (int off = 16; off > 0; off >>= 1) {
-        mn = fminf(mn, __shfl_xor_sync(URH_FULL_MASK, mn, off));
-        mx = fmaxf(mx, __shfl_xor_sync(URH_FULL_MASK, mx, off));
-    }
-    if ((threadIdx.x & 31) == 0) { s_mn[threadIdx.x >> 5] = mn; s_mx[threadIdx.x >> 5] = mx; }
+            v = atan2f(p.x * c.y - p.y * c.x, p.x * c.x + p.y * c.y);
+            mn = fminf(mn, v);
+            mx = fmaxf(mx, v);
+        }
+        gv[j] = v;
+    }
+    fold(mn, mx);
+    if (threadIdx.x == 0) {
+        gmm[blockIdx.x] = make_float2(mn, mx);
+        __threadfence();
+        s_last = urhts::arrives_last(ws);
+    }
     __syncthreads();
+    if (!s_last) return;
+    __threadfence();
+    for (int b = threadIdx.x; b < URH_GUESS_BINS; b += URH_GUESS_THREADS) s_hist[b] = 0u;
     mn = INFINITY; mx = -INFINITY;
-    for (int w = 0; w < URH_GUESS_THREADS / 32; w++) { mn = fminf(mn, s_mn[w]); mx = fmaxf(mx, s_mx[w]); }
+    for (int b = threadIdx.x; b < URH_GUESS_BLOCKS; b += URH_GUESS_THREADS) {
+        const float2 m = __ldcg(gmm + b);
+        mn = fminf(mn, m.x);
+        mx = fmaxf(mx, m.y);
+    }
+    __syncthreads();
+    fold(mn, mx);
     const float width = (mx - mn) / URH_GUESS_BINS;
     if (width > 0.0f) {
-#pragma unroll
-        for (int k = 0; k < PER; k++)
-            if (!isnan(v[k])) atomicAdd(&s_hist[min((int)((v[k] - mn) / width), URH_GUESS_BINS - 1)], 1u);
+        for (int j = threadIdx.x; j < URH_GUESS_SAMPLES; j += URH_GUESS_THREADS) {
+            const float v = __ldcg(gv + j);
+            if (!isnan(v)) atomicAdd(&s_hist[min((int)((v - mn) / width), URH_GUESS_BINS - 1)], 1u);
+        }
     }
     __syncthreads();
     if (threadIdx.x != 0) return;
-    *redone = 0u;
     if (!(mn <= mx)) { *d_tg = 0.0f; return; }
     if (!(width > 0.0f)) { *d_tg = mn; return; }
     constexpr int WINDOW = (int)(0.05 * URH_GUESS_BINS) + 1;
@@ -278,14 +303,14 @@
     const int vec_in = iq_vec_aligned(d_iq, DT) ? 1 : 0;
     const int vec_out = (d_qad && ((uintptr_t)d_qad % 8) == 0) ? 1 : 0;
     const int threads = URH_WARPS_PER_BLOCK * 32;
-    auto generic = [&](int64_t begin, int64_t end) -> int {
+    auto generic = [&](int64_t begin, int64_t end, cudaStream_t strm) -> int {
         begin = begin < tile_lo ? tile_lo : begin;
         end = end > tile_hi ? tile_hi : end;
         const int64_t count = end - begin;
         if (count <= 0) return URH_OK;
-        URH_LAUNCH(ctx, (k_dense_iq<DT, MOD, DIG>), (unsigned)urh_div_up(count, URH_WARPS_PER_BLOCK), threads, fine_smem, d_iq, n, dp,
-                   d_qad, vec_in, vec_out, cls, tol, tiles, staging, stage_cap, init_cls, cls_of_zero, begin, count, has_halo,
-                   tile_stats, fine);
+        URH_LAUNCH_ON(ctx, strm, (k_dense_iq<DT, MOD, DIG>), (unsigned)urh_div_up(count, URH_WARPS_PER_BLOCK), threads, fine_smem, d_iq, n,
+                      dp, d_qad, vec_in, vec_out, cls, tol, tiles, staging, stage_cap, init_cls, cls_of_zero, begin, count, has_halo,
+                      tile_stats, fine);
         return URH_OK;
     };
     const int64_t nfull = n / URH_TILE;
@@ -293,6 +318,11 @@
     URH_PROF_BEGIN(ctx);
     if (fast) {
         const int64_t fb = tile_lo > 1 ? tile_lo : 1, fe = tile_hi < nfull ? tile_hi : nfull;
+        URH_CUDA(ctx, cudaEventRecord(ctx->ev_fork, ctx->stream));
+        URH_CUDA(ctx, cudaStreamWaitEvent(ctx->side_stream, ctx->ev_fork, 0));
+        URH_CHECK(generic(0, 1, ctx->side_stream));
+        URH_CHECK(generic(nfull, ntiles, ctx->side_stream));
+        URH_CUDA(ctx, cudaEventRecord(ctx->ev_join, ctx->side_stream));
         if (fe > fb) {
             const unsigned grid = (unsigned)urh_div_up(fe - fb, URH_WARPS_PER_BLOCK);
             static const bool fifo = getenv("URH_B200_FSK_NO_FIFO") == nullptr;
@@ -325,10 +355,9 @@
                                 tiles, staging, stage_cap, fb, fe - fb, nullptr, UrhFine{});
             }
         }
-        URH_CHECK(generic(0, 1));
-        URH_CHECK(generic(nfull, ntiles));
+        URH_CUDA(ctx, cudaStreamWaitEvent(ctx->stream, ctx->ev_join, 0));
     } else {
-        URH_CHECK(generic(0, ntiles));
+        URH_CHECK(generic(0, ntiles, ctx->stream));
     }
     URH_PROF_END(ctx);
     return URH_OK;
@@ -410,9 +439,11 @@
 }
 
 int urh_finish_local(urh_ctx* ctx, int64_t n, int tol, bool is_ask, uint32_t sps, const UrhTileSummary* tiles, const uint32_t* staging,
-                     int stage_cap, const int16_t* d_init, int64_t* k);
+                     int stage_cap, const int16_t* d_init, int64_t* k, UrhStepRecord* rec = nullptr,
+                     UrhStepRecord* h_rec = nullptr);
 int urh_finish_shard(urh_ctx* ctx, int64_t n, int tol, bool is_ask, uint32_t sps, const UrhTileSummary* tiles, const uint32_t* staging,
-                     int stage_cap, const int16_t* d_init, int64_t global_offset, int64_t n_total, int64_t* k);
+                     int stage_cap, const int16_t* d_init, int64_t global_offset, int64_t n_total, int64_t* k, UrhStepRecord* rec = nullptr,
+                     UrhStepRecord* h_rec = nullptr);
 
 static int digitize_finish(urh_ctx* ctx, int64_t n, int tol, bool is_ask, uint32_t sps, UrhTileSummary* tiles,
                            uint32_t* staging, int stage_cap, int16_t* d_init, int64_t* k) {
@@ -802,9 +833,8 @@
 
 struct CenterPlan;
 int urh_center_chain(urh_ctx* ctx, const float* d_qad, int64_t n, const UrhTileStats* ts, int64_t max_size, int rank, int world,
-                     const UrhFine* fine, CenterPlan** d_plan_out);
+                     const UrhFine* fine, UrhStepRecord* rec, CenterPlan** d_plan_out);
 int urh_center_plan_result(urh_ctx* ctx, const CenterPlan* plan, const float** d_centerf, const double** d_center, const int** d_state);
-int urh_center_plan_certify_stats(urh_ctx* ctx, const CenterPlan* plan, int64_t* h_dst3);
 
 extern "C" int urh_shard_digitize(urh_ctx* ctx, const void* d_iq, int dtype, const float* d_qad_in, int64_t n, int has_halo,
                                   float noise_mag, int mod_type, float center, uint16_t tolerance, uint32_t samples_per_symbol,
@@ -881,14 +911,20 @@
     const int64_t ntiles = urh_div_up(n, URH_TILE);
     UrhTileStats* ts;
     URH_CHECK(urh_arena(ctx, (size_t)ntiles, &ts));
+    UrhStepRecord* rec;
+    URH_CHECK(urh_arena(ctx, 1, &rec));
+    UrhStepRecord h_rec = {};
+    const bool speculate = !sharded && !h_iq && !sc && mod_type == URH_MOD_FSK && dtype == URH_DT_F32 &&
+                           getenv("URH_B200_NO_SPECULATE") == nullptr;
     const bool no_certify = getenv("URH_B200_CENTER_NO_CERTIFY") != nullptr;
     UrhFine fine = {};
+    int64_t fine_words = 0;
     if (!sharded && !no_certify) {
         fine.slab_tiles = urh_div_up(ntiles, URH_FINE_SLABS);
         if (fine.slab_tiles < URH_WARPS_PER_BLOCK) fine.slab_tiles = URH_WARPS_PER_BLOCK;
-        const int64_t nslabs = urh_div_up(ntiles, fine.slab_tiles);
-        URH_CHECK(urh_arena(ctx, (size_t)(nslabs * URH_FINE_NB), &fine.gh));
-        URH_CUDA(ctx, cudaMemsetAsync(fine.gh, 0, (size_t)(nslabs * URH_FINE_NB) * sizeof(unsigned int), ctx->stream));
+        fine_words = urh_div_up(ntiles, fine.slab_tiles) * URH_FINE_NB;
+        URH_CHECK(urh_arena(ctx, (size_t)fine_words, &fine.gh));
+        if (!speculate) URH_CUDA(ctx, cudaMemsetAsync(fine.gh, 0, (size_t)fine_words * sizeof(unsigned int), ctx->stream));
         fine.scale = (mod_type == URH_MOD_FSK) ? 512.0f : 4096.0f;
         fine.off = (mod_type == URH_MOD_FSK) ? 2048.0f : 0.0f;
     }
@@ -919,18 +955,21 @@
         URH_CHECK(urh_arena(ctx, (size_t)ntiles * cap, &staging));
         URH_CHECK(urh_arena(ctx, 8, &d_init));
     }
-    const bool speculate = !sharded && !h_iq && !sc && mod_type == URH_MOD_FSK && dtype == URH_DT_F32 &&
-                           getenv("URH_B200_NO_SPECULATE") == nullptr;
     UrhSpec spec = {};
     if (speculate) {
-        float* tg;
+        float *tg, *gv;
+        float2* gmm;
         URH_CHECK(urh_arena(ctx, 1, &tg));
-        URH_CHECK(urh_arena(ctx, 1, &spec.redone));
+        URH_CHECK(urh_arena(ctx, URH_GUESS_SAMPLES, &gv));
+        URH_CHECK(urh_arena(ctx, URH_GUESS_BLOCKS, &gmm));
         URH_CHECK(urh_arena(ctx, (size_t)ntiles, &spec.margin));
         spec.tg = tg;
+        spec.redone = &rec->redone;
+        urhts::Ws ws;
+        URH_CHECK(urhts::prepare(ctx, URH_GUESS_BLOCKS, &ws));
         const char* forced = getenv("URH_B200_SPECULATE_GUESS");
-        URH_LAUNCH(ctx, k_speculate_guess, 1, URH_GUESS_THREADS, 0, (const float2*)d_iq, n, dp.noise_sqrd, forced ? 1 : 0,
-                   forced ? strtof(forced, nullptr) : 0.0f, tg, spec.redone);
+        URH_LAUNCH(ctx, k_speculate_guess, URH_GUESS_BLOCKS, URH_GUESS_THREADS, 0, (const float2*)d_iq, n, dp.noise_sqrd, forced ? 1 : 0,
+                   forced ? strtof(forced, nullptr) : 0.0f, tg, gv, gmm, ws, (uint4*)fine.gh, fine_words / 4);
     }
     int chunk_no = 0;
     for (int64_t t0 = 0; t0 < (sc ? 0 : ntiles); t0 += chunk_tiles, chunk_no++) {
@@ -951,22 +990,18 @@
     }
     CenterPlan* plan = nullptr;
     URH_CHECK(urh_center_chain(ctx, d_qad_out, n, ts, max_size, sharded ? ctx->nccl_rank : 0, sharded ? ctx->nccl_world : 1,
-                               fine.gh ? &fine : nullptr, &plan));
+                               fine.gh ? &fine : nullptr, rec, &plan));
     const float* d_centerf;
-    const double* d_center;
-    const int* d_state;
-    urh_center_plan_result(ctx, plan, &d_centerf, &d_center, &d_state);
+    urh_center_plan_result(ctx, plan, &d_centerf, nullptr, nullptr);
     int64_t rows = 0;
     if (sc) {
-        URH_CUDA(ctx, cudaMemcpyAsync(ctx->h_mail + 40, d_center, sizeof(double), cudaMemcpyDeviceToHost, ctx->stream));
-        URH_CUDA(ctx, cudaMemcpyAsync(ctx->h_mail + 41, d_state, sizeof(int), cudaMemcpyDeviceToHost, ctx->stream));
-        URH_CHECK(urh_center_plan_certify_stats(ctx, plan, ctx->h_mail + 42));
-        URH_CUDA(ctx, cudaMemcpyAsync(ctx->h_mail + 45, (const int64_t*)ctx->center_prefix + ntiles, sizeof(int64_t), cudaMemcpyDeviceToHost,
+        URH_CUDA(ctx, cudaMemcpyAsync(ctx->h_mail, rec, sizeof(UrhStepRecord), cudaMemcpyDeviceToHost, ctx->stream));
+        URH_CUDA(ctx, cudaMemcpyAsync(ctx->h_mail + 40, (const int64_t*)ctx->center_prefix + ntiles, sizeof(int64_t), cudaMemcpyDeviceToHost,
                                       ctx->stream));
         URH_CUDA(ctx, cudaStreamSynchronize(ctx->stream));
-        int st0 = 0;
-        memcpy(&st0, ctx->h_mail + 41, sizeof(int));
-        if (st0 == 1) {
+        memcpy(&h_rec, ctx->h_mail, sizeof(UrhStepRecord));
+        *sc->kept = ctx->h_mail[40];
+        if (h_rec.state == 1) {
             StreamDigitizer dz;
             URH_CHECK(dz.init(ctx, n, scs, tol, mod_type == URH_MOD_ASK, samples_per_symbol));
             for (int64_t s0 = 0; s0 < n; s0 += scs) {
@@ -976,9 +1011,7 @@
             }
             rows = dz.rows;
         }
-        *sc->kept = ctx->h_mail[45];
     } else {
-        URH_CUDA(ctx, cudaMemsetAsync(d_init, 0, 16, ctx->stream));
         const int vec_in = (((uintptr_t)d_qad_out % 8) == 0) ? 1 : 0;
         int64_t grid = urh_div_up(ntiles, URH_WARPS_PER_BLOCK);
         if (speculate) {
@@ -989,24 +1022,19 @@
         }
         URH_LAUNCH(ctx, (k_dense_f32<SrcQad2, float>), (unsigned)grid, URH_WARPS_PER_BLOCK * 32, 0,
                    (const float*)d_qad_out, n, vec_in, cls, tol, tiles, staging, cap, d_init, 0, d_centerf, (const UrhTileStats*)ts, spec);
-        URH_CUDA(ctx, cudaMemcpyAsync(ctx->h_mail + 40, d_center, sizeof(double), cudaMemcpyDeviceToHost, ctx->stream));
-        URH_CUDA(ctx, cudaMemcpyAsync(ctx->h_mail + 41, d_state, sizeof(int), cudaMemcpyDeviceToHost, ctx->stream));
-        URH_CHECK(urh_center_plan_certify_stats(ctx, plan, ctx->h_mail + 42));
-        ctx->h_mail[46] = 0;
-        if (speculate) URH_CUDA(ctx, cudaMemcpyAsync(ctx->h_mail + 46, spec.redone, sizeof(unsigned int), cudaMemcpyDeviceToHost, ctx->stream));
         if (sharded)
-            URH_CHECK(urh_finish_shard(ctx, n, tol, mod_type == URH_MOD_ASK, samples_per_symbol, tiles, staging, cap, d_init, global_offset, n_total, &rows));
+            URH_CHECK(urh_finish_shard(ctx, n, tol, mod_type == URH_MOD_ASK, samples_per_symbol, tiles, staging, cap, d_init, global_offset, n_total, &rows,
+                                       rec, &h_rec));
         else
-            URH_CHECK(urh_finish_local(ctx, n, tol, mod_type == URH_MOD_ASK, samples_per_symbol, tiles, staging, cap, d_init, &rows));
-    }
-    memcpy(center, ctx->h_mail + 40, sizeof(double));
-    int st = 0;
-    memcpy(&st, ctx->h_mail + 41, sizeof(int));
+            URH_CHECK(urh_finish_local(ctx, n, tol, mod_type == URH_MOD_ASK, samples_per_symbol, tiles, staging, cap, d_init, &rows, rec, &h_rec));
+    }
+    *center = h_rec.center;
+    const int st = h_rec.state;
     *center_state = st;
-    ctx->center_cert[0] = ctx->h_mail[42];
+    ctx->center_cert[0] = h_rec.certified;
     ctx->center_cert[1] = fine.gh ? URH_FINE_NB : 0;
-    ctx->center_cert[2] = ctx->h_mail[44];
-    const int64_t redone = (spec.hi > spec.lo) ? ctx->h_mail[46] : 0;
+    ctx->center_cert[2] = h_rec.straddle;
+    const int64_t redone = (spec.hi > spec.lo) ? (int64_t)h_rec.redone : 0;
     ctx->spec_stats[0] = spec.hi - spec.lo;
     ctx->spec_stats[1] = spec.hi - spec.lo - redone;
     ctx->spec_stats[2] = redone;
diff --git a/urh_b200/csrc/finish.cu b/urh_b200/csrc/finish.cu
--- a/urh_b200/csrc/finish.cu
+++ b/urh_b200/csrc/finish.cu
@@ -36,6 +36,7 @@
     const UrhTileSummary* tiles;
     int64_t n;
     RunCarry* carry;
+    int64_t* minus1;
     __device__ __forceinline__ RunCarry load(int64_t t) const {
         const int64_t rem = n - t * URH_TILE;
         const int tile_len = rem < URH_TILE ? (int)rem : URH_TILE;
@@ -46,7 +47,13 @@
         r.flags = (s.head_len == tile_len) ? 1 : 0;
         return r;
     }
-    __device__ __forceinline__ void post(int64_t t, const RunCarry& excl, const RunCarry&) const { carry[t] = excl; }
+    __device__ __forceinline__ void post(int64_t t, const RunCarry& excl, const RunCarry&) const {
+        carry[t] = excl;
+        if (t == 0) {
+            ((longlong2*)minus1)[0] = make_longlong2(-1, -1);
+            ((longlong2*)minus1)[1] = make_longlong2(-1, -1);
+        }
+    }
 };
 
 struct __align__(16) TileFire {
@@ -343,6 +350,8 @@
     int emit_tail;
     UrhChain* chain;
     int64_t row_base, rows_cap;
+    UrhStepRecord* rec;
+    UrhStepRecord* h_rec;
 };
 
 static int finish_tiles(urh_ctx* ctx, int64_t n, int tol, bool is_ask, uint32_t sps, const UrhTileSummary* tiles, const uint32_t* staging,
@@ -361,7 +370,6 @@
     TileFire* fire;
     URH_CHECK(urh_arena(ctx, (size_t)ntiles, &fire));
     URH_CHECK(urh_arena(ctx, (size_t)(32 + 8 * (sharded ? sh.world : 0)), &d_small));
-    URH_CUDA(ctx, cudaMemsetAsync(d_small, 0xff, 4 * sizeof(int64_t), ctx->stream));
     RunCarry* d_tot_run = (RunCarry*)(d_small + 4);
     CandAgg* d_tot_cand = (CandAgg*)(d_small + 6);
     FireAgg* d_tot_fire = (FireAgg*)(d_small + 8);
@@ -377,7 +385,7 @@
     RunCarry rc_ident;
     rc_ident.len = 0; rc_ident.cls = 0; rc_ident.flags = 2 | 1;
     ScanRunCarry fa;
-    fa.tiles = tiles; fa.n = n; fa.carry = carry;
+    fa.tiles = tiles; fa.n = n; fa.carry = carry; fa.minus1 = d_small;
     URH_CHECK((urhts::scan<RunCarry, RunCarryOp, ScanRunCarry>(ctx, ntiles, rc_ident, RunCarryOp(), fa, d_tot_run)));
     if (sharded) {
         URH_LAUNCH(ctx, k_pack_stage1, 1, 1, 0, d_init, (const RunCarry*)d_tot_run, d_msg1);
@@ -430,9 +438,17 @@
     for (int attempt = 0; attempt < 2; attempt++) {
         URH_LAUNCH(ctx, k_finish_rows, (unsigned)urh_div_up(ntiles, 8 * FIN_TILES), 256, 0, tiles, staging, stage_cap, (const int32_t*)head_rel,
                    (const int32_t*)prev_cls, prev0, (const int64_t*)row_off, (const int64_t*)prev_fired, xprev, ntiles, sh.global_offset,
-                   sh.n_total, tol, is_ask ? 1 : 0, (int64_t)sps, sh.emit_tail, row_base, raw, raw_cap, d_small);
+                   sh.n_total, tol, is_ask ? 1 : 0, (int64_t)sps, sh.emit_tail, row_base, raw, raw_cap, sh.rec ? (int64_t*)&sh.rec->rows : d_small);
         if (sharded && attempt == 0) URH_TL_MARK(ctx, "rows written");
-        URH_CHECK(urh_read_i64(ctx, d_small, 2, got));
+        if (sh.rec) {
+            URH_CUDA(ctx, cudaMemcpyAsync(ctx->h_mail, sh.rec, sizeof(UrhStepRecord), cudaMemcpyDeviceToHost, ctx->stream));
+            URH_CUDA(ctx, cudaStreamSynchronize(ctx->stream));
+            memcpy(sh.h_rec, ctx->h_mail, sizeof(UrhStepRecord));
+            got[0] = sh.h_rec->rows;
+            got[1] = sh.h_rec->fired;
+        } else {
+            URH_CHECK(urh_read_i64(ctx, d_small, 2, got));
+        }
         if (sharded) URH_CHECK(urh_p2p_check(ctx));
         if (got[0] <= raw_cap) break;
         if (attempt == 1 || chain) URH_FAIL(ctx, URH_ERR_CUDA, "finish_tiles: row buffer overflow after regrowth");
@@ -472,22 +488,26 @@
     sh.rank = 0; sh.world = 1; sh.global_offset = global_offset; sh.n_total = n_total;
     sh.emit_tail = (global_offset + n == n_total) ? 1 : 0;
     sh.chain = chain; sh.row_base = row_base; sh.rows_cap = rows_cap;
+    sh.rec = nullptr; sh.h_rec = nullptr;
     return finish_tiles(ctx, n, tol, is_ask, sps, tiles, staging, stage_cap, d_init, sh, k);
 }
 
 int urh_finish_local(urh_ctx* ctx, int64_t n, int tol, bool is_ask, uint32_t sps, const UrhTileSummary* tiles, const uint32_t* staging,
-                     int stage_cap, const int16_t* d_init, int64_t* k) {
+                     int stage_cap, const int16_t* d_init, int64_t* k, UrhStepRecord* rec, UrhStepRecord* h_rec) {
     FinishShard sh;
     sh.rank = 0; sh.world = 1; sh.global_offset = 0; sh.n_total = n; sh.emit_tail = 1;
     sh.chain = nullptr; sh.row_base = 0; sh.rows_cap = 0;
+    sh.rec = rec; sh.h_rec = h_rec;
     return finish_tiles(ctx, n, tol, is_ask, sps, tiles, staging, stage_cap, d_init, sh, k);
 }
 
 int urh_finish_shard(urh_ctx* ctx, int64_t n, int tol, bool is_ask, uint32_t sps, const UrhTileSummary* tiles, const uint32_t* staging,
-                     int stage_cap, const int16_t* d_init, int64_t global_offset, int64_t n_total, int64_t* k) {
+                     int stage_cap, const int16_t* d_init, int64_t global_offset, int64_t n_total, int64_t* k, UrhStepRecord* rec,
+                     UrhStepRecord* h_rec) {
     FinishShard sh;
     sh.rank = ctx->nccl_rank; sh.world = ctx->nccl_world; sh.global_offset = global_offset; sh.n_total = n_total;
     sh.emit_tail = (ctx->nccl_rank == ctx->nccl_world - 1) ? 1 : 0;
     sh.chain = nullptr; sh.row_base = 0; sh.rows_cap = 0;
+    sh.rec = rec; sh.h_rec = h_rec;
     return finish_tiles(ctx, n, tol, is_ask, sps, tiles, staging, stage_cap, d_init, sh, k);
 }
diff --git a/urh_b200/csrc/tilescan.cuh b/urh_b200/csrc/tilescan.cuh
--- a/urh_b200/csrc/tilescan.cuh
+++ b/urh_b200/csrc/tilescan.cuh
@@ -156,6 +156,8 @@
 
 int prepare(urh_ctx* ctx, int64_t nblocks, Ws* out);
 
+__device__ __forceinline__ bool arrives_last(const Ws& ws) { return atomicAdd(ws.counter, 1ull) - ws.base == gridDim.x - 1; }
+
 template <typename T, typename Op, typename F, int ITEMS = 16>
 static inline int scan(urh_ctx* ctx, int64_t n, T identity, Op op, F f, T* d_total) {
     if (n <= 0) return URH_OK;
```
